# gavinsyw/2ACE-mmWave-Channel-Estimation

Measured on AMD Instinct MI355X. Metric: channel recoveries/sec (32-ant, 256 RSS meas, 200 ADMM iters) @1/2/4/8 GPU, higher is better.
Workload: dtype f64

## Files before the change

2ace-mmwave-channel-estimation_amd/ace_amd/_lib.py:

```python
from __future__ import annotations

import ctypes as C
import os
import pathlib

_HERE = pathlib.Path(__file__).resolve().parent
LIB_PATH = pathlib.Path(os.environ.get("ACE_LIB", _HERE / "libace.so"))

ACE_OK = 0
ACE_ERR_ARG = -1
ACE_ERR_UNSUPPORTED = -2
ACE_ERR_HIP = -3
ACE_ERR_WORKSPACE = -4

ACE_VARIANT_A2ONLY = 0
ACE_VARIANT_NUCLEAR = 1

ACE_ST_CONVERGED = 1
ACE_ST_NO_OPT = 2
ACE_ST_EIG_NOCONV = 4
ACE_ST_ROLLBACK = 8
ACE_ST_RANK_ONE = 128
ACE_ST_EVAL_DEGENERATE = 256
ACE_ST_RSS_SKIPPED = 512
ACE_ST_OMP_DEPENDENT = 1024
ACE_ST_GAMP_NANBREAK = 2048
ACE_ST_GAMP_MAXEM = 4096
ACE_ST_GAMP_FAILED = 8192

ACE_TRAIN_SHARED = 0
ACE_TRAIN_PER_REALISATION = 1

KERNEL_CLASSES = ["setup", "init", "pre", "apply_A", "apply_G", "ystep", "apply_K", "apply_AH", "zstep", "final", "msr"]


class AceError(RuntimeError):
    def __init__(self, code, msg):
        super().__init__(f"ace error {code}: {msg}")
        self.code = code


class AdmmCfg(C.Structure):
    _fields_ = [
        ("variant", C.c_int),
        ("scale_by_row", C.c_int),
        ("use_rank_one", C.c_int),
        ("maxiter", C.c_int),
        ("fixed_iters", C.c_int),
        ("a_shared", C.c_int),
        ("eig_warm", C.c_int),
        ("f64_applies", C.c_int),
        ("mu0", C.c_double),
        ("rho", C.c_double),
        ("tol_rel", C.c_double),
        ("tol_abs", C.c_double),
        ("r", C.c_int),
        ("reserved", C.c_int),
        ("rank_one", C.c_void_p),
    ]


class PipelineCfg(C.Structure):
    _fields_ = [
        ("variant", C.c_int),
        ("restarts", C.c_int),
        ("r", C.c_int),
        ("maxiter", C.c_int),
        ("eig_warm", C.c_int),
        ("stop_before_refine", C.c_int),
        ("train_layout", C.c_int),
        ("train_seed", C.c_int),
        ("mu0", C.c_double),
        ("rho", C.c_double),
        ("cc_frac", C.c_double),
        ("tol_rel", C.c_double),
        ("tol_abs", C.c_double),
    ]


class GampCfg(C.Structure):
    _fields_ = [
        ("snr_db", C.c_double),
        ("lambda0", C.c_double),
        ("learn_lambda", C.c_int),
        ("max_em_iter", C.c_int),
        ("gamp_nit", C.c_int),
        ("reserved", C.c_int),
        ("step0", C.c_double),
        ("gamp_tol", C.c_double),
    ]


class MinL2Cfg(C.Structure):
    _fields_ = [
        ("r", C.c_int),
        ("maxiter", C.c_int),
        ("train_seed", C.c_int),
        ("reserved", C.c_int),
        ("mu0", C.c_double),
        ("rho", C.c_double),
        ("cc_frac", C.c_double),
        ("tol_rel", C.c_double),
        ("tol_abs", C.c_double),
    ]


_dp, _ip, _bp = C.POINTER(C.c_double), C.POINTER(C.c_int32), C.POINTER(C.c_ubyte)


class StageArgs(C.Structure):
    _fields_ = ([(k, C.c_int32) for k in ("op", "row_mode", "batch", "n", "m", "r", "nc", "mt", "count", "ld", "col",
                                          "first", "scatter", "isentinel")]
                + [("or_mask", C.c_uint32), ("bit", C.c_uint32), ("len", C.c_int64)]
                + [(k, C.c_double) for k in ("mu0", "tol_abs", "value", "sentinel")]
                + [(k, _dp) for k in ("X", "Y", "P0", "B", "S", "g", "M", "A", "G", "geinv", "q", "qmax", "Xmax",
                                      "Ymax", "anorm", "bnorm", "optX", "optY", "Zb1", "Zb2", "Yb1", "Yb2", "src",
                                      "state")]
                + [(k, _ip) for k in ("flags", "rows", "idx", "isrc", "idst")]
                + [("mask", _bp), ("bsrc", _bp)]
                + [(k, _dp) for k in ("Xo", "Yo", "Mo", "No", "qo", "state_out")]
                + [("iout", _ip), ("flags_out", _ip), ("bout", _bp)])


def _load():
    if not LIB_PATH.exists():
        raise ImportError(
            f"ace_amd: HIP library {LIB_PATH} not found -- build it with "
            f"`make -C 2ace-mmwave-channel-estimation_amd/csrc` (or __graft_entry__.build()). "
            f"There is no CPU fallback on the product path.")
    lib = C.CDLL(str(LIB_PATH))
    vp, dp, ip, up = C.c_void_p, C.POINTER(C.c_double), C.POINTER(C.c_int32), C.POINTER(C.c_uint32)
    cfgp = C.POINTER(AdmmCfg)
    lib.ace_admm_cfg_default.argtypes = [cfgp]
    lib.ace_admm_cfg_default.restype = None
    lib.ace_admm_workspace_size.argtypes = [cfgp, C.c_int, C.c_int, C.c_int]
    lib.ace_admm_workspace_size.restype = C.c_size_t
    lib.ace_admm_solve_batch.argtypes = [cfgp, C.c_int, C.c_int, C.c_int, C.c_int, C.c_int,
                                         vp, vp, vp, vp, vp, vp, vp, vp, vp, C.c_size_t, vp]
    lib.ace_admm_solve_batch.restype = C.c_int
    lib.ace_admm_solve_host.argtypes = [cfgp, C.c_int, C.c_int, C.c_int, C.c_int, C.c_int,
                                        dp, dp, dp, dp, dp, ip, up, dp]
    lib.ace_admm_solve_host.restype = C.c_int
    pcfgp = C.POINTER(PipelineCfg)
    lib.ace_pipeline_cfg_default.argtypes = [pcfgp, C.c_int]
    lib.ace_pipeline_cfg_default.restype = None
    lib.ace_pipeline_workspace_size.argtypes = [pcfgp, C.c_int, C.c_int, C.c_int]
    lib.ace_pipeline_workspace_size.restype = C.c_size_t
    lib.ace_pipeline_solve_batch.argtypes = [pcfgp, C.c_int, C.c_int, C.c_int, C.c_int, C.c_int,
                                             vp, vp, ip, vp, vp, vp, vp, vp, vp, C.c_size_t, vp]
    lib.ace_pipeline_solve_batch.restype = C.c_int
    lib.ace_pipeline_solve_host.argtypes = [pcfgp, C.c_int, C.c_int, C.c_int, C.c_int, C.c_int,
                                            dp, dp, ip, dp, dp, dp, ip, up]
    lib.ace_pipeline_solve_host.restype = C.c_int
    lib.ace_synth_codebook.argtypes = [C.c_uint64, C.c_int64, C.c_int, C.c_int, C.c_int, vp, vp]
    lib.ace_synth_codebook.restype = C.c_int
    lib.ace_synth_channels.argtypes = [C.c_uint64, C.c_int64, C.c_int, C.c_int, C.c_int, C.c_int, C.c_int,
                                       C.c_double, C.c_double, vp, C.c_int, vp, vp, vp, vp]
    lib.ace_synth_channels.restype = C.c_int
    lib.ace_prof_start.argtypes = [C.c_int]
    lib.ace_prof_start.restype = C.c_int
    lib.ace_prof_sample.argtypes = [C.c_int, C.c_uint32]
    lib.ace_prof_sample.restype = C.c_int
    lib.ace_prof_stop.argtypes = [dp, ip]
    lib.ace_prof_stop.restype = C.c_int
    lib.ace_prof_msp_steps.argtypes = [C.POINTER(C.c_longlong)]
    lib.ace_prof_msp_steps.restype = C.c_int
    lib.ace_prof_work.argtypes = [dp]
    lib.ace_prof_work.restype = C.c_int
    lib.ace_prof_work_ex.argtypes = [dp, dp, dp]
    lib.ace_prof_work_ex.restype = C.c_int
    lib.ace_nuclear_prox_batch.argtypes = [C.c_int, C.c_int, C.c_int, vp, C.c_double, vp, vp]
    lib.ace_nuclear_prox_batch.restype = C.c_int
    lib.ace_evaluate_batch.argtypes = [C.c_int, C.c_int, C.c_int, vp, vp, vp, vp, vp]
    lib.ace_evaluate_batch.restype = C.c_int
    lib.ace_evaluate_host.argtypes = [C.c_int, C.c_int, C.c_int, dp, dp, dp, up]
    lib.ace_evaluate_host.restype = C.c_int
    lib.ace_rss_evaluate_batch.argtypes = [C.c_int, C.c_int, C.c_int, vp, vp, vp, C.c_int, vp, vp, vp, vp]
    lib.ace_rss_evaluate_batch.restype = C.c_int
    lib.ace_rss_evaluate_host.argtypes = [C.c_int, C.c_int, C.c_int, dp, dp, dp, C.c_int, dp, dp, up]
    lib.ace_rss_evaluate_host.restype = C.c_int
    lib.ace_beam_scan_batch.argtypes = [C.c_int] * 5 + [vp, vp, vp, vp, C.c_int, vp, vp, vp, vp, vp, vp]
    lib.ace_beam_scan_batch.restype = C.c_int
    lib.ace_beam_scan_host.argtypes = [C.c_int] * 5 + [dp, dp, dp, dp, C.c_int, dp, ip, dp, dp, up]
    lib.ace_beam_scan_host.restype = C.c_int
    lib.ace_omp_workspace_size.argtypes = [C.c_int] * 4
    lib.ace_omp_workspace_size.restype = C.c_size_t
    lib.ace_omp_solve_batch.argtypes = [C.c_int] * 4 + [C.c_double] + [vp] * 10 + [C.c_size_t, vp]
    lib.ace_omp_solve_batch.restype = C.c_int
    lib.ace_omp_solve_host.argtypes = [C.c_int] * 4 + [C.c_double, dp, dp, dp, ip, dp, ip, dp, up, dp]
    lib.ace_omp_solve_host.restype = C.c_int
    gcfgp = C.POINTER(GampCfg)
    lib.ace_gamp_cfg_default.argtypes = [gcfgp]
    lib.ace_gamp_cfg_default.restype = None
    lib.ace_gamp_workspace_size.argtypes = [C.c_int] * 3
    lib.ace_gamp_workspace_size.restype = C.c_size_t
    lib.ace_gamp_solve_batch.argtypes = [gcfgp] + [C.c_int] * 3 + [vp] * 9 + [C.c_size_t, vp]
    lib.ace_gamp_solve_batch.restype = C.c_int
    lib.ace_gamp_solve_host.argtypes = [gcfgp] + [C.c_int] * 3 + [dp, dp, dp, dp, dp, ip, ip, up]
    lib.ace_gamp_solve_host.restype = C.c_int
    mcfgp = C.POINTER(MinL2Cfg)
    lib.ace_minl2_cfg_default.argtypes = [mcfgp]
    lib.ace_minl2_cfg_default.restype = None
    lib.ace_minl2_workspace_size.argtypes = [C.c_int] * 4
    lib.ace_minl2_workspace_size.restype = C.c_size_t
    lib.ace_minl2_admm_batch.argtypes = [mcfgp] + [C.c_int] * 5 + [vp] * 12 + [vp, C.c_size_t, vp]
    lib.ace_minl2_admm_batch.restype = C.c_int
    lib.ace_minl2_admm_host.argtypes = [mcfgp] + [C.c_int] * 5 + [dp, dp, dp, ip, dp, dp, dp, ip, ip, dp, dp, up]
    lib.ace_minl2_admm_host.restype = C.c_int
    lib.ace_minl2_solve_workspace_size.argtypes = [mcfgp] + [C.c_int] * 3
    lib.ace_minl2_solve_workspace_size.restype = C.c_size_t
    lib.ace_minl2_solve_batch.argtypes = [mcfgp] + [C.c_int] * 3 + [vp, vp, ip] + [vp] * 6 + [vp, C.c_size_t, vp]
    lib.ace_minl2_solve_batch.restype = C.c_int
    lib.ace_minl2_solve_host.argtypes = [mcfgp] + [C.c_int] * 3 + [dp, dp, ip, dp, dp, dp, ip, ip, up]
    lib.ace_minl2_solve_host.restype = C.c_int
    lib.ace_spectral_init_host.argtypes = [C.c_int, C.c_int, C.c_int, C.c_int, vp, vp, vp, vp]
    lib.ace_spectral_init_host.restype = C.c_int
    lib.ace_path_counts.argtypes = [C.POINTER(C.c_int64), C.c_int]
    lib.ace_path_counts.restype = C.c_int
    lib.ace_lds_request.argtypes = [C.c_char_p, C.c_int, C.POINTER(C.c_size_t)]
    lib.ace_lds_request.restype = C.c_int
    lib.ace_stage_host.argtypes = [C.POINTER(StageArgs)]
    lib.ace_stage_host.restype = C.c_int
    lib.ace_last_error.argtypes = []
    lib.ace_last_error.restype = C.c_char_p
    lib.ace_version.argtypes = []
    lib.ace_version.restype = C.c_char_p
    return lib


LIB = _load()


def check(rc):
    if rc != ACE_OK:
        raise AceError(rc, LIB.ace_last_error().decode())
    return rc


PATHS = ("int8_shared", "codes_private", "f64_shared", "f64_private")


def path_counts(reset=False):
    v = (C.c_int64 * 4)()
    check(LIB.ace_path_counts(v, int(bool(reset))))
    return dict(zip(PATHS, v))


def lds_request(kernel: str, m: int) -> int:
    v = C.c_size_t()
    check(LIB.ace_lds_request(kernel.encode(), int(m), C.byref(v)))
    return v.value


def default_cfg(**kw) -> AdmmCfg:
    cfg = AdmmCfg()
    LIB.ace_admm_cfg_default(C.byref(cfg))
    for k, v in kw.items():
        if not hasattr(cfg, k):
            raise TypeError(f"unknown ace_admm_cfg field {k!r}")
        setattr(cfg, k, v)
    return cfg


def gamp_cfg(**kw) -> GampCfg:
    cfg = GampCfg()
    LIB.ace_gamp_cfg_default(C.byref(cfg))
    for k, v in kw.items():
        if not hasattr(cfg, k):
            raise TypeError(f"unknown ace_gamp_cfg field {k!r}")
        setattr(cfg, k, v)
    return cfg


def minl2_cfg(**kw) -> MinL2Cfg:
    cfg = MinL2Cfg()
    LIB.ace_minl2_cfg_default(C.byref(cfg))
    for k, v in kw.items():
        if not hasattr(cfg, k):
            raise TypeError(f"unknown ace_minl2_cfg field {k!r}")
        setattr(cfg, k, v)
    return cfg


def pipeline_cfg(variant, **kw) -> PipelineCfg:
    cfg = PipelineCfg()
    LIB.ace_pipeline_cfg_default(C.byref(cfg), int(variant))
    for k, v in kw.items():
        if not hasattr(cfg, k):
            raise TypeError(f"unknown ace_pipeline_cfg field {k!r}")
        setattr(cfg, k, v)
    return cfg
```

2ace-mmwave-channel-estimation_amd/csrc/ace_admm.cpp:

```cpp
#include "ace_host.hpp"

#include <cmath>
#include <cstdio>
#include <cstdlib>
#include <utility>
#include <vector>
#include <algorithm>
#include <map>
#include <mutex>

namespace ace {

size_t linops_bytes(bool shared, int batch, int m, int n) {
    Carver cv{nullptr};
    LinOps L;
    linops_carve(cv, shared, batch, m, n, &L);
    return cv.off;
}

void linops_carve(Carver& cv, bool shared, int batch, int m, int n, LinOps* L) {
    const size_t cz = 16, mats = shared ? 1 : (size_t)batch;
    L->shared = shared;
    L->m = m;
    L->n = n;
    L->AH = shared ? cv.take(cz * n * m) : nullptr;
    const bool pc = !shared && pc_supported(m, n);
    L->K = cv.take(mats * std::max(cz * m * m, pc ? pc_gw_bytes(m) : 0));
    L->G = cv.take(mats * std::max(cz * m * m, pc ? pc_gt_bytes(m) : 0));
    L->pcodes = pc ? cv.take<uint32_t>(pc_codes_bytes(m, n) * (size_t)batch) : nullptr;
    L->pcb = pc ? cv.take(sizeof(double) * (size_t)batch) : nullptr;
    L->pcflag = pc ? cv.take<int>(sizeof(int)) : nullptr;
    L->pc_ok = false;
    L->batch = batch;
    L->ns = shared ? cv.take(cz * 4 * m * m + 2 * sizeof(double)) : nullptr;
    L->LA8 = shared ? cv.take<int8_t>(i8_frag_bytes(m, n)) : nullptr;
    L->LAH8 = shared ? cv.take<int8_t>(i8_frag_bytes(n, m)) : nullptr;
    L->LK8 = shared ? cv.take<int8_t>(i8k_frag_bytes(m)) : nullptr;
    L->c8 = shared ? cv.take(2 * sizeof(double)) : nullptr;
    L->i8flag = shared ? cv.take<int>(sizeof(int)) : nullptr;
    L->Gf = shared && m <= GYK_MAXM ? cv.take(gyk_gfrag_bytes(m)) : nullptr;
    L->Kfr = shared && m <= GYK_MAXM ? cv.take(gyk_gfrag_bytes(m)) : nullptr;
    L->frag_ok = false;
    L->i8ok = false;
    L->gyk_ok = false;
    L->allow_i8 = true;
}

struct Knobs {
    int zcompact = 0, cold_sync = 0, msp_fail_it = -1, gyf_ctl = 1, msr_start = 56, msr_retry = 8, msr_waves = 8;
    int tkeig = 6;
    bool tk_trace = false;
    bool msr = true;
    bool fuse = true, gyf = true, mspace = true, lazy_dual = true, lean = true, nuc_msp = true, i8r = true, zcert = true;
    bool r1lz = true;
    double msp_room = 32.0;
};
static Knobs read_knobs() {
    Knobs k;
    const auto on = [](const char* name) {
        const char* e = getenv(name);
        return !(e && e[0] == '0');
    };
    const auto num = [](const char* name, double dflt) {
        const char* e = getenv(name);
        return e ? atof(e) : dflt;
    };
    k.zcompact = (int)num("ACE_ZCOMPACT", 0);
    k.cold_sync = exp_env("ACE_COLD_SYNC") ? atoi(exp_env("ACE_COLD_SYNC")) : 0;
    k.msp_fail_it = (int)num("ACE_MSP_FAIL_IT", -1);
    k.gyf_ctl = (int)num("ACE_GYF_CTL", 1);
    k.msp_room = num("ACE_MSP_ROOM", 32.0);
    k.fuse = on("ACE_FUSE");
    k.gyf = on("ACE_GYF");
    k.mspace = on("ACE_MSPACE");
    k.lazy_dual = on("ACE_LAZY_DUAL");
    k.lean = on("ACE_LEAN");
    k.nuc_msp = on("ACE_NUC_MSP");
    k.i8r = on("ACE_I8_STAGES");
    k.msr = on("ACE_MSR");
    k.zcert = on("ACE_ZCERT");
    k.r1lz = on("ACE_R1_LANCZOS");
    k.tkeig = (int)num("ACE_TK_EIG", 6);
    k.tk_trace = num("ACE_TK_TRACE", 0) != 0;
    k.msr_start = (int)num("ACE_MSR_START", 56);
    k.msr_retry = (int)num("ACE_MSR_RETRY", 8);
    if (k.msr_retry < 1) k.msr_retry = 1;
    k.msr_waves = (int)num("ACE_MSR_WAVES", 8) == 4 ? 4 : 8;
    return k;
}
static bool msr_trace() {
    static const bool v = [] {
        const char* e = exp_env("ACE_MSR_TRACE");
        return e && e[0] == '1';
    }();
    return v;
}
static bool fuse_ok(const Knobs& k, int m) {
    return k.fuse && lds_ok_budget(i8ah_budget(1), i8ah_lds_bytes(m) + i8ah_fuse_lds_bytes());
}
static bool gyf_ok(const Knobs& k, int m) { return k.gyf && lds_ok_budget(gyf_budget(), gyf_lds_bytes(m)); }

static bool i8_disabled() {
    static const bool v = [] {
        const char* e = getenv("ACE_NO_I8");
        return e && e[0] == '1';
    }();
    return v;
}

static int i8_setup(LinOps& L, hipStream_t st) {
    const int m = L.m, n = L.n;
    L.i8ok = false;
    if (!L.allow_i8 || i8_disabled()) return ACE_OK;
    ACE_HIP(hipMemsetAsync(L.LA8, 0, i8_frag_bytes(m, n), st));
    ACE_HIP(hipMemsetAsync(L.LAH8, 0, i8_frag_bytes(n, m), st));
    ACE_HIP(hipMemsetAsync(L.i8flag, 0, sizeof(int), st));
    launch_max_abs(2LL * m * n, L.A, L.c8, st);
    launch_i8_expand(m, n, L.A, L.c8, L.LA8, L.LAH8, L.i8flag, st);
    int flag = 1;
    double c[2] = {0.0, 0.0};
    ACE_HIP(read_back(&flag, L.i8flag, sizeof(int), st));
    ACE_HIP(read_back(c, L.c8, sizeof(double), st));
    L.i8ok = flag == 0 && c[0] > 0.0 && std::isfinite(c[0]) && lds_ok_budget(i8ah_budget(0), i8ah_lds_bytes(m)) &&
             lds_ok_budget(i8ah_budget(2), i8ah_lds_bytes(m));
    if (!L.i8ok) return ACE_OK;
    c[1] = c[0] * c[0];
    ACE_HIP(upload(L.c8 + 1, c + 1, sizeof(double), st));
    ACE_HIP(hipMemsetAsync(L.LK8, 0, i8k_frag_bytes(m), st));
    launch_i8k_expand(m, L.K, L.c8, L.LK8, L.i8flag, st);
    ACE_HIP(read_back(&flag, L.i8flag, sizeof(int), st));
    L.i8ok = flag == 0;
    L.gyk_ok = L.i8ok && L.Gf && lds_ok_budget(gyk_budget(), gyk_lds_bytes(m));
    return ACE_OK;
}

int ns_inverse(LinOps& L, hipStream_t st) {
    const int m = L.m;
    const long long mm = (long long)m * m;
    double* Ap = L.ns;
    double* Id = L.ns + 2 * mm;
    double* R = L.ns + 4 * mm;
    double* Xn = L.ns + 6 * mm;
    double* X = L.G;
    double* flag = L.ns + 8 * mm;
    launch_ns_prep(m, L.K, Ap, Id, X, st, flag + 1);
    double b = 0.0;
    ACE_HIP(read_back(&b, flag + 1, sizeof(double), st));
    int kpred = 60;
    if (std::isfinite(b) && b >= 1.0) {
        const double rho = (b - 1.0) / (b + 1.0);
        kpred = 0;
        for (double e = rho; e >= 1e-10 && kpred < 60; e *= e) ++kpred;
    }
    int it = 0;
    bool done = false;
    auto step = [&]() -> int {
        launch_zgemm(1, true, m, m, m, Ap, m, 0, X, m, 0, R, Id, m, 0, 1, st);
        launch_zgemm(2, true, m, m, m, R, m, 0, X, m, 0, Xn, X, m, 0, 1, st);
        launch_hermitize(m, Xn, st);
        std::swap(X, Xn);
        ++it;
        return ACE_OK;
    };
    for (int k = 0; k <= kpred && k < 60; ++k) ACE_TRY(step());
    {
        double h = 0.0;
        launch_max_abs(2 * mm, R, flag, st);
        ACE_HIP(read_back(&h, flag, sizeof(double), st));
        done = h < 1e-10;
    }
    for (; it < 60 && !done;) {
        launch_zgemm(1, true, m, m, m, Ap, m, 0, X, m, 0, R, Id, m, 0, 1, st);
        double h = 0.0;
        launch_max_abs(2 * mm, R, flag, st);
        ACE_HIP(read_back(&h, flag, sizeof(double), st));
        done = h < 1e-10;
        launch_zgemm(2, true, m, m, m, R, m, 0, X, m, 0, Xn, X, m, 0, 1, st);
        launch_hermitize(m, Xn, st);
        std::swap(X, Xn);
        ++it;
    }
#ifdef ACE_DEBUG_SPEC
    fprintf(stderr, "ns_inverse m %d b %g kpred %d it %d done %d\n", m, b, kpred, it, (int)done);
#endif
    if (!done) return fail(ACE_ERR_UNSUPPORTED, "setup: Newton-Schulz inverse of I + K did not converge");
    if (X != L.G) ACE_HIP(hipMemcpyAsync(L.G, X, sizeof(double) * 2 * mm, hipMemcpyDeviceToDevice, st));
    return ACE_OK;
}

static int pc_setup(LinOps& L, int batch, hipStream_t st) {
    const int m = L.m, n = L.n;
    L.pc_ok = false;
    if (L.shared || !L.pcodes || !L.allow_i8 || i8_disabled() || !pc_supported(m, n) || batch != L.batch ||
        !zstep_takes_w(ACE_VARIANT_A2ONLY, 1))
        return ACE_OK;
    ACE_HIP(hipMemsetAsync(L.pcflag, 0, sizeof(int), st));
    launch_pc_pack(batch, m, n, L.A, L.pcb, L.pcodes, L.pcflag, st);
    int flag = 1;
    ACE_HIP(read_back(&flag, L.pcflag, sizeof(int), st));
    if (flag != 0) return ACE_OK;
    launch_pc_ginv(batch, m, n, L.pcodes, L.pcb, L.K, L.G, st);
    ACE_LAUNCHED("private setup (code images, G_b)");
    L.pc_ok = true;
    return ACE_OK;
}

int linops_setup(LinOps& L, int batch, hipStream_t st) {
    const int m = L.m, n = L.n;
    const int mats = L.shared ? 1 : batch;
    const long long mm = (long long)m * m, mn = (long long)m * n;
    ProfScope ps(ACE_K_SETUP, st);
    if (!L.shared) {
        ACE_TRY(pc_setup(L, batch, st));
        if (L.pc_ok) return ACE_OK;
    }
    launch_zgemm(0, true, m, n, m, L.A, n, mn, L.A, n, mn, L.K, nullptr, m, mm, mats, st);
    if (L.shared) {
        ACE_TRY(ns_inverse(L, st));
    } else {
        ACE_HIP(hipMemcpyAsync(L.G, L.K, sizeof(double) * 2 * mm * mats, hipMemcpyDeviceToDevice, st));
        launch_inv_ipk(m, mats, L.G, mm, st);
    }
    if (L.shared) {
        launch_conj_transpose(m, n, L.A, L.AH, st);
        L.frag_ok = L.Gf && L.Kfr;
        if (L.frag_ok) {
            launch_gyk_gfrag(m, L.G, L.Gf, st);
            launch_gyk_gfrag(m, L.K, L.Kfr, st);
        }
        ACE_TRY(i8_setup(L, st));
    }
    ACE_LAUNCHED("operator setup (K, G, A^H, fragments, digit planes)");
    return ACE_OK;
}

void admm_state_carve(Carver& cv, int batch, int m, int n, int r, AdmmState* s) {
    const size_t cz = 16, bn = (size_t)batch * r * n, bm = (size_t)batch * r * m;
    s->X = cv.take(cz * bn);
    s->Z = cv.take(cz * bn);
    s->N = cv.take(cz * bn);
    s->V = cv.take(cz * bn);
    s->optX = cv.take(cz * bn);
    s->Q = cv.take(cz * (size_t)batch * 32 * 32);
    s->Z2 = cv.take(cz * (size_t)batch * n);
    s->N2 = cv.take(cz * (size_t)batch * n);
    s->AX = cv.take(cz * (size_t)batch * m);
    for (int i = 0; i < 2; ++i) s->Y[i] = cv.take(cz * bm);
    for (int i = 0; i < 2; ++i) s->KY[i] = cv.take(cz * bm);
    s->M = cv.take(cz * bm);
    s->S = cv.take(cz * bm);
    s->T = cv.take(cz * bm);
    s->g = cv.take(cz * bm);
    s->optY = cv.take(cz * bm);
    s->ypart = cv.take(sizeof(double) * 5 * (size_t)batch * r * ((m + 63) / 64));
// ... 96 lines not shown
        SplitRes& r = it->second;
        r.used = ++tick;
        for (int h = 0; h < nsplit; ++h) {
            ev[h] = r.e[h];
            cev[h] = r.c[h];
            if (h > 0) ss[h] = r.s[h];
        }
    }
    ACE_HIP(hipEventRecord(ev[0], st));
    for (int h = 1; h < nsplit; ++h) ACE_HIP(hipStreamWaitEvent(ss[h], ev[0], 0));
    std::vector<AdmmState> ws(nsplit);
    std::vector<int> nb(nsplit);
    for (int h = 0; h < nsplit; ++h) {
        const long long ob = (long long)h * chunk;
        nb[h] = (int)std::max(0LL, std::min((long long)chunk, batch - ob));
        ws[h] = state_slice(w, ob, m, n, za0.tx);
    }
    static const int stg = [] {
        const char* e = exp_env("ACE_STAGGER");
        return e ? atoi(e) : 0;
    }();
    hipEvent_t evs = nullptr;
    if (stg > 0 && nsplit > 1) ACE_HIP(hipEventCreateWithFlags(&evs, hipEventDisableTiming));
    auto split_fail = [&](int lc) -> int {
        for (int h = 1; h < nsplit; ++h)
            if (hipEventRecord(ev[h], ss[h]) == hipSuccess) (void)hipStreamWaitEvent(st, ev[h], 0);
        if (evs) (void)hipEventDestroy(evs);
        return lc;
    };
#define SPLIT_LAUNCHED(stage)                                           \
    do {                                                                \
        const int lc_ = ::ace::launch_check(stage, __FILE__, __LINE__); \
        if (lc_) return split_fail(lc_);                                \
    } while (0)
    auto stagger_mark = [&](int h, int it, int k) -> hipError_t {
        return (evs && h == 0 && it == 1 && k == stg) ? hipEventRecord(evs, ss[0]) : hipSuccess;
    };
    const bool lean = p.variant != ACE_VARIANT_NUCLEAR && za0.warm && za0.Q && kn.lean;
    const bool msp = lean && za0.lazy_dual && fuse_ok(kn, m) && gyf_ok(kn, m) && kn.mspace;
    const DualCtl dc{za0.tol_abs, za0.tol_rel, za0.rho, za0.fixed_iters, n, 1, w.done};
    const int cold_sync = kn.cold_sync;
    auto barrier = [&]() -> int {
        for (int h = 0; h < nsplit; ++h) ACE_HIP(hipEventRecord(cev[h], ss[h]));
        for (int h = 0; h < nsplit; ++h)
            for (int k = 0; k < nsplit; ++k)
                if (k != h) ACE_HIP(hipStreamWaitEvent(ss[h], cev[k], 0));
        return ACE_OK;
    };
    const bool msr = msp && kn.msr && kn.gyf_ctl && msr_supported(m) && gyf_ok(kn, m) && fuse_ok(kn, m);
    int msr_next = kn.msr_start;
    int q = 0, rc = ACE_OK;
    for (int it = 1; it <= p.maxiter && rc == ACE_OK; ++it) {
        bool run_msr = false;
        if (msr && it >= msr_next && it < p.maxiter) {
            for (int h = 1; h < nsplit; ++h) {
                ACE_HIP(hipEventRecord(cev[h], ss[h]));
                ACE_HIP(hipStreamWaitEvent(st, cev[h], 0));
            }
            ACE_HIP(hipMemsetD32Async(reinterpret_cast<hipDeviceptr_t>(w.done + 28), 0, 3, st));
            launch_msr_ready(batch, w.st, it, w.done + 28, st);
            int nr[3] = {0, 0, 0};
            ACE_HIP(read_back(nr, w.done + 28, sizeof(nr), st));
            run_msr = nr[0] == 0;
            if (msr_trace())
                fprintf(stderr, "msr check it %d: not ready %d (not m-space %d, test pending %d)\n", it, nr[0], nr[1],
                        nr[2]);
            if (!run_msr) msr_next = it + kn.msr_retry;
        }
        if (run_msr) {
            int pidx[4] = {-1, -1, -1, -1};
            for (int h = 0; h < nsplit; ++h) {
                if (nb[h] == 0) continue;
                const AdmmState& wh = ws[h];
                ZArgs za = za0;
                za.it = it;
                za.st = wh.st;
                za.msp = 1;
                za.msp_fail_it = kn.msp_fail_it;
                za.rank_one = za0.rank_one ? za0.rank_one + (long long)h * chunk : nullptr;
                const MsrArgs ma{L.Gf, B + (long long)h * chunk * m, {wh.Y[0], wh.Y[1]}, wh.M, wh.AX,
                                 {wh.Sg[0], wh.Sg[1]}, wh.optS, wh.optY, wh.st, w.done + 8 + h, w.done + 1,
                                 w.done + 12 + 4 * h, msr_trace() ? w.done + 40 + h : nullptr, nb[h], m, it, p.maxiter};
                ACE_HIP(hipMemsetD32Async(reinterpret_cast<hipDeviceptr_t>(w.done + 8 + h), p.maxiter, 1, ss[h]));
                ACE_HIP(hipMemsetD32Async(reinterpret_cast<hipDeviceptr_t>(w.done + 12 + 4 * h), 0, 4, ss[h]));
                ProfScope ps(ACE_K_MSR, ss[h]);
                pidx[h] = ps.idx;
                launch_msr(ma, za, kn.msr_waves, ss[h]);
                SPLIT_LAUNCHED("m-space run (msr_kernel)");
            }
            for (int h = 1; h < nsplit; ++h) {
                ACE_HIP(hipEventRecord(cev[h], ss[h]));
                ACE_HIP(hipStreamWaitEvent(st, cev[h], 0));
            }
            int rv[20] = {p.maxiter, p.maxiter, p.maxiter, p.maxiter};
            ACE_HIP(read_back(rv, w.done + 8, sizeof(int) * 20, st));
            for (int h = 0; h < nsplit; ++h) {
                if (pidx[h] >= 0) g_prof.work[pidx[h]] = 8.0 * m * m * rv[4 + 4 * h];
                if (msr_trace())
                    fprintf(stderr, "msr h %d it %d: resume %d steps %d notready %d fail %d pend %d\n", h, it, rv[h],
                            rv[4 + 4 * h], rv[5 + 4 * h], rv[6 + 4 * h], rv[7 + 4 * h]);
            }
            if (msr_trace()) {
                int vw[4] = {0, 0, 0, 0};
                ACE_HIP(read_back(vw, w.done + 40, sizeof(vw), st));
                fprintf(stderr, "msr it %d: vectors written %d %d %d %d (m = %d)\n", it, vw[0], vw[1], vw[2], vw[3], m);
            }
            int e = p.maxiter;
            for (int h = 0; h < nsplit; ++h)
                if (nb[h] > 0) e = std::min(e, std::max(it, rv[h]));
            it = e;
            q = (it - 1) & 1;
            msr_next = e + kn.msr_retry;
        }
        const bool csync = nsplit > 1 && it <= cold_sync;
      for (int phase = 0; phase < (csync ? 2 : 1); ++phase) {
        const int pmask = csync ? (1 << phase) : 3;
        for (int h = 0; h < nsplit; ++h) {
            if (nb[h] == 0) continue;
            const AdmmState& wh = ws[h];
            const hipStream_t sh = ss[h];
            if (evs && h > 0 && it == 1) ACE_HIP(hipStreamWaitEvent(sh, evs, 0));
            const double* Bh = B + (long long)h * chunk * m;
            double* Zc = (it & 1) ? wh.Z : wh.Z2;
            double* Nc = (it & 1) ? wh.N : wh.N2;
            ACE_HIP(stagger_mark(h, it, 1));
            ZArgs za = za0;
            za.it = it;
            za.wmode = 1;
            za.yfused = 1;
            za.ypart = nullptr;
            za.X = wh.X;
            za.Z = Zc;
            za.N = Nc;
            za.Zn = (it & 1) ? wh.Z2 : wh.Z;
            za.Nn = (it & 1) ? wh.N2 : wh.N;
            za.Q = wh.Q;
            za.st = wh.st;
            za.optX = wh.optX;
            za.optY = wh.optY;
            za.Xcur = wh.V;
            za.Ynew = wh.Y[1 - q];
            za.Yold = wh.Y[q];
            za.fixup_now = it == p.maxiter;
            za.rank_one = za0.rank_one ? za0.rank_one + (long long)h * chunk : nullptr;
            za.lean = lean;
            za.compact = lean && kn.zcompact > 0 && it > kn.zcompact && it != p.maxiter;
            za.xfuse = lean && (it != p.maxiter || msp) && fuse_ok(kn, m);
            za.msp = msp;
            za.Af = L.A;
            za.Sold = wh.Sg[(it + 1) & 1];
            za.Snew = wh.Sg[it & 1];
            za.optS = wh.optS;
            za.msp_fail_it = kn.msp_fail_it;
            const bool gyf = za.xfuse && za0.lazy_dual && gyf_ok(kn, m);
            GykArgs ga{L.Gf, wh.T, Bh, wh.Y[q], wh.M, wh.Y[1 - q], wh.g, wh.KY[q], wh.KY[1 - q], wh.optY,
                       L.LK8, L.c8, wh.st, wh.AX, 2 - q, L.LA8, Zc, Nc, w.zeros, n, za0.lazy_dual, dc, gyf ? 1 : 0,
                       gyf && msp ? 1 : 0, it, za.Sold, wh.Sg[it & 1], wh.optS, za0.np,
                       {za0.fl[0], za0.fl[1], za0.fl[2], za0.fl[3]}, za.rank_one, kn.msp_room};
            if (!(pmask & 1)) {
            } else if (gyf) {
                ProfScope ps(ACE_K_APPLY_G, sh);
                launch_gyf(nb[h], m, n, ga, L.LAH8, wh.X, za, kn.gyf_ctl, sh);
                SPLIT_LAUNCHED("g / Y-step / apply_AH (gyf_kernel)");
            } else {
                {
                    ProfScope ps(ACE_K_APPLY_G, sh);
                    launch_gyk(nb[h], m, ga, sh);
                }
                SPLIT_LAUNCHED("g / Y-step (gyk_kernel)");
                ACE_HIP(stagger_mark(h, it, 2));
                ProfScope ps(ACE_K_APPLY_AH, sh);
                launch_i8_apply_AH(nb[h], m, n, L.LAH8, wh.g, wh.X, L.c8, wh.st, sh, za.xfuse ? &za : nullptr);
                SPLIT_LAUNCHED("apply_AH (i8ah_kernel)");
            }
            ACE_HIP(stagger_mark(h, it, 3));
            if (pmask & 2) {
                ProfScope ps(ACE_K_ZSTEP, sh);
                if (lean && !za.xfuse) launch_zlean(za, nb[h], sh);
                launch_zstep(p.variant, false, za, nb[h], sh);
                SPLIT_LAUNCHED("Z-step");
            }
        }
        if (csync) ACE_TRY(barrier());
      }
        q = 1 - q;
        if (!p.fixed_iters && (it % 8 == 0) && it < p.maxiter) {
            for (int h = 1; h < nsplit; ++h) {
                ACE_HIP(hipEventRecord(cev[h], ss[h]));
                ACE_HIP(hipStreamWaitEvent(st, cev[h], 0));
            }
            int h_done = 0;
            ACE_HIP(read_back(&h_done, w.done, sizeof(int), st));
            if (h_done >= batch) break;
        }
    }
    for (int h = 1; h < nsplit; ++h) {
        ACE_HIP(hipEventRecord(ev[h], ss[h]));
        ACE_HIP(hipStreamWaitEvent(st, ev[h], 0));
    }
    ACE_LAUNCHED("split iterations");
#undef SPLIT_LAUNCHED
    {
        ProfScope ps(ACE_K_FINAL, st);
        if (msp) launch_i8_msp_optx(batch, m, n, L.LAH8, w.optS, w.optX, L.c8, w.st, w.Z, w.Z2, w.Sg[0], w.Sg[1], st);
        if (msp && g_prof.on && g_prof.msp_used < g_prof.msp_cap)
            ACE_HIP(hipMemcpyAsync(g_prof.msp_slots + g_prof.msp_used++, w.done + 1, sizeof(int),
                                   hipMemcpyDeviceToHost, st));
        launch_finalize_r(n, m, 1, 1, batch, w.optX, w.optY, w.V, w.Y[q], Xo, Yo, iters, status, mu_out, w.st, st, w.Z,
                          w.Z2, w.Y[0], w.Y[1]);
    }
    ACE_LAUNCHED("finalize (split)");
    if (evs) ACE_HIP(hipEventDestroy(evs));
    return rc;
}

static int admm_nuclear_msp(const LinOps& L, const AdmmParams& p, const AdmmState& w, const ZArgs& za0, int batch,
                            const double* B, double* Xo, double* Yo, int32_t* iters, uint32_t* status,
                            double* mu_out, hipStream_t st) {
    const int m = L.m, n = L.n;
    NmsArgs a{};
    a.Gf = L.Gf;
    a.Kf = L.Kfr;
    a.B = B;
    a.M = w.M;
    double *Eb[2] = {w.Sg[0], w.Sg[1]}, *AEb[2] = {w.KY[0], w.KY[1]};
    a.Eo = Eb[0];
    a.En = Eb[1];
    a.AEo = AEb[0];
    a.AEn = AEb[1];
    a.P0 = w.T;
    a.optW = w.optS;
    a.optY = w.optY;
    a.curW = w.g;
    a.rs = w.st;
    a.dc = DualCtl{za0.tol_abs, za0.tol_rel, za0.rho, za0.fixed_iters, n, 1, w.done};
    ZArgs za = za0;
    za.lazy_dual = 1;
    {
        ProfScope ps(ACE_K_INIT, st);
        launch_zgemm(0, false, m, n, batch, L.A, n, 0, w.X, n, 0, w.T, nullptr, m, 0, 1, st);
        launch_nms_init(batch, n, m, w.X, a, st);
    }
    int q = 0, it = 1;
    for (; it <= p.maxiter; ++it) {
        a.Yo = w.Y[q];
        a.Yn = w.Y[1 - q];
        a.Eo = Eb[q];
        a.En = Eb[1 - q];
        a.AEo = AEb[q];
        a.AEn = AEb[1 - q];
        za.it = it;
        {
            ProfScope ps(ACE_K_APPLY_G, st);
            launch_nms(batch, m, a, za, false, st);
        }
        ACE_LAUNCHED("A2nuclear m-space iteration (nms_kernel)");
        q = 1 - q;
        if (!p.fixed_iters && (it % 8 == 0) && it < p.maxiter) {
            int h_done = 0;
            ACE_HIP(read_back(&h_done, w.done, sizeof(int), st));
            if (h_done >= batch) break;
        }
    }
    {
        ProfScope ps(ACE_K_FINAL, st);
        a.Yo = w.Y[q];
        a.Yn = w.Y[1 - q];
        za.it = std::min(it, p.maxiter);
        launch_nms(batch, m, a, za, true, st);
        launch_nms_out(batch, n, m, w.X, a, w.V, w.g, st);
        launch_zgemm(2, false, n, m, batch, L.AH, m, 0, w.g, m, 0, w.optX, w.V, n, 0, 1, st);
        launch_finalize_r(n, m, 1, 1, batch, w.optX, w.optY, w.optX, w.Y[q], Xo, Yo, iters, status, mu_out, w.st, st,
                          nullptr, nullptr, nullptr, nullptr);
    }
    ACE_LAUNCHED("finalize (A2nuclear m-space)");
    return ACE_OK;
}

static int tk_report(const Knobs& kn, const AdmmState& w, int rc, hipStream_t st) {
    if (!kn.tk_trace || rc != ACE_OK) return rc;
    int tkc[2] = {0, 0};
    ACE_HIP(read_back(tkc, w.done + 32, sizeof(tkc), st));
    fprintf(stderr, "[ace] tridiagonal Z-steps %d, Jacobi fallbacks %d\n", tkc[0], tkc[1]);
    return rc;
}

int admm_run(const LinOps& L, const AdmmParams& p, const AdmmState& w, int batch, const double* B,
             const double* X0, double* Xo, double* Yo, int32_t* iters, uint32_t* status, double* mu_out,
             hipStream_t st) {
    const int m = L.m, n = L.n, r = p.r;
    const Knobs kn = read_knobs();
    if (!L.shared && r != 1) return fail(ACE_ERR_UNSUPPORTED, "private sensing matrices support r = 1 only");
    if (p.part && (r == 1 || !L.shared || p.part->m != m))
        return fail(ACE_ERR_UNSUPPORTED, "per-realisation partitions run the r-column stages on a shared A");
    const int row_mode = (r == 1) ? 1 : p.row_mode;
    const int nv = batch * r;
    const long long mm = (long long)m * m, mn = (long long)m * n;
    const bool fast = (r == 1);
    const bool fused = fast && L.shared;
    const bool i8 = fused && L.i8ok && zstep_takes_w(p.variant, r);
    const bool gyk = i8 && L.gyk_ok;
    const bool pc = !L.shared && L.pc_ok && r == 1 && zstep_takes_w(p.variant, r);
    const bool wmode = i8 || pc;
    const bool i8r = !fast && L.shared && L.i8ok && kn.i8r && nv >= 256;
    g_path[(i8 || i8r) ? 0 : pc ? 1 : L.shared ? 2 : 3].fetch_add(1, std::memory_order_relaxed);
    if (L.pc_ok && !pc) return fail(ACE_ERR_UNSUPPORTED, "private phase-code setup without its iteration path");

    auto applyA = [&](int mode, const double* Vin, double* C, const double* E) {
        if (L.shared) launch_zgemm(mode, false, m, n, nv, L.A, n, 0, Vin, n, 0, C, E, m, 0, 1, st);
        else launch_zgemv_rows(mode, m, n, batch, L.A, mn, Vin, n, C, E, m, st);
    };
    auto applyMM = [&](const double* Lm, const double* Vin, double* C) {
        if (L.shared) launch_zgemm(0, false, m, m, nv, Lm, m, 0, Vin, m, 0, C, nullptr, m, 0, 1, st);
        else launch_zgemv_rows(0, m, m, batch, Lm, mm, Vin, m, C, nullptr, m, st);
    };
    auto applyAH = [&](const double* gin, double* C, const double* E) {
        if (L.shared) launch_zgemm(2, false, n, m, nv, L.AH, m, 0, gin, m, 0, C, E, n, 0, 1, st);
        else launch_zgemv_cols(2, m, n, batch, L.A, mn, gin, m, C, E, n, st);
    };

    ZArgs za{};
    za.n = n;
    za.m = m;
    za.tx = p.tx;
    za.rx = p.rx;
    za.r = r;
    za.row_mode = row_mode;
    za.X = w.X;
    za.N = w.N;
    za.Z = w.Z;
    za.Q = w.Q;
    za.st = w.st;
    za.optX = w.optX;
    za.optY = w.optY;
    za.done_count = w.done;
    za.np = rank_profile(p.prof_tx ? p.prof_tx : p.tx, p.rx, m, p.prof_n ? p.prof_n : n,
                         p.rank_one ? 0 : p.use_rank_one, za.rl, za.fl);
    za.rank_one = p.rank_one;
    za.tol_rel = p.tol_rel;
    za.tol_abs = p.tol_abs;
    za.rho = p.rho;
    za.fixed_iters = p.fixed_iters;
    za.warm = p.eig_warm;
    za.zcert = kn.zcert ? 1 : 0;
    za.mthr = p.part ? p.part->mt : 0;
    za.r1lz = kn.r1lz ? 1 : 0;
    za.tkeig = kn.tkeig > 0 ? kn.tkeig : 0;
    za.tkcnt = w.done + 32;
    za.wmode = 0;
    za.Xcur = w.V;
    za.Zn = nullptr;
    za.Nn = nullptr;
    za.zeros = w.zeros;
    za.nuclear = p.variant == ACE_VARIANT_NUCLEAR;
    za.lazy_dual = (gyk && kn.lazy_dual) ? 1 : 0;
    za.Kf = L.K;

    const bool nms = L.shared && L.frag_ok && r == 1 && p.variant == ACE_VARIANT_NUCLEAR && kn.nuc_msp && nms_supported(m);
    ACE_HIP(hipMemsetAsync(w.done, 0, 256, st));
    ACE_HIP(hipMemsetAsync(w.zeros, 0, 16 * (size_t)n, st));
    {
        ProfScope ps(ACE_K_INIT, st);
        if (pc) launch_pc_apply_a(batch, m, n, L.pcodes + pc_codesA_off(batch, m, n), L.pcb, X0, w.T, st);
        else applyA(0, X0, w.T, nullptr);
        launch_init_r(row_mode, n, m, r, batch, X0, w.T, B, w.X, w.Y[0], w.M, w.N, w.st, p.mu0, st, p.part);
        if (!nms) {
            za.it = 0;
            launch_zstep(p.variant, true, za, batch, st);
            if (!pc && !za.lazy_dual) applyMM(L.K, w.Y[0], w.KY[0]);
        }
    }
    ACE_LAUNCHED("init (A X0, init, Z-step)");
    if (nms) return admm_nuclear_msp(L, p, w, za, batch, B, Xo, Yo, iters, status, mu_out, st);

    int q = 0;
    const int poll = 8;
    const int nsplit = gyk ? split_count(batch) : 1;
    if (nsplit > 1 || (gyk && kn.mspace && p.variant != ACE_VARIANT_NUCLEAR))
        return tk_report(kn, w, admm_iterate_split(L, p, w, za, batch, B, nsplit, kn, Xo, Yo, iters, status, mu_out, st), st);
    const double fl_mn = 8.0 * m * n * nv, fl_mm = 8.0 * m * m * nv;
    const double vb = 16.0 * nv;
    const double op_mn = 2.0 * 8 * (2.0 * m) * (2.0 * n) * nv, op_mm = 2.0 * 8 * 2 * (2.0 * m) * (2.0 * m) * nv;
    const double shA = L.shared ? 16.0 * m * n : 16.0 * m * n * batch, shM = L.shared ? 16.0 * m * m : 16.0 * m * m * batch;
    const double zs_fl = !fast ? (p.variant == ACE_VARIANT_NUCLEAR
                                      ? 8.0 * 3 * n * r * r * batch
                                      : (8.0 * p.tx * p.tx * p.rx * r + 0.8e6 * std::pow(p.tx / 32.0, 3)) * batch)
                               : 0.0;
    const double zs_b = !fast ? (80.0 * n * r + 64.0 * m * r + 32.0 * p.tx * p.tx) * batch : 0.0;
    double *Zc = w.Z, *Nc = w.N, *Zo = w.Z2, *No = w.N2;
    double lv = 1.0;
    for (int it = 1; it <= p.maxiter; ++it) {
        if (pc) {
            ProfScope ps(ACE_K_APPLY_G, st);
            const PgkArgs pa{m, n, L.pcodes, L.pcodes + pc_codesA_off(batch, m, n), L.G, L.pcb, B, w.Y[q], w.M,
                             w.Y[1 - q], w.X, w.optY, w.st, w.AX, 2 - q, Zc, Nc, w.zeros};
            launch_pgk(batch, pa, st);
            ACE_LAUNCHED("private g / Y-step / apply_AH (pgk_kernel)");
        } else if (gyk) {
        } else if (i8) {
            ProfScope ps(ACE_K_APPLY_A, st);
            launch_i8_apply_A(batch, n, m, L.LA8, Zc, Nc, w.Y[q], w.M, w.T, L.c8, w.st, w.zeros, gyk ? w.AX : nullptr, st);
            ACE_LAUNCHED("apply_A (i8a_kernel)");
        } else if (fused) {
            ProfScope ps(ACE_K_APPLY_A, st, lv * (fl_mn));
            launch_zgemm_fused(true, m, n, batch, L.A, n, w.Z, w.N, n, w.T, w.Y[q], w.M, m, w.st, st);
        } else {
            {
                ProfScope ps(ACE_K_PRE, st, 0.0, lv * (vb * (3.0 * m + (i8r ? 0.0 : 3.0 * n))));
                launch_pre(n * r, m * r, batch, w.Z, w.N, w.Y[q], w.M, i8r ? nullptr : w.V, w.S, w.st, st);
            }
            if (i8r) {
                ProfScope ps(ACE_K_APPLY_A, st, 0.0, lv * (vb * (2.0 * n + 3.0 * m)), lv * (op_mn));
                launch_i8_apply_A(nv, n, m, L.LA8, w.Z, w.N, w.Y[q], w.M, w.T, L.c8, w.st, w.zeros, nullptr, st, r);
                ACE_LAUNCHED("r-column apply_A (i8a_kernel)");
            } else {
                ProfScope ps(ACE_K_APPLY_A, st, lv * (fl_mn), lv * (vb * (n + 2.0 * m) + shA));
                applyA(1, w.V, w.T, w.S);
            }
        }
        if (pc) {
        } else if (gyk) {
            ProfScope ps(ACE_K_APPLY_G, st);
            const GykArgs ga{L.Gf, w.T, B, w.Y[q], w.M, w.Y[1 - q], w.g, w.KY[q], w.KY[1 - q], w.optY, L.LK8, L.c8, w.st,
                             w.AX, 2 - q, L.LA8, Zc, Nc, w.zeros, n, za.lazy_dual,
                             DualCtl{za.tol_abs, za.tol_rel, za.rho, za.fixed_iters, n, 1, w.done}};
            launch_gyk(batch, m, ga, st);
            ACE_LAUNCHED("g / Y-step (gyk_kernel)");
        } else if (fused) {
            ProfScope ps(ACE_K_APPLY_G, st, lv * (fl_mm));
            const YsArgs ys{B, w.Y[q], w.M, w.Y[1 - q], w.ypart};
            launch_zgemm_ystep(m, batch, L.G, w.T, w.g, ys, w.st, st);
        } else {
            {
                ProfScope ps(ACE_K_APPLY_G, st, lv * (fl_mm), lv * (vb * 2.0 * m + shM) * (p.part ? 2.0 : 1.0));
                applyMM(L.G, w.T, w.g);
                if (p.part) launch_part_gfix(batch, r, *p.part, L.G, w.g, w.st, st);
            }
            {
                ProfScope ps(ACE_K_YSTEP, st, 0.0, lv * (vb * 6.0 * m + 8.0 * m * batch));
                if (fast) launch_ystep(m, batch, w.S, w.g, w.M, B, w.Y[q], w.Y[1 - q], w.st, st);
                else launch_ystep_r(row_mode, m, r, batch, w.S, w.g, w.M, B, w.Y[q], w.Y[1 - q], w.st, st, p.part);
            }
        }
        ACE_LAUNCHED("apply_A / g = G T / Y-step");
        if (!gyk && !pc) {
            ProfScope ps(ACE_K_APPLY_K, st, lv * ((i8 || i8r) ? 0.0 : fl_mm), lv * ((i8 && !i8r) ? 0.0 : vb * 2.0 * m + (i8r ? 0.0 : shM)), lv * (i8r ? op_mm : 0.0));
            if (i8) launch_i8_apply_K(batch, m, L.LK8, w.Y[1 - q], w.KY[1 - q], L.c8, w.st, st);
            else if (i8r) launch_i8_apply_K(nv, m, L.LK8, w.Y[1 - q], w.KY[1 - q], L.c8, w.st, st, r);
            else applyMM(L.K, w.Y[1 - q], w.KY[1 - q]);
            ACE_LAUNCHED((i8 || i8r) ? "K Y (i8ah_kernel<KY>)" : "K Y (zgemm)");
        }
        if (!pc) {
            ProfScope ps(ACE_K_APPLY_AH, st, lv * ((wmode || i8r) ? 0.0 : fl_mn),
                         lv * (wmode ? 0.0 : i8r ? vb * (m + 3.0 * n) : vb * (m + 2.0 * n) + shA), lv * (i8r ? op_mn : 0.0));
            if (wmode) {
                za.xfuse = gyk && wmode && p.variant != ACE_VARIANT_NUCLEAR && za.warm && za.Q && kn.lean &&
                           it != p.maxiter && fuse_ok(kn, m);
                if (za.xfuse) {
                    za.it = it;
                    za.wmode = 1;
                    za.Z = Zc;
                    za.N = Nc;
                    za.Zn = Zo;
                    za.Nn = No;
                }
                launch_i8_apply_AH(batch, m, n, L.LAH8, w.g, w.X, L.c8, w.st, st, za.xfuse ? &za : nullptr);
            }
            else if (fused) launch_zgemm_fused(false, n, m, batch, L.AH, m, w.g, nullptr, m, w.X, w.Z, w.N, n, w.st, st);
            else if (i8r) {
                ZArgs zv{};
                zv.r = r;
                zv.xzn = 1;
                zv.Z = w.Z;
                zv.N = w.N;
                zv.zeros = w.zeros;
                launch_i8_apply_AH(nv, m, n, L.LAH8, w.g, w.X, L.c8, w.st, st, nullptr, &zv);
            } else applyAH(w.g, w.X, w.V);
            ACE_LAUNCHED((wmode || i8r) ? "apply_AH (i8ah_kernel)" : "apply_AH (zgemm)");
        }
        za.it = it;
        za.wmode = wmode;
        if (wmode) {
            za.Z = Zc;
            za.N = Nc;
            za.Zn = Zo;
            za.Nn = No;
        }
        za.ypart = fused && !gyk ? w.ypart : nullptr;
        za.yfused = gyk || pc;
        za.ytiles = (m + 63) / 64;
        za.Ynew = w.Y[1 - q];
        za.Yold = w.Y[q];
        za.KYnew = w.KY[1 - q];
        za.KYold = w.KY[q];
        za.lean = wmode && p.variant != ACE_VARIANT_NUCLEAR && za.warm && za.Q && kn.lean;
        za.fixup_now = it == p.maxiter;
        za.compact = za.lean && kn.zcompact > 0 && it > kn.zcompact;
        {
            ProfScope ps(ACE_K_ZSTEP, st, lv * (zs_fl), lv * (zs_b));
            if (za.lean && !za.xfuse) launch_zlean(za, batch, st);
            launch_zstep(p.variant, false, za, batch, st);
            ACE_LAUNCHED("Z-step");
        }
        q = 1 - q;
        if (wmode) {
            std::swap(Zc, Zo);
            std::swap(Nc, No);
        }
        if (!p.fixed_iters && (it % poll == 0) && it < p.maxiter) {
            int h_done = 0;
            ACE_HIP(read_back(&h_done, w.done, sizeof(int), st));
            if (h_done >= batch) break;
            lv = (double)(batch - h_done) / batch;
        }
    }
    {
        ProfScope ps(ACE_K_FINAL, st);
        launch_finalize_r(n, m, r, row_mode ? r : 1, batch, w.optX, w.optY, wmode ? w.V : w.X, w.Y[q], Xo, Yo, iters, status,
                          mu_out, w.st, st, wmode ? w.Z : nullptr, wmode ? w.Z2 : nullptr, (gyk || pc) ? w.Y[0] : nullptr,
                          (gyk || pc) ? w.Y[1] : nullptr);
    }
    ACE_LAUNCHED("finalize");
    return tk_report(kn, w, ACE_OK, st);
}

}
```

2ace-mmwave-channel-estimation_amd/csrc/ace_api.cpp:

```cpp
#include <algorithm>
#include <cstring>
#include <mutex>
#include <unordered_map>

#include "ace_host.hpp"

using namespace ace;

namespace {
int cols(const ace_admm_cfg* c) { return c->r == 0 ? 1 : c->r; }

int validate(const ace_admm_cfg* c, int batch, int m, int n, int tx, int rx) {
    if (!c) return fail(ACE_ERR_ARG, "cfg is NULL");
    if (batch < 1 || m < 1 || n < 1) return fail(ACE_ERR_ARG, "batch/m/n must be >= 1 (got %d/%d/%d)", batch, m, n);
    if (tx * rx != n) return fail(ACE_ERR_ARG, "n (%d) != tx*rx (%d*%d)", n, tx, rx);
    if (c->variant != ACE_VARIANT_A2ONLY && c->variant != ACE_VARIANT_NUCLEAR)
        return fail(ACE_ERR_ARG, "unknown variant %d", c->variant);
    if (c->variant == ACE_VARIANT_A2ONLY && (tx < 1 || tx > 32 || ((tx & 1) && tx > 31) || rx > 32))
        return fail(ACE_ERR_UNSUPPORTED, "A2only Z-prox needs tx in [1,32] and rx <= 32 (got %d, %d)", tx, rx);
    if (n > 4096 || m > 4096) return fail(ACE_ERR_UNSUPPORTED, "m, n must be <= 4096 (got %d, %d)", m, n);
    if (c->maxiter < 1) return fail(ACE_ERR_ARG, "maxiter must be >= 1");
    if (!(c->mu0 > 0) || !(c->rho > 0)) return fail(ACE_ERR_ARG, "mu0 and rho must be > 0");
    const int r = cols(c);
    if (r < 1 || r > 32) return fail(ACE_ERR_UNSUPPORTED, "r must be in [1, 32] (got %d)", r);
    if (r > 1 && !c->a_shared) return fail(ACE_ERR_UNSUPPORTED, "r > 1 needs a shared A (a_shared = 1)");
    return ACE_OK;
}
}

namespace ace {
namespace {
std::mutex g_lds_mu;
std::unordered_map<const void*, size_t> g_lds_budget;
thread_local std::string t_refused;
}

size_t lds_dyn_budget(const void* kernel) {
    std::lock_guard<std::mutex> lk(g_lds_mu);
    const auto it = g_lds_budget.find(kernel);
    if (it != g_lds_budget.end()) return it->second;
    hipFuncAttributes fa{};
    size_t budget = 0;
    if (hipFuncGetAttributes(&fa, kernel) == hipSuccess && fa.sharedSizeBytes < LDS_PER_CU) {
        const size_t want = LDS_PER_CU - fa.sharedSizeBytes;
        if (hipFuncSetAttribute(kernel, hipFuncAttributeMaxDynamicSharedMemorySize, (int)want) == hipSuccess)
            budget = want;
    }
    (void)hipGetLastError();
    g_lds_budget.emplace(kernel, budget);
    return budget;
}

void launch_refused(const char* kernel, size_t need, size_t budget) {
    if (!t_refused.empty()) return;
    char buf[256];
    snprintf(buf, sizeof buf, "%s not launched: %zu B of dynamic LDS requested, budget %zu B", kernel, need, budget);
    t_refused = buf;
}

bool lds_ok_budget(size_t budget, size_t need) { return need <= 64 * 1024 || need <= budget; }
bool lds_ok(const void* kernel, size_t need) {
    return need <= 64 * 1024 || need <= lds_dyn_budget(kernel);
}
bool lds_fits(const void* kernel, const char* name, size_t need) {
    if (lds_ok(kernel, need)) return true;
    launch_refused(name, need, lds_dyn_budget(kernel));
    return false;
}

int launch_check(const char* stage, const char* file, int line) {
    if (!t_refused.empty()) {
        const std::string why = t_refused;
        t_refused.clear();
        (void)hipGetLastError();
        return fail(ACE_ERR_UNSUPPORTED, "%s: %s (%s:%d)", stage, why.c_str(), file, line);
    }
    const hipError_t e = hipGetLastError();
    if (e != hipSuccess) return fail(ACE_ERR_HIP, "%s: launch failed: %s (%s:%d)", stage, hipGetErrorString(e), file, line);
    return ACE_OK;
}
}

extern "C" {

const char* ace_last_error(void) { return g_err.c_str(); }
const char* ace_version(void) { return "ace-mi355x 0.1.0 (gfx950)"; }

int ace_lds_request(const char* kernel, int m, size_t* bytes) {
    g_err.clear();
    if (!kernel || !bytes || m < 1) return fail(ACE_ERR_ARG, "bad ace_lds_request arguments");
    const std::string k = kernel;
    if (k == "i8ah" || k == "i8ah_ky") *bytes = i8ah_lds_bytes(m);
    else if (k == "i8ah_fuse") *bytes = i8ah_lds_bytes(m) + i8ah_fuse_lds_bytes();
    else if (k == "gyk") *bytes = gyk_lds_bytes(m);
    else if (k == "gyf") *bytes = gyf_lds_bytes(m);
    else if (k == "msr") *bytes = msr_request_bytes();
    else if (k == "nms") *bytes = nms_lds_bytes(m);
    else if (k == "hetrd") *bytes = hetrd_request_bytes(m, 0);
    else if (k == "hetrd_blk") *bytes = hetrd_request_bytes(m, 1);
    else if (k == "he2hb") *bytes = heev2_request_bytes(m, 0);
    else if (k == "hb2st") *bytes = heev2_request_bytes(m, 1);
    else if (k == "bt2") *bytes = heev2_request_bytes(m, 2);
    else if (k == "scan") *bytes = scan_request_bytes();
    else if (k == "omp") *bytes = omp_request_bytes(m);
    else if (k == "gamp") *bytes = gamp_request_bytes(m);
    else if (k == "minl2") *bytes = minl2_request_bytes(m);
    else if (k == "part_geinv") *bytes = part_geinv_request_bytes(m);
    else return fail(ACE_ERR_ARG, "unknown kernel '%s'", kernel);
    return ACE_OK;
}

int ace_prof_sample(int stride, uint32_t full_mask) {
    g_err.clear();
    if (stride < 1) return fail(ACE_ERR_ARG, "stride must be >= 1");
    g_prof.stride = stride;
    g_prof.full = full_mask;
    return ACE_OK;
}

int ace_prof_start(int max_launches) {
    g_err.clear();
    if (max_launches < 1) return fail(ACE_ERR_ARG, "max_launches must be >= 1");
    for (hipEvent_t e : g_prof.ev) (void)hipEventDestroy(e);
    g_prof.ev.assign(2 * (size_t)max_launches, nullptr);
    for (auto& e : g_prof.ev) ACE_HIP(hipEventCreate(&e));
    g_prof.cls.assign(max_launches, 0);
    g_prof.work.assign(max_launches, 0.0);
    g_prof.wbytes.assign(max_launches, 0.0);
    g_prof.wops.assign(max_launches, 0.0);
    g_prof.used = 0;
    for (int& c : g_prof.seen) c = 0;
    if (!g_prof.msp_slots) {
        g_prof.msp_cap = 4096;
        ACE_HIP(hipHostMalloc(reinterpret_cast<void**>(&g_prof.msp_slots), sizeof(int) * g_prof.msp_cap));
    }
    g_prof.msp_used = 0;
    g_prof.on = true;
    return ACE_OK;
}

int ace_prof_msp_steps(long long* steps) {
    g_err.clear();
    if (!steps) return fail(ACE_ERR_ARG, "steps is NULL");
    *steps = g_prof.msp_total;
    return ACE_OK;
}

int ace_prof_work(double* flops) {
    g_err.clear();
    if (!flops) return fail(ACE_ERR_ARG, "flops is NULL");
    for (int c = 0; c < ACE_NKCLASS; ++c) flops[c] = g_prof.work_tot[c];
    return ACE_OK;
}

int ace_prof_work_ex(double* flops, double* bytes, double* int8_ops) {
    g_err.clear();
    for (int c = 0; c < ACE_NKCLASS; ++c) {
        if (flops) flops[c] = g_prof.work_tot[c];
        if (bytes) bytes[c] = g_prof.bytes_tot[c];
        if (int8_ops) int8_ops[c] = g_prof.ops_tot[c];
    }
    return ACE_OK;
}

int ace_path_counts(int64_t* counts, int reset) {
    g_err.clear();
    for (int k = 0; k < 4; ++k) {
        const long long v = reset ? g_path[k].exchange(0) : g_path[k].load();
        if (counts) counts[k] = v;
    }
    return ACE_OK;
}

int ace_prof_stop(double* total_ms, int32_t* launches) {
    g_err.clear();
    g_prof.on = false;
    for (int c = 0; c < ACE_NKCLASS; ++c) {
        if (total_ms) total_ms[c] = 0.0;
        if (launches) launches[c] = 0;
        g_prof.work_tot[c] = g_prof.bytes_tot[c] = g_prof.ops_tot[c] = 0.0;
    }
    for (size_t i = 0; i < g_prof.used; ++i) {
        ACE_HIP(hipEventSynchronize(g_prof.ev[2 * i + 1]));
        float ms = 0.f;
        ACE_HIP(hipEventElapsedTime(&ms, g_prof.ev[2 * i], g_prof.ev[2 * i + 1]));
        const int c = g_prof.cls[i];
        g_prof.work_tot[c] += g_prof.work[i];
        g_prof.bytes_tot[c] += g_prof.wbytes[i];
        g_prof.ops_tot[c] += g_prof.wops[i];
        if (total_ms) total_ms[c] += ms;
        if (launches) launches[c] += 1;
    }
    for (hipEvent_t e : g_prof.ev) (void)hipEventDestroy(e);
    g_prof.ev.clear();
    g_prof.cls.clear();
    g_prof.work.clear();
    g_prof.wbytes.clear();
    g_prof.wops.clear();
    g_prof.used = 0;
    ACE_HIP(hipDeviceSynchronize());
    g_prof.msp_total = 0;
    for (int i = 0; i < g_prof.msp_used; ++i) g_prof.msp_total += g_prof.msp_slots[i];
    g_prof.msp_used = 0;
    return ACE_OK;
}

void ace_admm_cfg_default(ace_admm_cfg* c) {
    std::memset(c, 0, sizeof *c);
    c->variant = ACE_VARIANT_A2ONLY;
    c->scale_by_row = 1;
    c->use_rank_one = 0;
    c->maxiter = 500;
    c->fixed_iters = 0;
    c->a_shared = 1;
    c->eig_warm = 1;
    c->mu0 = 1e-3;
    c->rho = 1.03;
    c->tol_rel = 1e-4;
    c->tol_abs = 1e-8;
    c->r = 1;
    c->rank_one = nullptr;
}

size_t ace_admm_workspace_size(const ace_admm_cfg* cfg, int batch, int m, int n) {
    if (!cfg || batch < 1 || m < 1 || n < 1) return 0;
    Carver cv{nullptr};
    LinOps L;
    AdmmState w;
    linops_carve(cv, cfg->a_shared != 0, batch, m, n, &L);
    admm_state_carve(cv, batch, m, n, std::max(1, cols(cfg)), &w);
    return cv.off + 256;
}

}

namespace {
int solve_core(const ace_admm_cfg* cfg, int batch, int m, int n, int tx, int rx, int prof_tx, int prof_n,
               const double* A, const double* B, const double* X0, double* Xo, double* Yo, int32_t* iters,
               uint32_t* status, double* mu_out, void* workspace, size_t workspace_bytes, hipStream_t st);

int solve_odd_tx(const ace_admm_cfg* cfg, int batch, int m, int n, int tx, int rx, const double* A,
                 const double* B, const double* X0, double* Xo, double* Yo, int32_t* iters, uint32_t* status,
                 double* mu_out, hipStream_t st) {
    const int txp = tx + 1, np = txp * rx, r = cols(cfg), R = cfg->scale_by_row ? r : 1;
    const size_t arows = (size_t)(cfg->a_shared ? 1 : batch) * m * rx, xrows = (size_t)batch * r * rx,
                 orows = (size_t)batch * R * rx, ws = ace_admm_workspace_size(cfg, batch, m, np) + 4096;
    DevScope d;
    d.borrow(st);
    double *dA, *dX0, *dX;
    char* dW;
    ACE_TRY(d.alloc(&dA, 2 * arows * txp));
    ACE_TRY(d.alloc(&dX0, 2 * xrows * txp));
    ACE_TRY(d.alloc(&dX, 2 * orows * txp));
    ACE_TRY(d.alloc(&dW, ws));
    ACE_HIP(hipMemsetAsync(dA, 0, arows * txp * 16, st));
    ACE_HIP(hipMemsetAsync(dX0, 0, xrows * txp * 16, st));
    ACE_HIP(hipMemcpy2DAsync(dA, (size_t)txp * 16, A, (size_t)tx * 16, (size_t)tx * 16, arows, hipMemcpyDeviceToDevice, st));
    ACE_HIP(hipMemcpy2DAsync(dX0, (size_t)txp * 16, X0, (size_t)tx * 16, (size_t)tx * 16, xrows, hipMemcpyDeviceToDevice,
                             st));
    ACE_TRY(solve_core(cfg, batch, m, np, txp, rx, tx, n, dA, B, dX0, dX, Yo, iters, status, mu_out, dW, ws, st));
    ACE_HIP(hipMemcpy2DAsync(Xo, (size_t)tx * 16, dX, (size_t)txp * 16, (size_t)tx * 16, orows, hipMemcpyDeviceToDevice,
                             st));
    return ACE_OK;
}
}

extern "C" {

int ace_admm_solve_batch(const ace_admm_cfg* cfg, int batch, int m, int n, int tx, int rx, const double* A,
                         const double* B, const double* X0, double* Xo, double* Yo, int32_t* iters, uint32_t* status,
                         double* mu_out, void* workspace, size_t workspace_bytes, void* stream) {
    g_err.clear();
    int rc = validate(cfg, batch, m, n, tx, rx);
    if (rc) return rc;
    if (!A || !B || !X0 || !Xo || !Yo || !workspace) return fail(ACE_ERR_ARG, "NULL buffer");
    hipStream_t st = (hipStream_t)stream;
    if (cfg->variant == ACE_VARIANT_A2ONLY && (tx & 1))
        return solve_odd_tx(cfg, batch, m, n, tx, rx, A, B, X0, Xo, Yo, iters, status, mu_out, st);
    return solve_core(cfg, batch, m, n, tx, rx, 0, 0, A, B, X0, Xo, Yo, iters, status, mu_out, workspace,
                      workspace_bytes, st);
}

}

namespace {
int solve_core(const ace_admm_cfg* cfg, int batch, int m, int n, int tx, int rx, int prof_tx, int prof_n,
               const double* A, const double* B, const double* X0, double* Xo, double* Yo, int32_t* iters,
               uint32_t* status, double* mu_out, void* workspace, size_t workspace_bytes, hipStream_t st) {
    const size_t need = ace_admm_workspace_size(cfg, batch, m, n);
    if (need > workspace_bytes)
        return fail(ACE_ERR_WORKSPACE, "workspace too small: need %zu bytes, got %zu", need, workspace_bytes);
    poison_workspace(workspace, workspace_bytes, st);
    Carver cv{(char*)(((uintptr_t)workspace + 255) & ~(uintptr_t)255)};
    LinOps L;
    AdmmState w;
    linops_carve(cv, cfg->a_shared != 0, batch, m, n, &L);
    admm_state_carve(cv, batch, m, n, cols(cfg), &w);
    L.A = A;
    L.allow_i8 = cfg->f64_applies == 0;
    ACE_TRY(linops_setup(L, batch, st));
    AdmmParams p{};
    p.variant = cfg->variant;
    p.r = cols(cfg);
    p.row_mode = cfg->scale_by_row != 0;
    p.maxiter = cfg->maxiter;
    p.fixed_iters = cfg->fixed_iters;
    p.eig_warm = cfg->eig_warm;
    p.mu0 = cfg->mu0;
    p.rho = cfg->rho;
    p.tol_rel = cfg->tol_rel;
    p.tol_abs = cfg->tol_abs;
    p.tx = tx;
    p.rx = rx;
    p.prof_tx = prof_tx;
    p.prof_n = prof_n;
    p.use_rank_one = cfg->use_rank_one;
    p.rank_one = cfg->rank_one;
    return admm_run(L, p, w, batch, B, X0, Xo, Yo, iters, status, mu_out, st);
}
}

extern "C" {

int ace_admm_solve_host(const ace_admm_cfg* cfg, int batch, int m, int n, int tx, int rx, const double* A,
                        const double* B, const double* X0, double* X, double* Y, int32_t* iters, uint32_t* status,
                        double* mu) {
    g_err.clear();
    int rc = validate(cfg, batch, m, n, tx, rx);
    if (rc) return rc;
    const int r = cols(cfg), R = cfg->scale_by_row ? r : 1;
    const size_t nA = (size_t)(cfg->a_shared ? 1 : batch) * m * n * 2;
    const size_t nB = (size_t)batch * m, nX0 = (size_t)batch * r * n * 2, nX = (size_t)batch * R * n * 2,
                 nY = (size_t)batch * R * m * 2;
    const size_t ws = ace_admm_workspace_size(cfg, batch, m, n) + 4096;
    DevScope d;
    double *dA, *dB, *dX0, *dX, *dY, *dM;
    char* dW;
    int32_t* dI;
    uint32_t* dS;
    ACE_TRY(d.put(&dA, A, nA));
    ACE_TRY(d.put(&dB, B, nB));
    ACE_TRY(d.put(&dX0, X0, nX0));
    ACE_TRY(d.alloc(&dX, nX));
    ACE_TRY(d.alloc(&dY, nY));
    ACE_TRY(d.alloc(&dW, ws));
    ACE_TRY(d.alloc(&dI, (size_t)batch));
    ACE_TRY(d.alloc(&dS, (size_t)batch));
    ACE_TRY(d.alloc(&dM, (size_t)batch));
    ace_admm_cfg dcfg = *cfg;
    if (cfg->rank_one) {
        uint8_t* dR;
        ACE_TRY(d.put(&dR, cfg->rank_one, (size_t)batch));
        dcfg.rank_one = dR;
    }
    ACE_TRY(ace_admm_solve_batch(&dcfg, batch, m, n, tx, rx, dA, dB, dX0, dX, dY, dI, dS, dM, dW, ws, nullptr));
    ACE_HIP(hipDeviceSynchronize());
// ... 40 lines not shown
```

2ace-mmwave-channel-estimation_amd/csrc/ace_common.hpp:

```cpp
#pragma once
#include <hip/hip_runtime.h>
#include <stdint.h>
#include <cstdlib>

#include "../../include/ace.h"

namespace ace {

using d2 = double2;
typedef double d4v __attribute__((ext_vector_type(4)));

__device__ __forceinline__ d2 cmul(d2 a, d2 b) { return make_double2(a.x * b.x - a.y * b.y, a.x * b.y + a.y * b.x); }
__device__ __forceinline__ d2 cmulc(d2 a, d2 b) {  return make_double2(a.x * b.x + a.y * b.y, a.x * b.y - a.y * b.x); }
__device__ __forceinline__ d2 cadd(d2 a, d2 b) { return make_double2(a.x + b.x, a.y + b.y); }
__device__ __forceinline__ d2 csub(d2 a, d2 b) { return make_double2(a.x - b.x, a.y - b.y); }
__device__ __forceinline__ d2 cscale(d2 a, double s) { return make_double2(a.x * s, a.y * s); }
__device__ __forceinline__ double cabs2(d2 a) { return a.x * a.x + a.y * a.y; }

struct RealState {
    double mu, last_res, opt_obj, nB;
    double obj2, nAX2, nY2, nJM2, dY2;
    double vbound;
    double dAtY, nAtY;
    int32_t iters, done, status, objcol;
// ... 51 lines not shown
}
__device__ __forceinline__ double bsum16(double v) {
    v += bfly16<1>(v);
    v += bfly16<2>(v);
    v += bfly16<4>(v);
    v += bfly16<8>(v);
    return v;
}
__device__ __forceinline__ double bmax16(double v) {
    v = fmax(v, bfly16<1>(v));
    v = fmax(v, bfly16<2>(v));
    v = fmax(v, bfly16<4>(v));
    v = fmax(v, bfly16<8>(v));
    return v;
}
__device__ __forceinline__ double wave_sum(double v) {
#pragma unroll
    for (int o = 32; o > 0; o >>= 1) v += __shfl_xor(v, o, 64);
    return v;
}

__device__ __forceinline__ double wave_max(double v) {
#pragma unroll
    for (int o = 32; o > 0; o >>= 1) v = fmax(v, __shfl_xor(v, o, 64));
    return v;
}

struct VMax {
    double m = 0.0, s = 0.0;
    __device__ __forceinline__ void add(double2 v) {
        const double ax = fabs(v.x), ay = fabs(v.y);
        m = fmax(m, fmax(ax, ay));
        s += 0.0 * (ax + ay);
    }
};

__device__ __forceinline__ double xor16_sum(double v) {
    const auto lo = __builtin_amdgcn_permlane16_swap(__double2loint(v), __double2loint(v), false, false);
    const auto hi = __builtin_amdgcn_permlane16_swap(__double2hiint(v), __double2hiint(v), false, false);
    return __hiloint2double(hi[0], lo[0]) + __hiloint2double(hi[1], lo[1]);
}
__device__ __forceinline__ double xor32_sum(double v) {
    const auto lo = __builtin_amdgcn_permlane32_swap(__double2loint(v), __double2loint(v), false, false);
    const auto hi = __builtin_amdgcn_permlane32_swap(__double2hiint(v), __double2hiint(v), false, false);
    return __hiloint2double(hi[0], lo[0]) + __hiloint2double(hi[1], lo[1]);
}
__device__ __forceinline__ double wave_sum_dpp(double v) {
    return xor32_sum(xor16_sum(bsum16(v)));
}
template <int NV>
__device__ __forceinline__ void block_sum_dpp(double (&v)[NV], double* sh) {
    const int lane = threadIdx.x & 63, w = threadIdx.x >> 6, nw = (blockDim.x + 63) >> 6;
#pragma unroll
    for (int i = 0; i < NV; ++i) v[i] = wave_sum_dpp(v[i]);
    __syncthreads();
    if (lane == 0)
#pragma unroll
        for (int i = 0; i < NV; ++i) sh[w * NV + i] = v[i];
    __syncthreads();
#pragma unroll
    for (int i = 0; i < NV; ++i) {
        double s = 0.0;
        for (int k = 0; k < nw; ++k) s += sh[k * NV + i];
        v[i] = s;
    }
    __syncthreads();
}

template <int NV>
__device__ __forceinline__ void block_sum_dpp1(double (&v)[NV], double* sh) {
    const int lane = threadIdx.x & 63, w = threadIdx.x >> 6, nw = (blockDim.x + 63) >> 6;
#pragma unroll
    for (int i = 0; i < NV; ++i) v[i] = wave_sum_dpp(v[i]);
    if (lane == 0)
#pragma unroll
        for (int i = 0; i < NV; ++i) sh[w * NV + i] = v[i];
    __syncthreads();
#pragma unroll
    for (int i = 0; i < NV; ++i) {
        double s = 0.0;
        for (int k = 0; k < nw; ++k) s += sh[k * NV + i];
        v[i] = s;
    }
}

template <int NV>
__device__ __forceinline__ void block_sum(double (&v)[NV], double* sh) {
    const int lane = threadIdx.x & 63, w = threadIdx.x >> 6, nw = (blockDim.x + 63) >> 6;
#pragma unroll
    for (int i = 0; i < NV; ++i) v[i] = wave_sum(v[i]);
    __syncthreads();
    if (lane == 0)
#pragma unroll
        for (int i = 0; i < NV; ++i) sh[w * NV + i] = v[i];
    __syncthreads();
#pragma unroll
    for (int i = 0; i < NV; ++i) {
        double s = 0.0;
        for (int k = 0; k < nw; ++k) s += sh[k * NV + i];
        v[i] = s;
    }
    __syncthreads();
}

inline const char* exp_env(const char* name) {
#ifdef ACE_EXPERIMENTS
    return getenv(name);
#else
    (void)name;
    return nullptr;
#endif
}

constexpr size_t LDS_PER_CU = 160 * 1024;
size_t lds_dyn_budget(const void* kernel);
void launch_refused(const char* kernel, size_t need, size_t budget);
int launch_check(const char* stage, const char* file, int line);
#define ACE_LAUNCHED(stage)                                                 \
    do {                                                                    \
        const int lc_ = ::ace::launch_check(stage, __FILE__, __LINE__);     \
        if (lc_) return lc_;                                                \
    } while (0)
bool lds_fits(const void* kernel, const char* name, size_t need);
bool lds_ok(const void* kernel, size_t need);
bool lds_ok_budget(size_t budget, size_t need);
size_t msr_request_bytes();
size_t hetrd_request_bytes(int d, int blk);
size_t heev2_request_bytes(int d, int which);
size_t scan_request_bytes();
size_t omp_request_bytes(int d);
size_t gamp_request_bytes(int d);
size_t minl2_request_bytes(int m);
size_t part_geinv_request_bytes(int te);

void launch_zgemm(int mode, bool conj_l, int M, int K, int nb, const double* L, int ldl, long long strideL,
                  const double* V, int ldv, long long strideV, double* C, const double* E, int ldc,
                  long long strideC, int nz, hipStream_t st, const double* klim = nullptr, long long klim_stride = 0);

void launch_zgemv_rows(int mode, int M, int K, int nb, const double* L, long long strideL, const double* V,
                       int ldv, double* C, const double* E, int ldc, hipStream_t st);
void launch_zgemv_cols(int mode, int M, int K, int nb, const double* L, long long strideL, const double* V,
                       int ldv, double* C, const double* E, int ldc, hipStream_t st);

void launch_inv_ipk(int m, int count, double* G, long long strideG, hipStream_t st);
struct RealState;
void launch_zgemm_fused(bool fv, int M, int K, int nb, const double* L, int ldl, const double* V, const double* V2,
                        int ldv, double* C, const double* E, const double* E2, int ldc, const RealState* rs,
                        hipStream_t st);
int i8_nks(int kc);
int i8_ncols(int mc);
size_t i8_frag_bytes(int mc, int kc);
void launch_i8_expand(int m, int n, const double* A, const double* cmax, int8_t* LA, int8_t* LH, int* flag,
                      hipStream_t st);
void launch_i8_apply_A(int nb, int n, int m, const int8_t* LA, const double* Z, const double* N, const double* Y,
                       const double* M, double* T, const double* cmax, const RealState* rs, const double* zeros,
                       const double* AX, hipStream_t st, int rcols = 1);
struct ZArgs;
void launch_i8_apply_AH(int nb, int m, int n, const int8_t* LAH, const double* g, double* W, const double* cmax,
                        const RealState* rs, hipStream_t st, const ZArgs* fuse = nullptr,
                        const ZArgs* plain = nullptr);
size_t i8ah_lds_bytes(int kc);
size_t i8ah_fuse_lds_bytes();
size_t i8ah_budget(int kind);
void launch_i8_msp_optx(int nb, int m, int n, const int8_t* LAH, const double* optS, double* optX, const double* cmax,
                        RealState* rs, const double* Zb1, const double* Zb2, const double* S0, const double* S1,
                        hipStream_t st);
constexpr int GYK_MAXM = 256;
size_t gyk_gfrag_bytes(int m);
size_t gyk_lds_bytes(int m);
size_t gyk_budget();
size_t gyf_budget();
void launch_gyk_gfrag(int m, const double* G, double* Gf, hipStream_t st);
struct GykArgs {
    const double* Gf;
    const double* T;
    const double* B;
    const double* Yo;
    double* M;
    double* Yn;
    double* g;
    const double* KYo;
    double* KYn;
    double* optY;
    const int8_t* LK;
    const double* c8;
    RealState* rs;
    double* AX;
    int yn_id;
    const int8_t* LA;
    const double* Z;
    const double* N;
    const double* zeros;
    int n;
    int lazy;
    DualCtl dc;
    int glds;
    int msp;
    int it;
    const double* Sold;
    double* Snew;
    double* optS;
    int np;
    double fl[4];
    const unsigned char* rank_one;
    double room;
};
void launch_gyk(int nb, int m, const GykArgs& a, hipStream_t st);
size_t gyf_lds_bytes(int m);
void launch_gyf(int nb, int m, int n, const GykArgs& a, const int8_t* LAH, double* W, const ZArgs& za, int ctl,
                hipStream_t st);
struct MsrArgs {
    const double* Gf;
    const double* B;
    double* Y[2];
    double* M;
    double* AX;
    double* S[2];
    double* optS;
    double* optY;
    RealState* rs;
    int* resume;
    int* mspcount;
    int* steps;
    int* vecw;
    int nb, m, it0, it_end;
};
bool msr_supported(int m);
void launch_msr_ready(int nb, const RealState* rs, int it, int* notready, hipStream_t st);
void launch_msr(const MsrArgs& a, const ZArgs& za, int waves, hipStream_t st);
size_t i8k_frag_bytes(int m);
void launch_i8k_expand(int m, const double* K, const double* cmax, int8_t* LK, int* flag, hipStream_t st);
void launch_i8_apply_K(int nb, int m, const int8_t* LK, const double* Y, double* KY, const double* cmax,
                       const RealState* rs, hipStream_t st, int rcols = 1);
void launch_ns_prep(int m, const double* K, double* Ap, double* Id, double* X0, hipStream_t st, double* bnd);
void launch_max_abs(long long n, const double* x, double* out, hipStream_t st);
void launch_hermitize(int m, double* X, hipStream_t st);

constexpr int PC_MAXM = 256, PC_MAXN = 2048;
bool pc_supported(int m, int n);
size_t pc_codes_bytes(int m, int n);
size_t pc_codesA_off(int batch, int m, int n);
size_t pc_gw_bytes(int m);
size_t pc_gt_bytes(int m);
void launch_pc_pack(int batch, int m, int n, const double* A, double* cb, uint32_t* codes, int* flag, hipStream_t st);
void launch_pc_ginv(int batch, int m, int n, const uint32_t* codes, const double* cb, double* Gw, double* Gt,
                    hipStream_t st);
struct PgkArgs {
    int m, n;
    const uint32_t* codesH;
    const uint32_t* codesA;
    const double* Gt;
    const double* cb;
    const double* B;
    const double* Yo;
    double* M;
    double* Yn;
    double* W;
    double* optY;
    RealState* rs;
    double* AX;
    int yn_id;
    const double* Z;
    const double* N;
    const double* zeros;
};
void launch_pgk(int batch, const PgkArgs& a, hipStream_t st);
void launch_pc_apply_a(int batch, int m, int n, const uint32_t* codesA, const double* cb, const double* X0, double* P0,
                       hipStream_t st);

struct NmsArgs {
    const double* Gf;
    const double* Kf;
    const double* B;
    const double* Yo;
    double* Yn;
    double* M;
    double* Eo;
    double* En;
    double* AEo;
    double* AEn;
    const double* P0;
    double* optW;
    double* optY;
    double* curW;
    RealState* rs;
    DualCtl dc;
};
size_t nms_lds_bytes(int m);
bool nms_supported(int m);
void launch_nms(int nb, int m, const NmsArgs& a, const ZArgs& za, bool fin, hipStream_t st);
void launch_nms_init(int nb, int n, int m, const double* Xi, const NmsArgs& a, hipStream_t st);
void launch_nms_out(int nb, int n, int m, const double* Xi, const NmsArgs& a, double* V, double* Wsel, hipStream_t st);

struct ZArgs {
    int n, m, tx, rx;
    int r;
    int row_mode;
    const double* X;
    double* N;
    double* Z;
    double* Q;
    RealState* st;
    double* optX;
    double* optY;
    const double* Ynew;
    const double* Yold;
    const double* KYnew;
    const double* KYold;
    int* done_count;
    int np;
    int rl[4];
    double fl[4];
    const unsigned char* rank_one;
    double tol_rel, tol_abs, rho;
    int it, fixed_iters, warm, ld_state;
    const double* ypart;
    int ytiles;
    int wmode;
    double* Xcur;
    double* Zn;
    double* Nn;
    int yfused;
    const double* zeros;
    int nuclear;
    int lean;
    int lazy_dual;
    const double* Kf;
    int fixup_now;
    int xfuse;
    int compact;
    int msp;
    const double* Af;
    const double* Sold;
    const double* Snew;
    const double* optS;
    int matz;
    int msp_fail_it;
    int xzn;
    int zcert;
    int r1lz;
    int mthr;
    int tkeig;
    int* tkcnt;
};
__device__ __forceinline__ double2 xw(double2 z, double2 n, double2 w, double imu) {
    return make_double2(fma(-n.x, imu, z.x) + w.x, fma(-n.y, imu, z.y) + w.y);
}
struct YsArgs {
    const double* B;
    const double* Yo;
    double* M;
    double* Yn;
    double* part;
};
void launch_zgemm_ystep(int m, int nb, const double* G, const double* T, double* g, const YsArgs& ys,
                        const RealState* rs, hipStream_t st);

void launch_zstep(int variant, bool init, const ZArgs& a, int batch, hipStream_t st);
int launch_nuclear_prox(int batch, int n, int r, const double* E, double tau, double* Z, hipStream_t st);
bool zstep_takes_w(int variant, int r);

struct ZProfile {
    int np;
    int rl[4];
    double fl[4];
};
__device__ __forceinline__ ZProfile z_profile_flag(const ZArgs& a, int rank_one_b) {
    ZProfile p;
    if (rank_one_b) {
        p.np = 1;
        p.rl[0] = 1;
        p.fl[0] = 0.95;
        for (int i = 1; i < 4; ++i) { p.rl[i] = 0; p.fl[i] = 0.0; }
    } else {
        p.np = a.np;
        for (int i = 0; i < 4; ++i) { p.rl[i] = a.rl[i]; p.fl[i] = a.fl[i]; }
    }
    return p;
}
__device__ __forceinline__ ZProfile z_profile(const ZArgs& a, int b) {
    return z_profile_flag(a, a.rank_one ? (int)a.rank_one[b] : 0);
}
void launch_zstep1w(bool init, const ZArgs& a, int batch, hipStream_t st);
void launch_zlean(const ZArgs& a, int batch, hipStream_t st);
void launch_pre(int n, int m, int batch, const double* Z, const double* N, const double* Y, const double* M, double* V,
                double* S, const RealState* rs, hipStream_t st);
void launch_ystep(int m, int batch, const double* S, const double* g, double* M, const double* B, const double* Yold,
                  double* Ynew, RealState* rs, hipStream_t st);
struct PartRows {
    const int* rows;
    const unsigned char* mask;
    const double* geinv;
    int m, mt, ldmask;
};
constexpr int PART_MAXTE = 96;
void launch_init_r(int row_mode, int n, int m, int r, int batch, const double* X0, const double* P0,
                   const double* B, double* X, double* Y, double* M, double* N, RealState* rs, double mu0,
                   hipStream_t st, const PartRows* pr = nullptr);
void launch_ystep_r(int row_mode, int m, int r, int batch, const double* S, const double* g, double* M,
                    const double* B, const double* Yold, double* Ynew, RealState* rs, hipStream_t st,
                    const PartRows* pr = nullptr);
void launch_part_geinv(int nb, const PartRows& pr, const double* G, double* geinv, int* status, hipStream_t st);
void launch_part_gfix(int nb, int r, const PartRows& pr, const double* G, double* g, const RealState* rs,
                      hipStream_t st);
void launch_part_expand(int nb, int r, const PartRows& pr, const double* src, double* dst, hipStream_t st);
void launch_part_compact(int nb, int r, const PartRows& pr, const double* src, double* dst, hipStream_t st);
void launch_part_quality(int n, int nb, const PartRows& pr, const double* A, const double* X, const double* B,
                         double* q, hipStream_t st);
void launch_finalize_r(int n, int m, int r, int nc, int batch, const double* optX, const double* optY,
                       const double* Xc, const double* Yc, double* Xo, double* Yo, int32_t* iters,
                       uint32_t* status, double* mu, RealState* rs, hipStream_t st,
                       const double* Zb1 = nullptr, const double* Zb2 = nullptr, const double* Yb1 = nullptr,
                       const double* Yb2 = nullptr);
void launch_conj_transpose(int rows, int cols, const double* A, double* AH, hipStream_t st);
void launch_synth_codebook(uint64_t seed, long long first, int count, int m, int n, double* A, hipStream_t st);
void launch_synth_channels(uint64_t seed, long long first, int count, int m, int tx, int rx, int L, double snr_db,
                           double x0_noise, const double* A, int a_shared, double* vecH, double* B, double* X0,
                           hipStream_t st);

}
```

2ace-mmwave-channel-estimation_amd/csrc/ace_host.hpp:

```cpp
#pragma once
#include <hip/hip_runtime.h>

#include <cmath>
#include <cstdarg>
#include <cstdio>
#include <cstdlib>
#include <cstring>
#include <atomic>
#include <string>
#include <vector>

#include "ace_common.hpp"

namespace ace {

inline thread_local std::string g_err;

__attribute__((format(printf, 2, 3))) inline int fail(int code, const char* fmt, ...) {
    char buf[512];
    va_list ap;
    va_start(ap, fmt);
    vsnprintf(buf, sizeof buf, fmt, ap);
    va_end(ap);
    g_err = buf;
    return code;
}

#define ACE_HIP(call)                                                                                  \
    do {                                                                                               \
        hipError_t e_ = (call);                                                                        \
        if (e_ != hipSuccess) return fail(ACE_ERR_HIP, "%s: %s (%s:%d)", #call, hipGetErrorString(e_), \
                                          __FILE__, __LINE__);                                         \
    } while (0)

#define ACE_TRY(call)          \
    do {                       \
        int rc_ = (call);      \
        if (rc_) return rc_;   \
    } while (0)

struct Prof {
    bool on = false;
    std::vector<hipEvent_t> ev;
    std::vector<int> cls;
    std::vector<double> work;
    std::vector<double> wbytes;
    std::vector<double> wops;
    double work_tot[ACE_NKCLASS] = {};
    double bytes_tot[ACE_NKCLASS] = {};
    double ops_tot[ACE_NKCLASS] = {};
    size_t used = 0;
    int stride = 1;
    unsigned full = 0;
    int seen[ACE_NKCLASS] = {};
    int* msp_slots = nullptr;
    int msp_cap = 0, msp_used = 0;
    long long msp_total = 0;
};
inline Prof g_prof;
inline std::atomic<long long> g_path[4];

struct Pinned {
    void* p = nullptr;
    size_t cap = 0;
    ~Pinned() {
        if (p) (void)hipHostFree(p);
    }
    hipError_t reserve(size_t bytes) {
        if (bytes <= cap) return hipSuccess;
        if (p) (void)hipHostFree(p);
        p = nullptr;
        cap = 0;
        const size_t want = bytes < 4096 ? 4096 : bytes;
        const hipError_t e = hipHostMalloc(&p, want, hipHostMallocDefault);
        if (e == hipSuccess) cap = want;
        return e;
    }
};
inline thread_local Pinned g_stage;
inline hipError_t read_back(void* dst, const void* src, size_t bytes, hipStream_t st) {
    hipError_t e = g_stage.reserve(bytes);
    if (e == hipSuccess) e = hipMemcpyAsync(g_stage.p, src, bytes, hipMemcpyDeviceToHost, st);
    if (e == hipSuccess) e = hipStreamSynchronize(st);
    if (e == hipSuccess) memcpy(dst, g_stage.p, bytes);
    return e;
}
inline hipError_t upload(void* dst, const void* src, size_t bytes, hipStream_t st) {
    hipError_t e = g_stage.reserve(bytes);
    if (e == hipSuccess) e = hipStreamSynchronize(st);
    if (e == hipSuccess) memcpy(g_stage.p, src, bytes);
    if (e == hipSuccess) e = hipMemcpyAsync(dst, g_stage.p, bytes, hipMemcpyHostToDevice, st);
    if (e == hipSuccess) e = hipStreamSynchronize(st);
    return e;
}

inline void poison_workspace(void* ws, size_t bytes, hipStream_t st) {
    static const bool on = [] {
        const char* e = exp_env("ACE_POISON");
        return e && e[0] == '1';
    }();
    if (on) (void)hipMemsetAsync(ws, 0xFF, bytes, st);
}

struct ProfScope {
    hipStream_t st;
    int idx = -1;
    ProfScope(int c, hipStream_t s, double work = 0.0, double bytes = 0.0, double ops = 0.0) : st(s) {
        const bool pick = ((g_prof.full >> c) & 1u) || (g_prof.seen[c] % g_prof.stride) == 0;
        if (g_prof.on) ++g_prof.seen[c];
        if (g_prof.on && pick && g_prof.used < g_prof.cls.size()) {
            idx = (int)g_prof.used++;
            g_prof.cls[idx] = c;
            g_prof.work[idx] = work;
            g_prof.wbytes[idx] = bytes;
            g_prof.wops[idx] = ops;
            (void)hipEventRecord(g_prof.ev[2 * idx], st);
        }
    }
    ~ProfScope() {
        if (idx >= 0) (void)hipEventRecord(g_prof.ev[2 * idx + 1], st);
    }
};

inline int rank_profile(int tx, int rx, int m, int n, int use_rank_one, int* rl, double* fl) {
    const int sz = tx < rx ? tx : rx;
    const int r0 = (int)std::ceil(std::sqrt((double)sz) * 0.5), r1 = (int)std::ceil(std::sqrt((double)sz) * 0.7);
    const int r2 = (int)std::ceil(std::sqrt((double)sz));
    int r3 = (int)std::ceil(std::sqrt((double)sz) * 2.0);
    if (r3 > sz) r3 = sz;
    if (use_rank_one) { rl[0] = 1; fl[0] = 0.95; return 1; }
    if (m >= n * 3) { rl[0] = r3; fl[0] = 0.995; return 1; }
    if (r1 <= 2) { rl[0] = r2; fl[0] = 0.95; return 1; }
    if (r0 <= 2) {
        rl[0] = r1; rl[1] = r2; rl[2] = r3;
        fl[0] = 0.9; fl[1] = 0.95; fl[2] = 0.995;
        return 3;
    }
    rl[0] = r0; rl[1] = r1; rl[2] = r2; rl[3] = r3;
    fl[0] = 0.8; fl[1] = 0.9; fl[2] = 0.95; fl[3] = 0.995;
    return 4;
}

struct Carver {
    char* base;
    size_t off = 0;
    template <class T = double>
    T* take(size_t bytes) {
        char* p = base ? base + off : nullptr;
        off += (bytes + 255) & ~(size_t)255;
        return reinterpret_cast<T*>(p);
    }
};

template <class T>
struct NoDeduce {
    using type = T;
};
struct DevScope {
    std::vector<void*> bufs;
    hipStream_t st = nullptr;
    bool drain = false, owned = false;
    DevScope() = default;
    DevScope(const DevScope&) = delete;
    DevScope& operator=(const DevScope&) = delete;
    ~DevScope() {
        if (drain) (void)hipStreamSynchronize(st);
        if (owned) (void)hipStreamDestroy(st);
        for (void* p : bufs) (void)hipFree(p);
    }
    int own_stream() {
        ACE_HIP(hipStreamCreateWithFlags(&st, hipStreamNonBlocking));
        drain = owned = true;
        return ACE_OK;
    }
    void borrow(hipStream_t s) {
        st = s;
        drain = true;
    }
    template <class T>
    int alloc(T** p, size_t count) {
        void* q = nullptr;
        ACE_HIP(hipMalloc(&q, sizeof(T) * (count ? count : 1)));
        bufs.push_back(q);
        *p = static_cast<T*>(q);
        return ACE_OK;
    }
    template <class T>
    int set(T* dst, const typename NoDeduce<T>::type* src, size_t count, typename NoDeduce<T>::type fill = T{}) {
        if (!count) return ACE_OK;
        std::vector<T> tmp;
        if (!src) {
            tmp.assign(count, fill);
            src = tmp.data();
        }
        if (owned) ACE_HIP(upload(dst, src, sizeof(T) * count, st));
        else ACE_HIP(hipMemcpy(dst, src, sizeof(T) * count, hipMemcpyHostToDevice));
        return ACE_OK;
    }
    template <class T>
    int put(T** p, const typename NoDeduce<T>::type* src, size_t count, typename NoDeduce<T>::type fill = T{}) {
        ACE_TRY(alloc(p, count));
        return set(*p, src, count, fill);
    }
    template <class T>
    int get(T* dst, const typename NoDeduce<T>::type* src, size_t count) {
        if (!dst || !count) return ACE_OK;
        if (owned) ACE_HIP(read_back(dst, src, sizeof(T) * count, st));
        else ACE_HIP(hipMemcpy(dst, src, sizeof(T) * count, hipMemcpyDeviceToHost));
        return ACE_OK;
    }
// ... 70 lines not shown
```

2ace-mmwave-channel-estimation_amd/csrc/ace_i8gemm.hip:

```cpp
#include "ace_i8.hpp"
#include "ace_mfma.hpp"
#include "ace_zcommon.hpp"

namespace ace {

namespace {

#ifdef ACE_PHASE_STAMPS
#define STAMP_DECL unsigned long long ts_[12] = {}
#define STAMP(i) do { if (blockIdx.x == 5 && threadIdx.x == 0) ts_[i] = __builtin_amdgcn_s_memrealtime(); } while (0)
#define STAMP_D(i) (i < k_ ? ts_[i] - ts_[i - 1] : 0ull)
#define STAMP_PRINT(name, k) do { if (blockIdx.x == 5 && threadIdx.x == 0) { const int k_ = (k); \
    printf("%s %llu %llu %llu %llu %llu %llu %llu\n", name, STAMP_D(1), STAMP_D(2), STAMP_D(3), STAMP_D(4), \
           STAMP_D(5), STAMP_D(6), STAMP_D(7)); } } while (0)
#else
#define STAMP_DECL
#define STAMP(i)
#define STAMP_PRINT(name, k)
#endif

constexpr int RB = 16;
constexpr int ROWS = RB * 8;
constexpr int KC = 128;
constexpr int NCB = 512;
constexpr int NT = 512;
constexpr int KSC = KC / 32;

__device__ __forceinline__ int i8_nks_dev(int kc) { return (2 * kc + KC - 1) / KC * KSC; }

__device__ __forceinline__ void digits4(const double (&v)[4], double p2, uint32_t (&out)[8]) {
    uint32_t lo[4];
    int32_t hi[4];
#pragma unroll
    for (int i = 0; i < 4; ++i) {
        const double x = rint(v[i] * p2);
        const double h = floor(x * 0x1p-32);
        const double l = fma(-h, 0x1p32, x);
        hi[i] = (int32_t)h;
        lo[i] = (uint32_t)l;
    }
#pragma unroll
    for (int t = 0; t < 8; ++t) {
        uint32_t d[4];
#pragma unroll
        for (int i = 0; i < 4; ++i) {
            if (t < 4) d[i] = (lo[i] >> (7 * t)) & 127u;
            else if (t == 4) d[i] = __builtin_amdgcn_alignbit((uint32_t)hi[i], lo[i], 28) & 127u;
            else if (t == 5) d[i] = ((uint32_t)hi[i] >> 3) & 127u;
            else if (t == 6) d[i] = ((uint32_t)hi[i] >> 10) & 127u;
            else d[i] = (uint32_t)(hi[i] >> 17) & 255u;
        }
        out[t] = d[0] | (d[1] << 8) | (d[2] << 16) | (d[3] << 24);
    }
}

__device__ __forceinline__ void aload(const int8_t* arow, int rstride, i4v (&af)[4]) {
#ifdef ACE_I8_PROBE_NO_LDS
    for (int R = 0; R < 4; ++R) af[R] = i4v{R, 1, 2, 3};
#else
#pragma unroll
    for (int R = 0; R < 4; ++R) af[R] = *reinterpret_cast<const i4v*>(arow + 32 * R * rstride);
#endif
}
__device__ __forceinline__ void kstep(const i4v (&af)[4], i4v b0, i4v b1, i16v (&acc)[4][2]) {
#pragma unroll
    for (int R = 0; R < 4; ++R) {
        acc[R][0] = __builtin_amdgcn_mfma_i32_32x32x32_i8(af[R], b0, acc[R][0], 0, 0, 0);
        acc[R][1] = __builtin_amdgcn_mfma_i32_32x32x32_i8(af[R], b1, acc[R][1], 0, 0, 0);
    }
}

constexpr int SK = 2;
struct BSet {
    i4v f[SK][2];
};
__device__ __forceinline__ void bload(BSet& b, const i4v* bp0, const i4v* bp1, int ks0, int kmax) {
#pragma unroll
    for (int kk = 0; kk < SK; ++kk) {
        const long long ks = min(ks0 + kk, kmax);
        b.f[kk][0] = bp0[ks * 64];
        b.f[kk][1] = bp1[ks * 64];
    }
}
__device__ __forceinline__ void stage_mma(const int8_t* arow, int rstride, const BSet& b, i16v (&acc)[4][2]) {
    i4v a0[4], a1[4];
    aload(arow, rstride, a0);
    aload(arow + 32, rstride, a1);
    kstep(a0, b.f[0][0], b.f[0][1], acc);
    kstep(a1, b.f[1][0], b.f[1][1], acc);
}
constexpr int SKR = SK * 32;
constexpr int RSA = SKR + 16;
template <bool TOL>
__device__ __forceinline__ void i8a_block(int nb, int Kc, int Mc, int nks, const i4v* __restrict__ Bf,
                                          const double* __restrict__ Zp, const double* __restrict__ Np,
                                          const double* __restrict__ Yp, const double* __restrict__ Mp,
                                          double* __restrict__ Tp, int ldt, const double* __restrict__ cptr,
                                          const RealState* __restrict__ rs, const double* __restrict__ zeros,
                                          const double* __restrict__ AXp, int8_t (*As)[ROWS * RSA], double* sc_s,
                                          double* imu_s, int* live_s, const int* avok_s, int j0, int cb, int rc = 1) {
    const int t = threadIdx.x, lane = t & 63, w = t >> 6;
    const int bl = t >> 5, cq = t & 31, jb = j0 + bl;
    const RealState* rj = rs + (jb < nb ? jb / rc : 0);
    const bool live = jb < nb && !rj->done;
    const double imu = live ? 1.0 / rj->mu : 0.0;
    const d2* z = reinterpret_cast<const d2*>(Zp) + (long long)(live ? jb : 0) * Kc;
    const d2* nn = (live && rj->nzero) ? reinterpret_cast<const d2*>(zeros)
                                       : reinterpret_cast<const d2*>(Np) + (long long)(live ? jb : 0) * Kc;
    double p2, sc;
    plane_scale(live ? rj->vbound : 0.0, *cptr, p2, sc);
    if (cq == 0) {
        sc_s[bl] = sc;
        imu_s[bl] = imu;
        live_s[bl] = live;
    }
    const int nstage = nks / SK, kmax = nks - 1;
    struct Raw {
        d2 z, n;
    };
    auto gload = [&](int s, Raw& r) {
        const int k = min(32 * s + cq, Kc - 1);
        r.z = z[k];
        r.n = nn[k];
    };
    auto lstore = [&](const Raw& r, int s, int buf) {
        const bool in = live && 32 * s + cq < Kc;
        const double v[2] = {in ? fma(-r.n.x, imu, r.z.x) : 0.0, in ? fma(-r.n.y, imu, r.z.y) : 0.0};
        uint32_t lo[2];
        int32_t hi[2];
#pragma unroll
        for (int i = 0; i < 2; ++i) {
            const double x = rint(v[i] * p2);
            const double h = floor(x * 0x1p-32);
            hi[i] = (int32_t)h;
            lo[i] = (uint32_t)fma(-h, 0x1p32, x);
        }
#pragma unroll
        for (int tt = 0; tt < 8; ++tt) {
            uint32_t d[2];
#pragma unroll
            for (int i = 0; i < 2; ++i) {
                if (tt < 4) d[i] = (lo[i] >> (7 * tt)) & 127u;
                else if (tt == 4) d[i] = __builtin_amdgcn_alignbit((uint32_t)hi[i], lo[i], 28) & 127u;
                else if (tt == 5) d[i] = ((uint32_t)hi[i] >> 3) & 127u;
                else if (tt == 6) d[i] = ((uint32_t)hi[i] >> 10) & 127u;
                else d[i] = (uint32_t)(hi[i] >> 17) & 255u;
            }
            *reinterpret_cast<uint16_t*>(&As[buf][lds_row(bl, tt) * RSA + 2 * cq]) = (uint16_t)(d[0] | (d[1] << 8));
        }
    };

    const int ct0 = cb * (NCB / 32) + 2 * w;
    const i4v* bp0 = Bf + (long long)ct0 * nks * 64 + lane;
    const i4v* bp1 = bp0 + (long long)nks * 64;

    i16v acc[4][2];
#pragma unroll
    for (int R = 0; R < 4; ++R) acc[R][0] = acc[R][1] = i16v{};

    Raw r0, r1;
    BSet bA, bB;
    bload(bA, bp0, bp1, 0, kmax);
    gload(0, r0);
    gload(1, r1);
    lstore(r0, 0, 0);
    __syncthreads();
    const int8_t* arow0 = &As[0][(lane & 31) * RSA + 16 * (lane >> 5)];
    const int8_t* arow1 = arow0 + ROWS * RSA;
    for (int s = 0; s < nstage; s += 2) {
        bload(bB, bp0, bp1, (s + 1) * SK, kmax);
        gload(min(s + 2, nstage - 1), r0);
        __builtin_amdgcn_sched_barrier(0);
        stage_mma(arow0, RSA, bA, acc);
        __builtin_amdgcn_sched_barrier(0);
        lstore(r1, s + 1, 1);
        __syncthreads();
        bload(bA, bp0, bp1, (s + 2) * SK, kmax);
        gload(min(s + 3, nstage - 1), r1);
        __builtin_amdgcn_sched_barrier(0);
        stage_mma(arow1, RSA, bB, acc);
        __builtin_amdgcn_sched_barrier(0);
        lstore(r0, s + 2, 0);
        __syncthreads();
    }

    const int h = lane >> 5, ldo = 2 * Mc;
#pragma unroll
    for (int R = 0; R < 4; ++R)
#pragma unroll
        for (int q = 0; q < 2; ++q) {
            const int blo = 4 * R + 2 * q + h, j = j0 + blo;
            if (j >= nb || !live_s[blo]) continue;
            const double scb = sc_s[blo], im = imu_s[blo];
#pragma unroll
            for (int c = 0; c < 2; ++c) {
                const int col = (ct0 + c) * 32 + (lane & 31);
                if (col >= ldo) continue;
                const long long off = (long long)j * ldo + col;
                const double av = avok_s[blo] ? AXp[off] : scb * recombine(acc[R][c], q);
                const double tv = fma(-Mp[off], im, Yp[off]) - av;
                if (TOL) Tp[blo * ldt + col] = tv;
                else Tp[off] = tv;
            }
        }
}

__global__ __launch_bounds__(NT, 1) void i8a_kernel(int nb, int Kc, int Mc, int nks, const i4v* __restrict__ Bf,
                                                    const double* __restrict__ Zp, const double* __restrict__ Np,
                                                    const double* __restrict__ Yp, const double* __restrict__ Mp,
                                                    double* __restrict__ Tp, const double* __restrict__ cptr,
                                                    const RealState* __restrict__ rs, const double* __restrict__ zeros,
                                                    const double* __restrict__ AXp, int rc) {
    __shared__ __attribute__((aligned(16))) int8_t As[2][ROWS * RSA];
    __shared__ double sc_s[RB], imu_s[RB];
    __shared__ int live_s[RB], avok_s[RB];
    const int t = threadIdx.x, j0 = blockIdx.x * RB;
    if (t < RB) {
        const int j = j0 + t;
        avok_s[t] = AXp && j < nb && !rs[j].done && rs[j].avok;
    }
    __syncthreads();
    i8a_block<false>(nb, Kc, Mc, nks, Bf, Zp, Np, Yp, Mp, Tp, 0, cptr, rs, zeros, AXp, As, sc_s, imu_s, live_s, avok_s,
                     j0, blockIdx.y, rc);
}

struct FuseState {
    int el, keep_cur, optsrc;
};
template <bool KY, bool FUSE, bool GLDS>
__device__ __forceinline__ void i8ah_body(int nb, int Kc, int Mc, int nks, const i4v* __restrict__ Bf,
                                          const double* __restrict__ Gp, double* __restrict__ Wp,
                                          const double* __restrict__ cptr, const RealState* __restrict__ rs,
                                          const ZArgs& za, int8_t* Ad, double* zsum, const d2* gl, int gst) {
    __shared__ double sc_s[RB], imu_s[RB];
    __shared__ int live_s[RB];
    __shared__ FuseState fs_s[FUSE ? RB : 1];
    __shared__ int z0_s[(!FUSE && !KY) ? RB : 1];
    __shared__ int nz_s[(!FUSE && !KY) ? RB : 1];
    const int rst = 32 * nks + 16;

    const int t = threadIdx.x, lane = t & 63, w = t >> 6;
    const int j0 = blockIdx.x * RB;
    const int bl = t >> 5, cp = t & 31, jb = j0 + bl;
    STAMP_DECL;
    STAMP(0);
    const bool matz = !FUSE && !KY && za.matz;
    const int rc = (!FUSE && za.r > 1) ? za.r : 1;
    const bool live = jb < nb && (matz ? rs[jb].optsrc == 3
                                       : (!rs[jb / rc].done && !(za.msp && rs[jb / rc].mzit == za.it)));
    if (!__syncthreads_or(live)) return;
    const int zn_id = 1 + (za.it & 1);
    if constexpr (!FUSE && !KY) {
        if (matz && t < RB) z0_s[t] = j0 + t < nb ? rs[j0 + t].z0id : 0;
    }
    if constexpr (FUSE) {
        if (t < RB) {
            const int j = j0 + t;
            FuseState f{};
            if (j < nb && !rs[j].done && !(za.msp && rs[j].mzit == za.it)) {
                const RealState& r = rs[j];
                f.el = r.kfok && r.nzero;
                const bool improved_pre = sqrt(r.obj2) < r.opt_obj;
                f.keep_cur = !improved_pre && !(r.opt_obj < INFINITY);
                f.optsrc = r.optsrc;
            }
            fs_s[t] = f;
        }
    }
    const d2* g = reinterpret_cast<const d2*>(Gp) + (long long)jb * Kc;

    constexpr int GR = 4;
    const int nst = nks / 4;
    d2 gv[GR][2];
    double mx = 0.0, sn = 0.0;
    auto gat = [&](int s, int u) -> d2 {
        const int k = 64 * s + 2 * cp + u;
        if constexpr (GLDS) return (live && k < Kc) ? gl[bl * gst + k] : make_double2(0.0, 0.0);
        return (live && k < Kc) ? g[k] : make_double2(0.0, 0.0);
    };
#pragma unroll
    for (int s = 0; s < GR; ++s)
#pragma unroll
        for (int u = 0; u < 2; ++u) gv[s][u] = s < nst ? gat(s, u) : make_double2(0.0, 0.0);
    auto acc_max = [&](d2 v) {
        const double ax = fabs(v.x), ay = fabs(v.y);
        mx = fmax(mx, fmax(ax, ay));
        sn += 0.0 * (ax + ay);
    };
#pragma unroll
    for (int s = 0; s < GR; ++s) {
        acc_max(gv[s][0]);
        acc_max(gv[s][1]);
    }
    for (int s = GR; s < nst; ++s) {
        acc_max(gat(s, 0));
        acc_max(gat(s, 1));
    }
#pragma unroll
    for (int o = 1; o < 32; o <<= 1) {
        mx = fmax(mx, __shfl_xor(mx, o, 64));
        sn += __shfl_xor(sn, o, 64);
    }
    double p2, sc;
    plane_scale(mx + sn, *cptr, p2, sc);
    if (cp == 0) {
        sc_s[bl] = sc;
        live_s[bl] = live;
        imu_s[bl] = (!KY && !FUSE && za.xzn && live) ? 1.0 / rs[jb / rc].mu : 0.0;
        if constexpr (!FUSE && !KY) nz_s[bl] = za.xzn && live && rc > 1 && rs[jb / rc].nzero;
    }
    for (int s = 0; s < nst; ++s) {
        d2 x0, x1;
        if (s < GR) {
#pragma unroll
            for (int q = 0; q < GR; ++q)
                if (q == s) {
                    x0 = gv[q][0];
                    x1 = gv[q][1];
                }
        } else {
            x0 = gat(s, 0);
            x1 = gat(s, 1);
        }
        const double v[4] = {x0.x, x0.y, x1.x, x1.y};
        uint32_t d[8];
        digits4(v, p2, d);
#pragma unroll
        for (int tt = 0; tt < 8; ++tt) *reinterpret_cast<uint32_t*>(&Ad[lds_row(bl, tt) * rst + KC * s + 4 * cp]) = d[tt];
    }
    __syncthreads();
    STAMP(1);
    if constexpr (FUSE) {
        for (int r = 0; r < RB; ++r)
            if (fs_s[r].el && fs_s[r].optsrc == zn_id) {
                const long long o = (long long)(j0 + r) * 2 * Mc;
                for (int i = t; i < 2 * Mc; i += NT) za.optX[o + i] = za.Zn[o + i];
                __syncthreads();
                if (t == 0) za.st[j0 + r].optsrc = 0;
            }
    }

    const int h = lane >> 5, ldo = 2 * Mc, ocb = KY ? NCB / 2 : NCB, ncb = (ldo + ocb - 1) / ocb;
    const int8_t* arow = &Ad[(lane & 31) * rst + 16 * (lane >> 5)];
    const int total = ncb * nks;
    auto bfl = [&](BSet& b, int f0) {
#pragma unroll
        for (int kk = 0; kk < SK; ++kk) {
            const int f = min(f0 + kk, total - 1), cb = f / nks, ks = f - cb * nks;
            const i4v* p = Bf + ((long long)(cb * (NCB / 32) + 2 * w) * nks + ks) * 64 + lane;
            b.f[kk][0] = p[0];
            b.f[kk][1] = p[(long long)nks * 64];
        }
    };
    auto zload = [&](int cbk, double (&zv)[4][2][2]) {
        const int ct0 = cbk * (NCB / 32) + 2 * w;
#pragma unroll
        for (int R = 0; R < 4; ++R)
#pragma unroll
            for (int q = 0; q < 2; ++q) {
                const int blo = 4 * R + 2 * q + (lane >> 5), j = min(j0 + blo, nb - 1);
#pragma unroll
                for (int c = 0; c < 2; ++c) {
                    const int col = min((ct0 + c) * 32 + (lane & 31), 2 * Mc - 1);
                    zv[R][q][c] = fs_s[blo].el ? za.Z[(long long)j * 2 * Mc + col] : 0.0;
                }
            }
    };
    auto epilogue = [&](int cbk, i16v (&acc)[4][2], const double (&zv)[4][2][2]) {
        if constexpr (KY) {
            const int col = (cbk * (NCB / 64) + w) * 32 + (lane & 31);
#pragma unroll
            for (int R = 0; R < 4; ++R)
#pragma unroll
                for (int q = 0; q < 2; ++q) {
                    const int blo = 4 * R + 2 * q + h, j = j0 + blo;
                    if (j >= nb || !live_s[blo] || col >= ldo) continue;
                    i16v cmb;
#pragma unroll
                    for (int e = 0; e < 16; ++e) cmb[e] = acc[R][0][e] + 128 * acc[R][1][e];
                    Wp[(long long)j * ldo + col] = sc_s[blo] * recombine(cmb, q);
                }
#pragma unroll
            for (int R = 0; R < 4; ++R) acc[R][0] = acc[R][1] = i16v{};
            return;
        }
        const int ct0 = cbk * (NCB / 32) + 2 * w;
        if constexpr (FUSE) {
#pragma unroll
            for (int R = 0; R < 4; ++R)
#pragma unroll
                for (int q = 0; q < 2; ++q) {
                    const int blo = 4 * R + 2 * q + h, j = j0 + blo;
                    const bool el = fs_s[blo].el, kc = fs_s[blo].keep_cur;
                    double p0 = 0.0, p3 = 0.0;
                    if (j < nb && live_s[blo]) {
                        const double scb = sc_s[blo];
#pragma unroll
                        for (int c = 0; c < 2; ++c) {
                            const int col = (ct0 + c) * 32 + (lane & 31);
                            if (col >= ldo) continue;
                            const long long off = (long long)j * ldo + col;
                            const double wv = scb * recombine(acc[R][c], q);
                            if (el) {
                                const double x = zv[R][q][c] + wv, d = x - zv[R][q][c];
                                za.Zn[off] = x;
                                if (kc) za.Xcur[off] = x;
                                p0 += x * x;
                                p3 += d * d;
                            } else {
                                Wp[off] = wv;
                            }
                        }
                    }
                    if (el) {
                        double* zs = zsum + ((w * 8 + 2 * R + q) * 2) * 64 + lane;
                        zs[0] = cbk == 0 ? p0 : zs[0] + p0;
                        zs[64] = cbk == 0 ? p3 : zs[64] + p3;
                    }
                }
        } else {
#pragma unroll
        for (int R = 0; R < 4; ++R)
#pragma unroll
            for (int q = 0; q < 2; ++q) {
                const int blo = 4 * R + 2 * q + h, j = j0 + blo;
                if (j >= nb || !live_s[blo]) continue;
                const double scb = sc_s[blo];
#pragma unroll
                for (int c = 0; c < 2; ++c) {
                    const int col = (ct0 + c) * 32 + (lane & 31);
                    if (col >= ldo) continue;
                    const long long off = (long long)j * ldo + col;
                    const double wv = scb * recombine(acc[R][c], q);
                    if (matz) Wp[off] = (z0_s[blo] == 1 ? za.Z : za.Zn)[off] + wv;
                    else if (za.xzn) {
                        const double* nrow = nz_s[blo] ? za.zeros : za.N + (long long)j * ldo;
                        Wp[off] = fma(-nrow[col], imu_s[blo], za.Z[off]) + wv;
                    }
                    else Wp[off] = wv;
                }
            }
        }
#pragma unroll
        for (int R = 0; R < 4; ++R) acc[R][0] = acc[R][1] = i16v{};
    };
    i16v acc[4][2];
#pragma unroll
    for (int R = 0; R < 4; ++R) acc[R][0] = acc[R][1] = i16v{};
    BSet bA, bB;
    bfl(bA, 0);
    if constexpr (FUSE) {
        double zv[4][2][2];
        const int per = nks / (2 * SK);
        for (int cbk = 0; cbk < ncb; ++cbk) {
            const int f0 = cbk * nks;
            for (int i = 0; i < per - 1; ++i) {
                const int f = f0 + 2 * SK * i;
                bfl(bB, f + SK);
                __builtin_amdgcn_sched_barrier(0);
                stage_mma(arow + 32 * (f % nks), rst, bA, acc);
                __builtin_amdgcn_sched_barrier(0);
                bfl(bA, f + 2 * SK);
                __builtin_amdgcn_sched_barrier(0);
                stage_mma(arow + 32 * ((f + SK) % nks), rst, bB, acc);
                __builtin_amdgcn_sched_barrier(0);
            }
            const int f = f0 + 2 * SK * (per - 1);
            bfl(bB, f + SK);
            zload(cbk, zv);
            __builtin_amdgcn_sched_barrier(0);
            stage_mma(arow + 32 * (f % nks), rst, bA, acc);
            __builtin_amdgcn_sched_barrier(0);
            bfl(bA, f + 2 * SK);
            __builtin_amdgcn_sched_barrier(0);
            stage_mma(arow + 32 * ((f + SK) % nks), rst, bB, acc);
            __builtin_amdgcn_sched_barrier(0);
            epilogue(cbk, acc, zv);
        }
    } else {
        const double zv0[4][2][2] = {};
        for (int f = 0; f < total; f += 2 * SK) {
            bfl(bB, f + SK);
            __builtin_amdgcn_sched_barrier(0);
            stage_mma(arow + 32 * (f % nks), rst, bA, acc);
            __builtin_amdgcn_sched_barrier(0);
            bfl(bA, f + 2 * SK);
            __builtin_amdgcn_sched_barrier(0);
            stage_mma(arow + 32 * ((f + SK) % nks), rst, bB, acc);
            __builtin_amdgcn_sched_barrier(0);
            if ((f + 2 * SK) % nks == 0) epilogue(f / nks, acc, zv0);
        }
    }
    STAMP(2);
    if (!KY && !FUSE) STAMP_PRINT("i8ah prologue|sweep:", 3);
    if constexpr (!FUSE && !KY) {
        if (matz && (t & 31) == 0 && live) za.st[jb].optsrc = 0;
    }
    if constexpr (FUSE) {
        __syncthreads();
        {
            const int blo = t >> 5, sub = t & 31, R = blo >> 2, q = (blo >> 1) & 1, hh = blo & 1;
            double s0 = 0.0, s3 = 0.0;
            if (fs_s[blo].el && live_s[blo])
                for (int ww = 0; ww < 8; ++ww) {
                    const double* zs = zsum + ((ww * 8 + 2 * R + q) * 2) * 64 + 32 * hh + sub;
                    s0 += zs[0];
                    s3 += zs[64];
                }
#pragma unroll
            for (int o = 1; o < 32; o <<= 1) {
                s0 += __shfl_xor(s0, o, 64);
                s3 += __shfl_xor(s3, o, 64);
            }
            if (sub == 0 && fs_s[blo].el && live_s[blo]) {
                RealState* st = za.st + j0 + blo;
                st->fs0 = s0;
                st->fs3 = s3;
                st->fzit = za.it;
            }
        }
        STAMP(3);
        STAMP_PRINT("i8ah-fused prologue|sweep|post:", 4);
    }
}
template <bool KY, bool FUSE>
__global__ __launch_bounds__(NT, 1) void i8ah_kernel(int nb, int Kc, int Mc, int nks, const i4v* __restrict__ Bf,
                                                     const double* __restrict__ Gp, double* __restrict__ Wp,
                                                     const double* __restrict__ cptr,
                                                     const RealState* __restrict__ rs, ZArgs za) {
    extern __shared__ __attribute__((aligned(16))) int8_t Ad[];
    double* zsum = reinterpret_cast<double*>(Ad + ((ROWS * (32 * nks + 16) + 255) & ~255));
    i8ah_body<KY, FUSE, false>(nb, Kc, Mc, nks, Bf, Gp, Wp, cptr, rs, za, Ad, zsum, nullptr, 0);
}

__device__ __forceinline__ long long frag_off(int col, int k, int nks) {
    return ((long long)((col >> 5) * nks + (k >> 5)) * 64 + (col & 31) + 32 * ((k & 31) >> 4)) * 16 + (k & 15);
}
__global__ __launch_bounds__(256) void i8_expand_kernel(int m, int n, const double* __restrict__ Ap,
                                                         const double* __restrict__ cmax, int8_t* __restrict__ LA,
                                                         int nksA, int8_t* __restrict__ LH, int nksH, int* flag) {
    const long long e = blockIdx.x * 256LL + threadIdx.x;
    if (e >= (long long)m * n) return;
    const int i = (int)(e / n), k = (int)(e % n);
    const d2 a = reinterpret_cast<const d2*>(Ap)[e];
    const double c = *cmax;
    auto code = [&](double x, int& ok) -> int {
        if (x == c) return 1;
        if (x == -c) return -1;
        if (x == 0.0) return 0;
        ok = 0;
        return 0;
    };
    int ok = 1;
    const int p = code(a.x, ok), q = code(a.y, ok);
    if (!ok) atomicOr(flag, 1);
    LA[frag_off(2 * i, 2 * k, nksA)] = (int8_t)p;
    LA[frag_off(2 * i, 2 * k + 1, nksA)] = (int8_t)(-q);
    LA[frag_off(2 * i + 1, 2 * k, nksA)] = (int8_t)q;
    LA[frag_off(2 * i + 1, 2 * k + 1, nksA)] = (int8_t)p;
    LH[frag_off(2 * k, 2 * i, nksH)] = (int8_t)p;
    LH[frag_off(2 * k, 2 * i + 1, nksH)] = (int8_t)q;
    LH[frag_off(2 * k + 1, 2 * i, nksH)] = (int8_t)(-q);
    LH[frag_off(2 * k + 1, 2 * i + 1, nksH)] = (int8_t)p;
}
#ifndef ACE_GSK
#define ACE_GSK 4
#endif
constexpr int GSK = ACE_GSK;
constexpr int GRB = 16;
__host__ __device__ __forceinline__ int gyk_mp(int m) { return (m + 31) & ~31; }

__device__ __forceinline__ void ystep_elem(double e1, double e2, double e3, double mu, d2 mii, d2 yo, double Bi,
                                           d2& gv, d2& ax, d2& mn, d2& y, double (&v)[9]) {
#pragma clang fp contract(off)
    gv = comb3m(e1, e2, e3);
    const double imu = 1.0 / mu;
    const double pr = mii.x * imu, pi = mii.y * imu;
    ax = make_double2((yo.x - pr) - gv.x, (yo.y - pi) - gv.y);
    double cr = ax.x + pr, ci = ax.y + pi;
    double d = sqrt(cr * cr + ci * ci);
    if (d == 0.0) {
        cr = 1.0;
        ci = 0.0;
        d = 1.0;
    }
    const double f = (Bi / d + mu) / (1.0 + mu);
    y = make_double2(cr * f, ci * f);
    const double jr = ax.x - y.x, ji = ax.y - y.y;
    mn = make_double2(mii.x + jr * mu, mii.y + ji * mu);
    const double aax = sqrt(ax.x * ax.x + ax.y * ax.y) - Bi;
    v[0] += aax * aax;
    v[1] += ax.x * ax.x + ax.y * ax.y;
    v[2] += y.x * y.x + y.y * y.y;
    v[3] += jr * jr + ji * ji;
    const double dr = y.x - yo.x, di = y.y - yo.y;
    v[4] += dr * dr + di * di;
    const double ay = fmax(fabs(y.x), fabs(y.y));
    v[5] = fmax(v[5], ay);
    v[6] += 0.0 * (fabs(y.x) + fabs(y.y));
}
__device__ __forceinline__ void msp_sums_elem(d2 yo, d2 mii, double imu, d2 tv, d2 gv, double (&v)[9]) {
#pragma clang fp contract(off)
    const double ar = (yo.x - mii.x * imu) - tv.x, ai = (yo.y - mii.y * imu) - tv.y;
    v[7] += ar * gv.x + ai * gv.y;
    v[8] += gv.x * (tv.x - gv.x) + gv.y * (tv.y - gv.y);
}

template <bool GLDS>
__device__ __forceinline__ void gyk_body(int nb, int m, const GykArgs& a, unsigned char* smem, const ZArgs& za,
                                         int za_ctl) {
    __shared__ double red[8][GRB][9];
    __shared__ double sc_s[GRB], p2_s[GRB];
    __shared__ int live_s[GRB], imp_s[GRB], avok_s[GRB], oys_s[GRB], pend_s[GRB], msp_s[GRB], ent_s[GRB], oss_s[GRB];
    __shared__ double imu0_s[GRB], mu_s[GRB];
    const int mp = gyk_mp(m), tst = mp + 1;
    d2* Ts = reinterpret_cast<d2*>(smem);
    int8_t* Ad = reinterpret_cast<int8_t*>(smem) + ((GRB * tst * 16 + 255) & ~255);
    const int t = threadIdx.x, lane = t & 63, w = t >> 6, j0 = blockIdx.x * GRB;
    STAMP_DECL;
    STAMP(0);
    constexpr int TU = 8;
    d2 tyv[TU], tmv[TU], txv[TU];
    const bool early = a.LA && a.AX;
    if (early) {
#pragma unroll
        for (int u = 0; u < TU; ++u) {
            const int idx = min(t + NT * u, GRB * mp - 1), jl = idx / mp, k = min(idx - jl * mp, m - 1);
            const long long o = (long long)min(j0 + jl, nb - 1) * m + k;
            tyv[u] = reinterpret_cast<const d2*>(a.Yo)[o];
            tmv[u] = reinterpret_cast<const d2*>(a.M)[o];
            txv[u] = reinterpret_cast<const d2*>(a.AX)[o];
        }
    }
    if (t < GRB) {
        const int j = j0 + t;
        const bool lv = j < nb && !a.rs[j].done;
        live_s[t] = lv;
        avok_s[t] = lv && a.AX && a.rs[j].avok;
        mu_s[t] = lv ? a.rs[j].mu : 1.0;
        imu0_s[t] = lv ? 1.0 / mu_s[t] : 0.0;
        oys_s[t] = lv ? a.rs[j].optysrc : 0;
        pend_s[t] = lv && a.lazy && a.rs[j].dpend;
        int ms = 0, en = 0;
        if (GLDS && a.msp && lv && a.it >= 2) {
            const RealState& r = a.rs[j];
            ms = r.msp || (avok_s[t] && r.kfok && r.nzero && r.opt_obj < INFINITY && r.fzit == a.it - 1);
            en = ms && !r.msp;
        }
        msp_s[t] = ms;
        ent_s[t] = en;
        oss_s[t] = lv ? a.rs[j].optsrc : 0;
    }
    __syncthreads();
    auto t_from = [&](const d2 (&yv)[TU], const d2 (&mv)[TU], const d2 (&xv)[TU]) {
#pragma unroll
        for (int u = 0; u < TU; ++u) {
            const int idx = t + NT * u;
            if (idx >= GRB * mp) continue;
            const int jl = idx / mp, k = idx - jl * mp;
            d2 v = make_double2(0.0, 0.0);
            if (live_s[jl] && avok_s[jl] && k < m) {
                const double im = imu0_s[jl];
                v = make_double2(fma(-mv[u].x, im, yv[u].x) - xv[u].x, fma(-mv[u].y, im, yv[u].y) - xv[u].y);
            }
            Ts[jl * tst + k] = v;
        }
    };
    if (early) t_from(tyv, tmv, txv);
    const int nksK = i8_nks_dev(m), rst = 32 * nksK + 16;
    if (a.lazy && __syncthreads_or(t < GRB && pend_s[t])) {
        const int bl = t >> 5, cp = t & 31, h = lane >> 5, ldo = 2 * m, ocb = NCB / 2, ncb = (ldo + ocb - 1) / ocb;
        const int8_t* arow = &Ad[(lane & 31) * rst + 16 * (lane >> 5)];
        const i4v* Bf = reinterpret_cast<const i4v*>(a.LK);
        const int total = ncb * nksK;
        const double* Ysd = reinterpret_cast<const double*>(Ts);
        for (int pass = 0; pass < 2; ++pass) {
            double mx = 0.0, sn = 0.0;
            for (int i = cp; i < mp; i += 32) {
                d2 v = make_double2(0.0, 0.0);
                if (pend_s[bl] && i < m) {
                    const long long o = (long long)(j0 + bl) * m + i;
                    const d2 yk = reinterpret_cast<const d2*>(a.Yo)[o];
                    v = pass ? csub(yk, reinterpret_cast<const d2*>(a.Yn)[o]) : yk;
                }
                Ts[bl * tst + i] = v;
                mx = fmax(mx, fmax(fabs(v.x), fabs(v.y)));
                sn += 0.0 * (fabs(v.x) + fabs(v.y));
            }
#pragma unroll
            for (int o = 1; o < 32; o <<= 1) {
                mx = fmax(mx, __shfl_xor(mx, o, 64));
                sn += __shfl_xor(sn, o, 64);
            }
            double p2, sc;
            plane_scale(mx + sn, a.c8[1], p2, sc);
            if (cp == 0) sc_s[bl] = sc;
            __syncthreads();
            for (int s = 0; s < nksK / KSC; ++s) {
                d2 x[2];
#pragma unroll
                for (int u = 0; u < 2; ++u) {
                    const int k = 64 * s + 2 * cp + u;
                    x[u] = k < m ? Ts[bl * tst + k] : make_double2(0.0, 0.0);
                }
                const double v[4] = {x[0].x, x[0].y, x[1].x, x[1].y};
                uint32_t d[8];
                digits4(v, p2, d);
#pragma unroll
                for (int tt = 0; tt < 8; ++tt)
                    *reinterpret_cast<uint32_t*>(&Ad[lds_row(bl, tt) * rst + KC * s + 4 * cp]) = d[tt];
            }
            __syncthreads();
            auto bfl = [&](BSet& bs, int f0) {
#pragma unroll
                for (int kk = 0; kk < SK; ++kk) {
                    const int f = min(f0 + kk, total - 1), cb = f / nksK, ks = f - cb * nksK;
                    const i4v* pp = Bf + ((long long)(cb * (NCB / 32) + 2 * w) * nksK + ks) * 64 + lane;
                    bs.f[kk][0] = pp[0];
                    bs.f[kk][1] = pp[(long long)nksK * 64];
                }
            };
            double pacc[4][2];
#pragma unroll
            for (int R = 0; R < 4; ++R) pacc[R][0] = pacc[R][1] = 0.0;
            i16v acc[4][2];
#pragma unroll
            for (int R = 0; R < 4; ++R) acc[R][0] = acc[R][1] = i16v{};
            BSet bA, bB;
            bfl(bA, 0);
            for (int f = 0; f < total; f += 2 * SK) {
                bfl(bB, f + SK);
                __builtin_amdgcn_sched_barrier(0);
                stage_mma(arow + 32 * (f % nksK), rst, bA, acc);
                __builtin_amdgcn_sched_barrier(0);
                bfl(bA, f + 2 * SK);
                __builtin_amdgcn_sched_barrier(0);
                stage_mma(arow + 32 * ((f + SK) % nksK), rst, bB, acc);
                __builtin_amdgcn_sched_barrier(0);
                if ((f + 2 * SK) % nksK == 0) {
                    const int col = ((f / nksK) * (NCB / 64) + w) * 32 + (lane & 31);
#pragma unroll
                    for (int R = 0; R < 4; ++R)
#pragma unroll
                        for (int q = 0; q < 2; ++q) {
                            const int blo = 4 * R + 2 * q + h;
                            if (pend_s[blo] && col < ldo) {
                                i16v cmb;
#pragma unroll
                                for (int e = 0; e < 16; ++e) cmb[e] = acc[R][0][e] + 128 * acc[R][1][e];
                                pacc[R][q] += Ysd[2 * blo * tst + col] * (sc_s[blo] * recombine(cmb, q));
                            }
                        }
#pragma unroll
                    for (int R = 0; R < 4; ++R) acc[R][0] = acc[R][1] = i16v{};
                }
            }
#pragma unroll
            for (int R = 0; R < 4; ++R)
#pragma unroll
                for (int q = 0; q < 2; ++q) {
#pragma unroll
                    for (int o = 1; o < 32; o <<= 1) pacc[R][q] += __shfl_xor(pacc[R][q], o, 64);
                    if ((lane & 31) == 0) red[w][4 * R + 2 * q + h][pass] = pacc[R][q];
                }
            __syncthreads();
        }
        if (t < GRB && pend_s[t]) {
            double nv = 0.0, dv = 0.0;
            for (int q = 0; q < 8; ++q) {
                nv += red[q][t][0];
                dv += red[q][t][1];
            }
            RealState* rs = a.rs + j0 + t;
            if (dual_finish(a.dc, rs, dv, nv)) live_s[t] = 0;
            mu_s[t] = rs->mu;
            imu0_s[t] = 1.0 / mu_s[t];
        }
        __syncthreads();
        if (early) {
#pragma unroll
            for (int u = 0; u < TU; ++u) {
                const int idx = min(t + NT * u, GRB * mp - 1), jl = idx / mp, k = min(idx - jl * mp, m - 1);
                const long long o = (long long)min(j0 + jl, nb - 1) * m + k;
                tyv[u] = reinterpret_cast<const d2*>(a.Yo)[o];
                tmv[u] = reinterpret_cast<const d2*>(a.M)[o];
                txv[u] = reinterpret_cast<const d2*>(a.AX)[o];
            }
            t_from(tyv, tmv, txv);
        }
    }
    if (a.yn_id)
        for (int r = 0; r < GRB; ++r)
            if (oys_s[r] == a.yn_id)
                for (int i = t; i < m; i += NT)
                    reinterpret_cast<d2*>(a.optY)[(long long)(j0 + r) * m + i] =
                        reinterpret_cast<const d2*>(a.Yn)[(long long)(j0 + r) * m + i];
    int need = 0;
    if (a.LA && t < GRB) need = live_s[t] && !avok_s[t];
    if (__syncthreads_or(need)) {
        for (int idx = t; idx < GRB * tst; idx += NT) Ts[idx] = make_double2(0.0, 0.0);
        __syncthreads();
        i8a_block<true>(nb, a.n, m, i8_nks_dev(a.n), reinterpret_cast<const i4v*>(a.LA), a.Z, a.N, a.Yo, a.M,
                        reinterpret_cast<double*>(Ts), 2 * tst, a.c8, a.rs, a.zeros, a.AX,
                        reinterpret_cast<int8_t(*)[ROWS * RSA]>(Ad), sc_s, p2_s, live_s, avok_s, j0, 0);
    } else if (early) {
    } else
    for (int idx = t; idx < GRB * mp; idx += NT) {
        const int jl = idx / mp, k = idx - jl * mp, j = j0 + jl;
        d2 v = make_double2(0.0, 0.0);
        if (live_s[jl] && k < m) {
            const long long o = (long long)j * m + k;
            if (avok_s[jl]) {
                const d2 y = reinterpret_cast<const d2*>(a.Yo)[o], mm = reinterpret_cast<const d2*>(a.M)[o],
                         ax = reinterpret_cast<const d2*>(a.AX)[o];
                const double im = imu0_s[jl];
                v = make_double2(fma(-mm.x, im, y.x) - ax.x, fma(-mm.y, im, y.y) - ax.y);
            } else {
                v = reinterpret_cast<const d2*>(a.T)[o];
            }
        }
        Ts[jl * tst + k] = v;
    }
    __syncthreads();
    STAMP(1);

    const int nct = mp / 16, nks = mp / 4;
    const d2* const gp[2] = {reinterpret_cast<const d2*>(a.Gf) + (long long)min(2 * w, nct - 1) * 64 + lane,
                             reinterpret_cast<const d2*>(a.Gf) + (long long)min(2 * w + 1, nct - 1) * 64 + lane};
    d4v p1[2], p2[2], p3[2];
    frag_mv<2, GSK>(gp, Ts, tst, nct, nks, lane, p1, p2, p3);
    d2 mi[2][4], yov[2][4], sov[2][4];
    double biv[2][4], muv[4];
    const bool mspl = GLDS && a.msp;
#pragma unroll
    for (int r = 0; r < 4; ++r) {
        const int jl = (lane >> 4) + 4 * r;
        muv[r] = mu_s[jl];
#pragma unroll
        for (int c = 0; c < 2; ++c) {
            const int i = min(16 * (2 * w + c) + (lane & 15), m - 1);
            const long long off = (long long)(live_s[jl] ? j0 + jl : j0) * m + i;
            mi[c][r] = reinterpret_cast<const d2*>(a.M)[off];
            yov[c][r] = reinterpret_cast<const d2*>(a.Yo)[off];
            biv[c][r] = a.B[off];
            sov[c][r] = mspl ? reinterpret_cast<const d2*>(a.Sold)[off] : make_double2(0.0, 0.0);
        }
    }
    __syncthreads();
    STAMP(2);
#ifdef ACE_GYK_PROBE_ONLY_A
    {
        double sacc = 0.0;
        for (int c = 0; c < 2; ++c)
            for (int r = 0; r < 4; ++r) sacc += p1[c][r] + p2[c][r] + p3[c][r];
        if (sacc == 12345.678) a.g[0] = sacc;
    }
    return;
#endif

    double v7[4][9];
#pragma unroll
    for (int r = 0; r < 4; ++r)
#pragma unroll
        for (int k = 0; k < 9; ++k) v7[r][k] = 0.0;
#pragma unroll
    for (int c = 0; c < 2; ++c) {
        const int ct = 2 * w + c;
#pragma unroll
        for (int r = 0; r < 4; ++r) {
            const int jl = (lane >> 4) + 4 * r, j = j0 + jl, i = 16 * ct + (lane & 15);
            if (ct >= nct || i >= m || !live_s[jl]) continue;
            const long long off = (long long)j * m + i;
            const double mu = muv[r];
            const d2 mii = mi[c][r], yo = yov[c][r];
            d2 gv, ax, mn, y;
            ystep_elem(p1[c][r], p2[c][r], p3[c][r], mu, mii, yo, biv[c][r], gv, ax, mn, y, v7[r]);
            if constexpr (!GLDS) reinterpret_cast<d2*>(a.g)[off] = gv;
            if (a.AX) reinterpret_cast<d2*>(a.AX)[off] = ax;
            reinterpret_cast<d2*>(a.M)[off] = mn;
            reinterpret_cast<d2*>(a.Yn)[off] = y;
            if constexpr (GLDS) {
                if (msp_s[jl]) {
                    msp_sums_elem(yo, mii, 1.0 / mu, Ts[jl * tst + i], gv, v7[r]);
                    const d2 so = ent_s[jl] ? make_double2(0.0, 0.0) : sov[c][r];
                    d2* sn = reinterpret_cast<d2*>(a.Snew) + off;
                    if (oss_s[jl] == 4 + (a.it & 1)) reinterpret_cast<d2*>(a.optS)[off] = *sn;
                    *sn = cadd(so, gv);
                }
                Ts[jl * tst + i] = gv;
            } else {
                Ts[jl * tst + i] = y;
            }
        }
    }
#ifdef ACE_GYK_PROBE_P1
    return;
#endif
#pragma unroll
    for (int r = 0; r < 4; ++r) {
#pragma unroll
        for (int k = 0; k < 5; ++k) v7[r][k] = bsum16(v7[r][k]);
        v7[r][5] = bmax16(v7[r][5]);
        v7[r][6] = bsum16(v7[r][6]);
        if (GLDS && a.msp) {
            v7[r][7] = bsum16(v7[r][7]);
            v7[r][8] = bsum16(v7[r][8]);
        }
        if ((lane & 15) == 0)
#pragma unroll
            for (int k = 0; k < 9; ++k) red[w][(lane >> 4) + 4 * r][k] = v7[r][k];
    }
    __syncthreads();
    STAMP(3);
    if (t < GRB) {
        double v[9] = {0, 0, 0, 0, 0, 0, 0, 0, 0};
        for (int q = 0; q < 8; ++q) {
#pragma unroll
            for (int k = 0; k < 5; ++k) v[k] += red[q][t][k];
            v[5] = fmax(v[5], red[q][t][5]);
            v[6] += red[q][t][6];
            v[7] += red[q][t][7];
            v[8] += red[q][t][8];
        }
        int imp = 0;
        double p2 = 1.0, sc = 0.0;
        if (live_s[t]) {
            RealState& rs = a.rs[j0 + t];
            rs.obj2 = v[0];
            rs.nAX2 = v[1];
            rs.nY2 = v[2];
            rs.nJM2 = v[3];
            rs.dY2 = v[4];
            imp = sqrt(v[0]) < rs.opt_obj;
            plane_scale(v[5] + v[6], a.c8[1], p2, sc);
            if (a.yn_id)
                rs.optysrc = imp ? a.yn_id : (oys_s[t] == a.yn_id ? 0 : oys_s[t]);
            if (msp_s[t]) {
                const double s0 = rs.fs0 + 2.0 * v[7] + v[8];
                const double s3 = v[8];
                bool take = !ent_s[t];
                if (!take) {
                    const bool r1 = a.rank_one && a.rank_one[j0 + t];
                    const int np = r1 ? 1 : a.np;
                    const double cum = rs.kfcum + a.room * sqrt(s3);
                    take = s0 > 0.0;
                    for (int p = 0; p < 4 && p < np; ++p) {
                        const double fl = r1 ? 0.95 : a.fl[p], lb = rs.kf[p] * (1.0 - 1e-12) - cum;
                        take = take && lb > 0.0 && lb * lb > fl * s0 * (1.0 + 1e-9);
                    }
                }
                if (take) {
                    atomicAdd(a.dc.done_count + 1, 1);
                    rs.fs0 = s0;
                    rs.fs3 = s3;
                    rs.fzit = a.it;
                    rs.mzit = a.it;
                    if (ent_s[t]) {
// ... 335 lines not shown
                    v[6] += red[q][t][6];
                    v[7] += red[q][t][7];
                    v[8] += red[q][t][8];
                }
                RealState& rs = rsl[t];
                rs.obj2 = v[0];
                rs.nAX2 = v[1];
                rs.nY2 = v[2];
                rs.nJM2 = v[3];
                rs.dY2 = v[4];
                const bool imp = sqrt(v[0]) < rs.opt_obj;
                rs.fs0 = rs.fs0 + 2.0 * v[7] + v[8];
                rs.fs3 = v[8];
                rs.fzit = it;
                rs.mzit = it;
                ++cnt;
                const int ok = fused_control<false>(za, &rs, z_profile(za, j0 + t), it);
                if (pbY && !imp) fl |= 1;
                if (pbS && !imp) fl |= 2;
                pbY = imp;
                pbS = imp && (ok & 1);
                if (pbY) fl |= 64;
                if (pbS) {
                    fl |= 128;
                    rs.optsrc = 3;
                }
                if (!(ok & 1)) fl |= 8;
                if (ok & 2) fl |= 16;
                fl |= rs.done ? 4 : 32;
                mylive = !rs.done;
                mu_s[t] = rs.mu;
            }
            flg_s[t] = fl;
        }
        __syncthreads();
        MSR_STAMP(4);
        int any = 0;
#pragma unroll
        for (int q = 0; q < GRB; ++q) {
            const int f = flg_s[q];
            any |= f;
        }
        const bool alive = any & 32;
        const bool stop = (any & 24) || it + 1 >= a.it_end || !alive;
        if (t < GRB) {
            const int f = flg_s[t];
            vw += (f & 1) + ((f >> 1) & 1);
            if (f & (4 | 32) && (stop || (f & 4))) vw += 6 + ((f >> 6) & 1) + ((f >> 7) & 1);
        }
#pragma unroll
        for (int r = 0; r < 4; ++r) {
            if (!lv[r]) continue;
            const int f = flg_s[(lane >> 4) + 4 * r];
            const bool wb = stop || (f & 4);
            const int jl = (lane >> 4) + 4 * r;
#pragma unroll
            for (int c = 0; c < TPW; ++c) {
                const int i = 16 * (TPW * w + c) + (lane & 15);
                const long long o = (long long)(j0 + jl) * m + i;
                d2* ssl = &Ss[(4 * c + r) * NTW + t];
                if (f & 1) reinterpret_cast<d2*>(a.optY)[o] = yv[c][r];
                if (f & 2) reinterpret_cast<d2*>(a.optS)[o] = *ssl;
                if (wb && (f & 64)) reinterpret_cast<d2*>(a.optY)[o] = yn[c][r];
                if (wb && (f & 128)) reinterpret_cast<d2*>(a.optS)[o] = sn[c][r];
                if (wb) {
                    reinterpret_cast<d2*>(a.Y[it & 1])[o] = yn[c][r];
                    reinterpret_cast<d2*>(a.Y[(it + 1) & 1])[o] = yv[c][r];
                    reinterpret_cast<d2*>(a.M)[o] = mv[c][r];
                    reinterpret_cast<d2*>(a.AX)[o] = Ts[jl * tst + i];
                    reinterpret_cast<d2*>(a.S[it & 1])[o] = sn[c][r];
                    reinterpret_cast<d2*>(a.S[(it + 1) & 1])[o] = *ssl;
                }
                *ssl = sn[c][r];
                yv[c][r] = yn[c][r];
            }
            if (f & 4) lv[r] = false;
        }
        MSR_STAMP(5);
        if (stop) {
#ifdef ACE_MSR_STAMPS
            if (blockIdx.x == 5 && t == 0)
                printf("msr it %d..%d: T %llu GT %llu bar %llu Ystep %llu ctl %llu wb %llu (x10ns)\n", a.it0, it,
                       ph[0], ph[1], ph[2], ph[3], ph[4], ph[5]);
#endif
            const int rp = (any & 8) ? it : it + 1;
            if (t < GRB && cnt) {
                atomicAdd(a.mspcount, cnt);
                atomicAdd(a.steps, cnt);
            }
            if (t < GRB && vw && a.vecw) atomicAdd(a.vecw, vw);
            if (t < GRB && live_s[t]) {
                if (mylive) rsl[t].mres = rp;
                a.rs[j0 + t] = rsl[t];
            }
            if (t == 0 && alive) atomicMin(a.resume, rp);
            if (t == 0 && (any & 24)) atomicAdd(a.steps + ((any & 8) ? 2 : 3), 1);
            return;
        }
    }
}

__global__ __launch_bounds__(256) void gyk_gfrag_kernel(int m, const double* __restrict__ Gp, double* __restrict__ Gf) {
    const int mp = gyk_mp(m), nct = mp / 16;
    const long long e = blockIdx.x * 256LL + threadIdx.x;
    if (e >= (long long)mp * mp) return;
    const int lane = (int)(e & 63);
    const long long q = e >> 6;
    const int ct = (int)(q % nct), ks = (int)(q / nct);
    const int i = 16 * ct + (lane & 15), k = 4 * ks + (lane >> 4);
    const d2 v = (i < m && k < m) ? reinterpret_cast<const d2*>(Gp)[(long long)i * m + k] : make_double2(0.0, 0.0);
    reinterpret_cast<d2*>(Gf)[e] = v;
}

__global__ __launch_bounds__(256) void i8k_expand_kernel(int m, const double* __restrict__ Kp,
                                                          const double* __restrict__ cmax, int8_t* __restrict__ LK,
                                                          int nks, int* flag) {
    const long long e = blockIdx.x * 256LL + threadIdx.x;
    if (e >= (long long)m * m) return;
    const int i = (int)(e / m), k = (int)(e % m);
    const d2 kv = reinterpret_cast<const d2*>(Kp)[e];
    const double c2 = cmax[1];
    const double kr = rint(kv.x / c2), ki = rint(kv.y / c2);
    if (fabs(kr) > 8192.0 || fabs(ki) > 8192.0) atomicOr(flag, 2);
    auto put = [&](int oc, int kk, double v) {
        const int iv = (int)v, hi = iv >> 7, lo = iv & 127;
        const int t = oc >> 5, cc = oc & 31;
        LK[frag_off(32 * (2 * t) + cc, kk, nks)] = (int8_t)lo;
        LK[frag_off(32 * (2 * t + 1) + cc, kk, nks)] = (int8_t)hi;
    };
    put(2 * i, 2 * k, kr);
    put(2 * i, 2 * k + 1, -ki);
    put(2 * i + 1, 2 * k, ki);
    put(2 * i + 1, 2 * k + 1, kr);
}
}
size_t msr_request_bytes() { return msr_lds_bytes(); }

int i8_nks(int kc) { return (2 * kc + KC - 1) / KC * KSC; }
int i8_ncols(int mc) { return (2 * mc + NCB - 1) / NCB * NCB; }
size_t i8_frag_bytes(int mc, int kc) { return (size_t)i8_ncols(mc) * i8_nks(kc) * 32; }

void launch_i8_expand(int m, int n, const double* A, const double* cmax, int8_t* LA, int8_t* LH, int* flag,
                      hipStream_t st) {
    const long long tot = (long long)m * n;
    hipLaunchKernelGGL(i8_expand_kernel, dim3((unsigned)((tot + 255) / 256)), dim3(256), 0, st, m, n, A, cmax, LA,
                       i8_nks(n), LH, i8_nks(m), flag);
}

size_t i8ah_lds_bytes(int kc) { return ((size_t)ROWS * (32 * i8_nks(kc) + 16) + 255) & ~(size_t)255; }
size_t i8ah_fuse_lds_bytes() { return (size_t)8 * 8 * 2 * 64 * sizeof(double); }

void launch_i8_apply_A(int nb, int n, int m, const int8_t* LA, const double* Z, const double* N, const double* Y,
                       const double* M, double* T, const double* cmax, const RealState* rs, const double* zeros,
                       const double* AX, hipStream_t st, int rcols) {
    dim3 grid((nb + RB - 1) / RB, i8_ncols(m) / NCB, 1), block(NT);
    hipLaunchKernelGGL(i8a_kernel, grid, block, 0, st, nb, n, m, i8_nks(n), reinterpret_cast<const i4v*>(LA), Z, N,
                       Y, M, T, cmax, rs, zeros, AX, rcols < 1 ? 1 : rcols);
}
size_t i8k_frag_bytes(int m) { return (size_t)2 * ((2 * m + NCB / 2 - 1) / (NCB / 2)) * (NCB / 2) * i8_nks(m) * 32; }
void launch_i8k_expand(int m, const double* K, const double* cmax, int8_t* LK, int* flag, hipStream_t st) {
    const long long tot = (long long)m * m;
    hipLaunchKernelGGL(i8k_expand_kernel, dim3((unsigned)((tot + 255) / 256)), dim3(256), 0, st, m, K, cmax, LK,
                       i8_nks(m), flag);
}
void launch_i8_apply_K(int nb, int m, const int8_t* LK, const double* Y, double* KY, const double* cmax,
                       const RealState* rs, hipStream_t st, int rcols) {
    const size_t lds = i8ah_lds_bytes(m);
    if (!lds_fits(reinterpret_cast<const void*>(&i8ah_kernel<true, false>), "i8ah_kernel<KY>", lds)) return;
    dim3 grid((nb + RB - 1) / RB, 1, 1), block(NT);
    ZArgs za{};
    za.r = rcols;
    hipLaunchKernelGGL((i8ah_kernel<true, false>), grid, block, lds, st, nb, m, m, i8_nks(m),
                       reinterpret_cast<const i4v*>(LK), Y, KY, cmax + 1, rs, za);
}
size_t gyk_gfrag_bytes(int m) { return (size_t)gyk_mp(m) * gyk_mp(m) * 16; }
size_t gyk_lds_bytes(int m) {
    return (((size_t)GRB * (gyk_mp(m) + 1) * 16 + 255) & ~(size_t)255) +
           (i8ah_lds_bytes(m) > (size_t)2 * ROWS * RSA ? i8ah_lds_bytes(m) : (size_t)2 * ROWS * RSA);
}
void launch_gyk_gfrag(int m, const double* G, double* Gf, hipStream_t st) {
    const long long tot = (long long)gyk_mp(m) * gyk_mp(m);
    hipLaunchKernelGGL(gyk_gfrag_kernel, dim3((unsigned)((tot + 255) / 256)), dim3(256), 0, st, m, G, Gf);
}
void launch_gyk(int nb, int m, const GykArgs& a, hipStream_t st) {
    const size_t lds = gyk_lds_bytes(m);
    if (!lds_fits(reinterpret_cast<const void*>(&gyk_kernel), "gyk_kernel", lds)) return;
    hipLaunchKernelGGL(gyk_kernel, dim3((nb + GRB - 1) / GRB), dim3(NT), lds, st, nb, m, a);
}
size_t gyf_lds_bytes(int m) {
    const size_t ts = gyf_ts_bytes(m), ad = gyk_lds_bytes(m) - ts, zs = i8ah_fuse_lds_bytes();
    return ts + ad + (ts >= zs ? 0 : zs);
}
void launch_gyf(int nb, int m, int n, const GykArgs& a, const int8_t* LAH, double* W, const ZArgs& za, int ctl,
                hipStream_t st) {
    const size_t lds = gyf_lds_bytes(m);
    if (!lds_fits(reinterpret_cast<const void*>(&gyf_kernel), "gyf_kernel", lds)) return;
    const size_t ad = gyk_lds_bytes(m) - gyf_ts_bytes(m);
    hipLaunchKernelGGL(gyf_kernel, dim3((nb + GRB - 1) / GRB), dim3(NT), lds, st, nb, m, n, a,
                       reinterpret_cast<const i4v*>(LAH), W, za, ad, ctl);
}
__global__ __launch_bounds__(256) void msr_ready_kernel(int nb, const RealState* __restrict__ rs, int it, int* notready) {
    const int j = blockIdx.x * 256 + threadIdx.x;
    int bad = 0, nm = 0, np = 0;
    if (j < nb && !rs[j].done) {
        const RealState& r = rs[j];
        bad = !r.msp || r.dpend || r.mzit < it - 1 || r.zit < it - 1;
        nm = !r.msp;
        np = r.dpend;
    }
    bad = __syncthreads_count(bad);
    nm = __syncthreads_count(nm);
    np = __syncthreads_count(np);
    if (threadIdx.x == 0 && bad) {
        atomicAdd(notready, bad);
        atomicAdd(notready + 1, nm);
        atomicAdd(notready + 2, np);
    }
}
bool msr_supported(int m) { return m == 256; }
void launch_msr_ready(int nb, const RealState* rs, int it, int* notready, hipStream_t st) {
    hipLaunchKernelGGL(msr_ready_kernel, dim3((nb + 255) / 256), dim3(256), 0, st, nb, rs, it, notready);
}
void launch_msr(const MsrArgs& a, const ZArgs& za, int waves, hipStream_t st) {
    const size_t lds = msr_lds_bytes();
    if (waves == 8) {
        if (!lds_fits(reinterpret_cast<const void*>(&msr_kernel<2>), "msr_kernel<2>", lds)) return;
        hipLaunchKernelGGL(msr_kernel<2>, dim3((a.nb + GRB - 1) / GRB), dim3(512), lds, st, a, za);
    } else {
        if (!lds_fits(reinterpret_cast<const void*>(&msr_kernel<4>), "msr_kernel<4>", lds)) return;
        hipLaunchKernelGGL(msr_kernel<4>, dim3((a.nb + GRB - 1) / GRB), dim3(256), lds, st, a, za);
    }
}
__global__ __launch_bounds__(256) void msp_opt_gather_kernel(int m, RealState* rs, const double* S0, const double* S1,
                                                             double* optS) {
    const int b = blockIdx.x, os = rs[b].optsrc;
    if (os != 4 && os != 5) return;
    const d2* src = reinterpret_cast<const d2*>(os == 4 ? S0 : S1) + (long long)b * m;
    d2* dst = reinterpret_cast<d2*>(optS) + (long long)b * m;
    for (int i = threadIdx.x; i < m; i += 256) dst[i] = src[i];
    if (threadIdx.x == 0) rs[b].optsrc = 3;
}
void launch_i8_msp_optx(int nb, int m, int n, const int8_t* LAH, const double* optS, double* optX, const double* cmax,
                        RealState* rs, const double* Zb1, const double* Zb2, const double* S0, const double* S1,
                        hipStream_t st) {
    hipLaunchKernelGGL(msp_opt_gather_kernel, dim3(nb), dim3(256), 0, st, m, rs, S0, S1, const_cast<double*>(optS));
    ZArgs za{};
    za.matz = 1;
    za.st = rs;
    za.Z = const_cast<double*>(Zb1);
    za.Zn = const_cast<double*>(Zb2);
    launch_i8_apply_AH(nb, m, n, LAH, optS, optX, cmax, rs, st, nullptr, &za);
}
void launch_i8_apply_AH(int nb, int m, int n, const int8_t* LAH, const double* g, double* W, const double* cmax,
                        const RealState* rs, hipStream_t st, const ZArgs* fuse, const ZArgs* plain) {
    dim3 grid((nb + RB - 1) / RB, 1, 1), block(NT);
    if (fuse) {
        const size_t lds = i8ah_lds_bytes(m) + i8ah_fuse_lds_bytes();
        if (!lds_fits(reinterpret_cast<const void*>(&i8ah_kernel<false, true>), "i8ah_kernel<FUSE>", lds)) return;
        hipLaunchKernelGGL((i8ah_kernel<false, true>), grid, block, lds, st, nb, m, n, i8_nks(m),
                           reinterpret_cast<const i4v*>(LAH), g, W, cmax, rs, *fuse);
    } else {
        const size_t lds = i8ah_lds_bytes(m);
        if (!lds_fits(reinterpret_cast<const void*>(&i8ah_kernel<false, false>), "i8ah_kernel", lds)) return;
        hipLaunchKernelGGL((i8ah_kernel<false, false>), grid, block, lds, st, nb, m, n, i8_nks(m),
                           reinterpret_cast<const i4v*>(LAH), g, W, cmax, rs, plain ? *plain : ZArgs{});
    }
}
size_t i8ah_budget(int kind) {
    const void* k = kind == 1 ? reinterpret_cast<const void*>(&i8ah_kernel<false, true>)
                  : kind == 2 ? reinterpret_cast<const void*>(&i8ah_kernel<true, false>)
                              : reinterpret_cast<const void*>(&i8ah_kernel<false, false>);
    return lds_dyn_budget(k);
}
size_t gyk_budget() { return lds_dyn_budget(reinterpret_cast<const void*>(&gyk_kernel)); }
size_t gyf_budget() { return lds_dyn_budget(reinterpret_cast<const void*>(&gyf_kernel)); }

}
```

include/ace.h:

```cpp
#ifndef ACE_H_
#define ACE_H_

#include <stddef.h>
#include <stdint.h>

#ifdef __cplusplus
extern "C" {
#endif

#define ACE_OK 0
#define ACE_ERR_ARG -1
#define ACE_ERR_UNSUPPORTED -2
#define ACE_ERR_HIP -3
#define ACE_ERR_WORKSPACE -4

#define ACE_VARIANT_A2ONLY 0
#define ACE_VARIANT_NUCLEAR 1

#define ACE_ST_CONVERGED 1u
#define ACE_ST_NO_OPT 2u
#define ACE_ST_EIG_NOCONV 4u
#define ACE_ST_ROLLBACK 8u
#define ACE_ST_RANK_ONE 128u

// ... 124 lines not shown
enum {
    ACE_STAGE_INIT_R = 0, ACE_STAGE_YSTEP_R, ACE_STAGE_FINALIZE_R, ACE_STAGE_GRAM_ROTATE, ACE_STAGE_QUALITY,
    ACE_STAGE_PART_QUALITY, ACE_STAGE_KEEP_BEST, ACE_STAGE_FINISH, ACE_STAGE_PART_GEINV, ACE_STAGE_PART_GFIX,
    ACE_STAGE_PART_EXPAND, ACE_STAGE_PART_COMPACT, ACE_STAGE_ANORM, ACE_STAGE_BNORM, ACE_STAGE_GATHER_ROWS,
    ACE_STAGE_GATHER_B, ACE_STAGE_MOVE_ROWS, ACE_STAGE_MOVE_BYTES, ACE_STAGE_PUT_COL, ACE_STAGE_FLAG_BITS,
    ACE_STAGE_FILL, ACE_STAGE_NOPS
};
#define ACE_SG_NSTATE 9
#define ACE_SG_NFLAG 6
typedef struct ace_stage_args {
    int32_t op, row_mode, batch, n, m, r, nc, mt;
    int32_t count, ld, col, first, scatter, isentinel;
    uint32_t or_mask, bit;
    int64_t len;
    double mu0, tol_abs, value, sentinel;
    const double *X, *Y, *P0, *B, *S, *g, *M, *A, *G, *geinv;
    const double *q, *qmax, *Xmax, *Ymax, *anorm, *bnorm, *optX, *optY, *Zb1, *Zb2, *Yb1, *Yb2, *src;
    const double* state;
    const int32_t* flags;
    const int32_t *rows, *idx, *isrc, *idst;
    const unsigned char *mask, *bsrc;
    double *Xo, *Yo, *Mo, *No, *qo, *state_out;
    int32_t *iout, *flags_out;
    unsigned char* bout;
} ace_stage_args;
int ace_stage_host(const ace_stage_args* args);

#define ACE_DRIVER_A2ONLY 0
#define ACE_DRIVER_A2NUCLEAR 1
#define ACE_DRIVER_MULTIRES 2
#define ACE_DRIVER_PHASELIFT 3
int ace_recover_driver(int driver, int tx, int rx, int P, const double* cb_amp, const double* cb_angle,
                       const double* rss_dbm, int seed_id, int n_M, const int32_t* M_list,
                       double* H_amp, double* H_angle);
int ace_recover_driver_ex(int driver, int tx, int rx, int P, const double* cb_amp, const double* cb_angle,
                          const double* rss_dbm, int seed_id, int n_M, const int32_t* M_list, int maxiter,
                          double* H_amp, double* H_angle);
int ace_driver_m_sweep(int tx, int rx, int32_t* M_out);
int ace_driver_randperm(uint64_t seed, uint64_t stream, int P, int k, int32_t* out);

#define ACE_ST_BF_NONFINITE 16u
#define ACE_ST_BF_NOCONV 32u
#define ACE_ST_BF_DC 64u
int ace_svd_beamformer_batch(int batch, int tx, int rx, const double* H, const double* offset,
                             uint8_t* wr_code, uint8_t* wt_code, int32_t* beam_idx, double* rss,
                             uint32_t* status, double* vh_r, double* vh_t, void* stream);
int ace_svd_beamformer_host(int batch, int tx, int rx, const double* H, const double* offset,
                            uint8_t* wr_code, uint8_t* wt_code, int32_t* beam_idx, double* rss,
                            uint32_t* status, double* vh_r, double* vh_t);

#define ACE_ST_EVAL_DEGENERATE 256u
int ace_evaluate_batch(int batch, int tx, int rx, const double* X, const double* G,
                       double* metrics, uint32_t* status, void* stream);
int ace_evaluate_host(int batch, int tx, int rx, const double* X, const double* G,
                      double* metrics, uint32_t* status);

#define ACE_ST_RSS_SKIPPED 512u
int ace_rss_evaluate_batch(int batch, int n, int Pt, const double* X, const double* CB, const double* rss,
                           int rss_shared, double* metrics, double* pred, uint32_t* status, void* stream);
int ace_rss_evaluate_host(int batch, int n, int Pt, const double* X, const double* CB, const double* rss,
                          int rss_shared, double* metrics, double* pred,
                          uint32_t* status);

int ace_beam_scan_batch(int batch, int d0, int d1, int Q0, int Q1, const double* X, const double* W0,
                        const double* F1, const double* noise, int K, double* top_pow, int32_t* top_idx,
                        double* total, double* power, uint32_t* status, void* stream);
int ace_beam_scan_host(int batch, int d0, int d1, int Q0, int Q1, const double* X, const double* W0,
                       const double* F1, const double* noise, int K, double* top_pow, int32_t* top_idx,
                       double* total, double* power, uint32_t* status);

#define ACE_ST_OMP_DEPENDENT 1024u
size_t ace_omp_workspace_size(int batch, int d, int N, int kmax);
int ace_omp_solve_batch(int batch, int d, int N, int kmax, double tol, const double* D, const double* colscale,
                        const double* Y, int32_t* idx, double* coef, int32_t* count, double* resnorm,
                        uint32_t* status, double* x, void* workspace, size_t workspace_bytes, void* stream);
int ace_omp_solve_host(int batch, int d, int N, int kmax, double tol, const double* D, const double* colscale,
                       const double* Y, int32_t* idx, double* coef, int32_t* count, double* resnorm,
                       uint32_t* status, double* x);

#define ACE_ST_GAMP_NANBREAK 2048u
#define ACE_ST_GAMP_MAXEM 4096u
#define ACE_ST_GAMP_FAILED 8192u
typedef struct ace_gamp_cfg {
    double snr_db;
    double lambda0;
    int learn_lambda;
    int max_em_iter;
    int gamp_nit;
    int reserved;
    double step0;
    double gamp_tol;
} ace_gamp_cfg;
void ace_gamp_cfg_default(ace_gamp_cfg* cfg);
size_t ace_gamp_workspace_size(int batch, int d, int N);
int ace_gamp_solve_batch(const ace_gamp_cfg* cfg, int batch, int d, int N, const double* D, const double* Y,
                         double* xhat, double* xvar, double* params, int32_t* em_iters, int32_t* trace,
                         uint32_t* status, void* workspace, size_t workspace_bytes, void* stream);
int ace_gamp_solve_host(const ace_gamp_cfg* cfg, int batch, int d, int N, const double* D, const double* Y,
                        double* xhat, double* xvar, double* params, int32_t* em_iters, int32_t* trace,
                        uint32_t* status);

typedef struct ace_minl2_cfg {
    int r;
    int maxiter;
    int train_seed;
    int reserved;
    double mu0;
    double rho;
    double cc_frac;
    double tol_rel;
    double tol_abs;
} ace_minl2_cfg;
void ace_minl2_cfg_default(ace_minl2_cfg* cfg);
size_t ace_minl2_workspace_size(int batch, int m, int n, int r);
int ace_minl2_admm_batch(const ace_minl2_cfg* cfg, int batch, int m, int n, int r, int scale_by_row, const double* A,
                         const double* B, const double* X0, const int32_t* rcols, double* X, double* Y, double* Xall,
                         int32_t* iters, int32_t* objcol, double* opt_obj, double* mu, uint32_t* status,
                         void* workspace, size_t workspace_bytes, void* stream);
int ace_minl2_admm_host(const ace_minl2_cfg* cfg, int batch, int m, int n, int r, int scale_by_row, const double* A,
                        const double* B, const double* X0, const int32_t* rcols, double* X, double* Y, double* Xall,
                        int32_t* iters, int32_t* objcol, double* opt_obj, double* mu,
                        uint32_t* status);
size_t ace_minl2_solve_workspace_size(const ace_minl2_cfg* cfg, int batch, int m, int n);
int ace_minl2_solve_batch(const ace_minl2_cfg* cfg, int batch, int m, int n, const double* A, const double* B,
                          const int32_t* train_idx_host, double* X, double* Y, double* quality, int32_t* stage_iters,
                          int32_t* r_used, uint32_t* status, void* workspace, size_t workspace_bytes, void* stream);
int ace_minl2_solve_host(const ace_minl2_cfg* cfg, int batch, int m, int n, const double* A, const double* B,
                         const int32_t* train_idx, double* X, double* Y, double* quality, int32_t* stage_iters,
                         int32_t* r_used, uint32_t* status);

int ace_nuclear_prox_batch(int batch, int n, int r, const double* E, double tau, double* Z, void* stream);

int ace_synth_codebook(uint64_t seed, int64_t first, int count, int m, int n, double* A, void* stream);
int ace_synth_channels(uint64_t seed, int64_t first, int count, int m, int tx, int rx, int L,
                       double snr_db, double x0_noise, const double* A, int a_shared,
                       double* vecH, double* B, double* X0, void* stream);

#define ACE_K_SETUP 0
#define ACE_K_INIT 1
#define ACE_K_PRE 2
#define ACE_K_APPLY_A 3
#define ACE_K_APPLY_G 4
#define ACE_K_YSTEP 5
#define ACE_K_APPLY_K 6
#define ACE_K_APPLY_AH 7
#define ACE_K_ZSTEP 8
#define ACE_K_FINAL 9
#define ACE_K_MSR 10
#define ACE_NKCLASS 11
int ace_prof_start(int max_launches);
int ace_prof_sample(int stride, uint32_t full_mask);
int ace_prof_stop(double* total_ms, int32_t* launches);
int ace_prof_msp_steps(long long* steps);
int ace_prof_work(double* flops);
int ace_prof_work_ex(double* flops, double* bytes, double* int8_ops);

int ace_path_counts(int64_t* counts, int reset);

int ace_lds_request(const char* kernel, int m, size_t* bytes);

const char* ace_last_error(void);

const char* ace_version(void);

#ifdef __cplusplus
}
#endif
#endif
```

Before: 201,200.

## Skip int8 MFMA row-tiles for converged batch elements in apply_A/AH kernels

Each workgroup votes a mask of which 32-row tiles still hold live, unconverged problems, then dispatches a templated sweep that loads A fragments and issues MFMAs only for those tiles. Tiles whose AX slot can be reused are also marked, so Z/N loads read zeros instead of the real inputs. The goal is to drop int8 GEMM work and LDS traffic for batch entries that have already converged in late ADMM iterations. In exchange it adds a workgroup OR-reduction, four template instantiations (more code size and register pressure), and atomic skip counters for profiling.

Measured after the change: 203,100, median of 6. No clear change (+1.0%).

```diff
diff --git a/2ace-mmwave-channel-estimation_amd/ace_amd/_lib.py b/2ace-mmwave-channel-estimation_amd/ace_amd/_lib.py
--- a/2ace-mmwave-channel-estimation_amd/ace_amd/_lib.py
+++ b/2ace-mmwave-channel-estimation_amd/ace_amd/_lib.py
@@ -165,6 +165,9 @@
     lib.ace_prof_stop.restype = C.c_int
     lib.ace_prof_msp_steps.argtypes = [C.POINTER(C.c_longlong)]
     lib.ace_prof_msp_steps.restype = C.c_int
+    if hasattr(lib, "ace_prof_tile_skips"):
+        lib.ace_prof_tile_skips.argtypes = [C.POINTER(C.c_longlong)]
+        lib.ace_prof_tile_skips.restype = C.c_int
     lib.ace_prof_work.argtypes = [dp]
     lib.ace_prof_work.restype = C.c_int
     lib.ace_prof_work_ex.argtypes = [dp, dp, dp]
diff --git a/2ace-mmwave-channel-estimation_amd/csrc/ace_admm.cpp b/2ace-mmwave-channel-estimation_amd/csrc/ace_admm.cpp
--- a/2ace-mmwave-channel-estimation_amd/csrc/ace_admm.cpp
+++ b/2ace-mmwave-channel-estimation_amd/csrc/ace_admm.cpp
@@ -52,6 +52,7 @@
     bool tk_trace = false;
     bool msr = true;
     bool fuse = true, gyf = true, mspace = true, lazy_dual = true, lean = true, nuc_msp = true, i8r = true, zcert = true;
+    bool tiles = true, tile_trace = false;
     bool r1lz = true;
     double msp_room = 32.0;
 };
@@ -80,6 +81,8 @@
     k.msr = on("ACE_MSR");
     k.zcert = on("ACE_ZCERT");
     k.r1lz = on("ACE_R1_LANCZOS");
+    k.tiles = on("ACE_I8_TILES");
+    k.tile_trace = num("ACE_TILE_TRACE", 0) != 0;
     k.tkeig = (int)num("ACE_TK_EIG", 6);
     k.tk_trace = num("ACE_TK_TRACE", 0) != 0;
     k.msr_start = (int)num("ACE_MSR_START", 56);
@@ -100,6 +103,17 @@
 }
 static bool gyf_ok(const Knobs& k, int m) { return k.gyf && lds_ok_budget(gyf_budget(), gyf_lds_bytes(m)); }
 
+static int tile_report(const Knobs& kn, const AdmmState& w, hipStream_t st) {
+    if (g_prof.on && g_prof.tile_used < g_prof.msp_cap)
+        ACE_HIP(hipMemcpyAsync(g_prof.tile_slots + g_prof.tile_used++, w.done + I8_SKIP_SLOT, sizeof(int),
+                               hipMemcpyDeviceToHost, st));
+    if (kn.tile_trace) {
+        int c[2] = {0, 0};
+        ACE_HIP(read_back(c, w.done + I8_SKIP_SLOT, sizeof(c), st));
+        fprintf(stderr, "[ace] row-tile sweeps skipped %d, A V blocks with reused-AX slots %d\n", c[0], c[1]);
+    }
+    return ACE_OK;
+}
 static bool i8_disabled() {
     static const bool v = [] {
         const char* e = getenv("ACE_NO_I8");
@@ -502,11 +516,12 @@
             za.Snew = wh.Sg[it & 1];
             za.optS = wh.optS;
             za.msp_fail_it = kn.msp_fail_it;
+            za.tiles = kn.tiles ? 1 : 0;
             const bool gyf = za.xfuse && za0.lazy_dual && gyf_ok(kn, m);
             GykArgs ga{L.Gf, wh.T, Bh, wh.Y[q], wh.M, wh.Y[1 - q], wh.g, wh.KY[q], wh.KY[1 - q], wh.optY,
                        L.LK8, L.c8, wh.st, wh.AX, 2 - q, L.LA8, Zc, Nc, w.zeros, n, za0.lazy_dual, dc, gyf ? 1 : 0,
                        gyf && msp ? 1 : 0, it, za.Sold, wh.Sg[it & 1], wh.optS, za0.np,
-                       {za0.fl[0], za0.fl[1], za0.fl[2], za0.fl[3]}, za.rank_one, kn.msp_room};
+                       {za0.fl[0], za0.fl[1], za0.fl[2], za0.fl[3]}, za.rank_one, kn.msp_room, kn.tiles ? 1 : 0};
             if (!(pmask & 1)) {
             } else if (gyf) {
                 ProfScope ps(ACE_K_APPLY_G, sh);
@@ -556,6 +571,7 @@
         if (msp && g_prof.on && g_prof.msp_used < g_prof.msp_cap)
             ACE_HIP(hipMemcpyAsync(g_prof.msp_slots + g_prof.msp_used++, w.done + 1, sizeof(int),
                                    hipMemcpyDeviceToHost, st));
+        ACE_TRY(tile_report(kn, w, st));
         launch_finalize_r(n, m, 1, 1, batch, w.optX, w.optY, w.V, w.Y[q], Xo, Yo, iters, status, mu_out, w.st, st, w.Z,
                           w.Z2, w.Y[0], w.Y[1]);
     }
@@ -697,6 +713,7 @@
     za.r1lz = kn.r1lz ? 1 : 0;
     za.tkeig = kn.tkeig > 0 ? kn.tkeig : 0;
     za.tkcnt = w.done + 32;
+    za.tiles = kn.tiles ? 1 : 0;
     za.wmode = 0;
     za.Xcur = w.V;
     za.Zn = nullptr;
@@ -749,7 +766,8 @@
         } else if (gyk) {
         } else if (i8) {
             ProfScope ps(ACE_K_APPLY_A, st);
-            launch_i8_apply_A(batch, n, m, L.LA8, Zc, Nc, w.Y[q], w.M, w.T, L.c8, w.st, w.zeros, gyk ? w.AX : nullptr, st);
+            launch_i8_apply_A(batch, n, m, L.LA8, Zc, Nc, w.Y[q], w.M, w.T, L.c8, w.st, w.zeros, gyk ? w.AX : nullptr, st, 1,
+                              kn.tiles ? 1 : 0, w.done);
             ACE_LAUNCHED("apply_A (i8a_kernel)");
         } else if (fused) {
             ProfScope ps(ACE_K_APPLY_A, st, lv * (fl_mn));
@@ -761,7 +779,8 @@
             }
             if (i8r) {
                 ProfScope ps(ACE_K_APPLY_A, st, 0.0, lv * (vb * (2.0 * n + 3.0 * m)), lv * (op_mn));
-                launch_i8_apply_A(nv, n, m, L.LA8, w.Z, w.N, w.Y[q], w.M, w.T, L.c8, w.st, w.zeros, nullptr, st, r);
+                launch_i8_apply_A(nv, n, m, L.LA8, w.Z, w.N, w.Y[q], w.M, w.T, L.c8, w.st, w.zeros, nullptr, st, r,
+                                  kn.tiles ? 1 : 0, w.done);
                 ACE_LAUNCHED("r-column apply_A (i8a_kernel)");
             } else {
                 ProfScope ps(ACE_K_APPLY_A, st, lv * (fl_mn), lv * (vb * (n + 2.0 * m) + shA));
@@ -771,9 +790,10 @@
         if (pc) {
         } else if (gyk) {
             ProfScope ps(ACE_K_APPLY_G, st);
-            const GykArgs ga{L.Gf, w.T, B, w.Y[q], w.M, w.Y[1 - q], w.g, w.KY[q], w.KY[1 - q], w.optY, L.LK8, L.c8, w.st,
-                             w.AX, 2 - q, L.LA8, Zc, Nc, w.zeros, n, za.lazy_dual,
-                             DualCtl{za.tol_abs, za.tol_rel, za.rho, za.fixed_iters, n, 1, w.done}};
+            GykArgs ga{L.Gf, w.T, B, w.Y[q], w.M, w.Y[1 - q], w.g, w.KY[q], w.KY[1 - q], w.optY, L.LK8, L.c8, w.st,
+                       w.AX, 2 - q, L.LA8, Zc, Nc, w.zeros, n, za.lazy_dual,
+                       DualCtl{za.tol_abs, za.tol_rel, za.rho, za.fixed_iters, n, 1, w.done}};
+            ga.tiles = kn.tiles ? 1 : 0;
             launch_gyk(batch, m, ga, st);
             ACE_LAUNCHED("g / Y-step (gyk_kernel)");
         } else if (fused) {
@@ -814,7 +834,10 @@
                     za.Zn = Zo;
                     za.Nn = No;
                 }
-                launch_i8_apply_AH(batch, m, n, L.LAH8, w.g, w.X, L.c8, w.st, st, za.xfuse ? &za : nullptr);
+                ZArgs zp{};
+                zp.tiles = za.tiles;
+                zp.done_count = w.done;
+                launch_i8_apply_AH(batch, m, n, L.LAH8, w.g, w.X, L.c8, w.st, st, za.xfuse ? &za : nullptr, &zp);
             }
             else if (fused) launch_zgemm_fused(false, n, m, batch, L.AH, m, w.g, nullptr, m, w.X, w.Z, w.N, n, w.st, st);
             else if (i8r) {
@@ -824,6 +847,8 @@
                 zv.Z = w.Z;
                 zv.N = w.N;
                 zv.zeros = w.zeros;
+                zv.tiles = za.tiles;
+                zv.done_count = w.done;
                 launch_i8_apply_AH(nv, m, n, L.LAH8, w.g, w.X, L.c8, w.st, st, nullptr, &zv);
             } else applyAH(w.g, w.X, w.V);
             ACE_LAUNCHED((wmode || i8r) ? "apply_AH (i8ah_kernel)" : "apply_AH (zgemm)");
@@ -871,6 +896,7 @@
                           (gyk || pc) ? w.Y[1] : nullptr);
     }
     ACE_LAUNCHED("finalize");
+    ACE_TRY(tile_report(kn, w, st));
     return tk_report(kn, w, ACE_OK, st);
 }
 
diff --git a/2ace-mmwave-channel-estimation_amd/csrc/ace_api.cpp b/2ace-mmwave-channel-estimation_amd/csrc/ace_api.cpp
--- a/2ace-mmwave-channel-estimation_amd/csrc/ace_api.cpp
+++ b/2ace-mmwave-channel-estimation_amd/csrc/ace_api.cpp
@@ -134,8 +134,18 @@
         g_prof.msp_cap = 4096;
         ACE_HIP(hipHostMalloc(reinterpret_cast<void**>(&g_prof.msp_slots), sizeof(int) * g_prof.msp_cap));
     }
+    if (!g_prof.tile_slots)
+        ACE_HIP(hipHostMalloc(reinterpret_cast<void**>(&g_prof.tile_slots), sizeof(int) * g_prof.msp_cap));
     g_prof.msp_used = 0;
+    g_prof.tile_used = 0;
     g_prof.on = true;
+    return ACE_OK;
+}
+
+int ace_prof_tile_skips(long long* skips) {
+    g_err.clear();
+    if (!skips) return fail(ACE_ERR_ARG, "skips is NULL");
+    *skips = g_prof.tile_total;
     return ACE_OK;
 }
 
@@ -202,6 +212,9 @@
     g_prof.msp_total = 0;
     for (int i = 0; i < g_prof.msp_used; ++i) g_prof.msp_total += g_prof.msp_slots[i];
     g_prof.msp_used = 0;
+    g_prof.tile_total = 0;
+    for (int i = 0; i < g_prof.tile_used; ++i) g_prof.tile_total += g_prof.tile_slots[i];
+    g_prof.tile_used = 0;
     return ACE_OK;
 }
 
diff --git a/2ace-mmwave-channel-estimation_amd/csrc/ace_common.hpp b/2ace-mmwave-channel-estimation_amd/csrc/ace_common.hpp
--- a/2ace-mmwave-channel-estimation_amd/csrc/ace_common.hpp
+++ b/2ace-mmwave-channel-estimation_amd/csrc/ace_common.hpp
@@ -227,9 +227,11 @@
 size_t i8_frag_bytes(int mc, int kc);
 void launch_i8_expand(int m, int n, const double* A, const double* cmax, int8_t* LA, int8_t* LH, int* flag,
                       hipStream_t st);
+constexpr int I8_SKIP_SLOT = 44;
+constexpr int I8_AVOK_SLOT = 45;
 void launch_i8_apply_A(int nb, int n, int m, const int8_t* LA, const double* Z, const double* N, const double* Y,
                        const double* M, double* T, const double* cmax, const RealState* rs, const double* zeros,
-                       const double* AX, hipStream_t st, int rcols = 1);
+                       const double* AX, hipStream_t st, int rcols = 1, int tiles = 0, int* counters = nullptr);
 struct ZArgs;
 void launch_i8_apply_AH(int nb, int m, int n, const int8_t* LAH, const double* g, double* W, const double* cmax,
                         const RealState* rs, hipStream_t st, const ZArgs* fuse = nullptr,
@@ -279,6 +281,7 @@
     double fl[4];
     const unsigned char* rank_one;
     double room;
+    int tiles;
 };
 void launch_gyk(int nb, int m, const GykArgs& a, hipStream_t st);
 size_t gyf_lds_bytes(int m);
@@ -417,6 +420,7 @@
     int mthr;
     int tkeig;
     int* tkcnt;
+    int tiles;
 };
 __device__ __forceinline__ double2 xw(double2 z, double2 n, double2 w, double imu) {
     return make_double2(fma(-n.x, imu, z.x) + w.x, fma(-n.y, imu, z.y) + w.y);
diff --git a/2ace-mmwave-channel-estimation_amd/csrc/ace_host.hpp b/2ace-mmwave-channel-estimation_amd/csrc/ace_host.hpp
--- a/2ace-mmwave-channel-estimation_amd/csrc/ace_host.hpp
+++ b/2ace-mmwave-channel-estimation_amd/csrc/ace_host.hpp
@@ -56,6 +56,9 @@
     int* msp_slots = nullptr;
     int msp_cap = 0, msp_used = 0;
     long long msp_total = 0;
+    int* tile_slots = nullptr;
+    int tile_used = 0;
+    long long tile_total = 0;
 };
 inline Prof g_prof;
 inline std::atomic<long long> g_path[4];
diff --git a/2ace-mmwave-channel-estimation_amd/csrc/ace_i8gemm.hip b/2ace-mmwave-channel-estimation_amd/csrc/ace_i8gemm.hip
--- a/2ace-mmwave-channel-estimation_amd/csrc/ace_i8gemm.hip
+++ b/2ace-mmwave-channel-estimation_amd/csrc/ace_i8gemm.hip
@@ -7,16 +7,21 @@
 namespace {
 
 #ifdef ACE_PHASE_STAMPS
+#ifndef ACE_STAMP_BLOCK
+#define ACE_STAMP_BLOCK 5
+#endif
 #define STAMP_DECL unsigned long long ts_[12] = {}
-#define STAMP(i) do { if (blockIdx.x == 5 && threadIdx.x == 0) ts_[i] = __builtin_amdgcn_s_memrealtime(); } while (0)
+#define STAMP(i) do { if (threadIdx.x == 0) ts_[i] = __builtin_amdgcn_s_memrealtime(); } while (0)
 #define STAMP_D(i) (i < k_ ? ts_[i] - ts_[i - 1] : 0ull)
-#define STAMP_PRINT(name, k) do { if (blockIdx.x == 5 && threadIdx.x == 0) { const int k_ = (k); \
+#define STAMP_PRINT_IF(cond, name, k) do { if ((cond) && threadIdx.x == 0) { const int k_ = (k); \
     printf("%s %llu %llu %llu %llu %llu %llu %llu\n", name, STAMP_D(1), STAMP_D(2), STAMP_D(3), STAMP_D(4), \
            STAMP_D(5), STAMP_D(6), STAMP_D(7)); } } while (0)
+#define STAMP_PRINT(name, k) STAMP_PRINT_IF(blockIdx.x == ACE_STAMP_BLOCK, name, k)
 #else
 #define STAMP_DECL
 #define STAMP(i)
 #define STAMP_PRINT(name, k)
+#define STAMP_PRINT_IF(cond, name, k)
 #endif
 
 constexpr int RB = 16;
@@ -89,8 +94,64 @@
     kstep(a0, b.f[0][0], b.f[0][1], acc);
     kstep(a1, b.f[1][0], b.f[1][1], acc);
 }
+struct TileList {
+    int n;
+    int pk;
+};
+__device__ __forceinline__ int wg_or_mask(int v) { return __builtin_amdgcn_readfirstlane(__ockl_wgred_or_i32(v)); }
+__device__ __forceinline__ TileList tile_list(int mask) {
+    TileList tl{__builtin_popcount(mask & 15), 0};
+    int mk = mask & 15;
+#pragma unroll
+    for (int i = 0; i < 4; ++i) {
+        tl.pk |= (mk ? __builtin_ctz(mk) : 0) << (2 * i);
+        mk &= mk - 1;
+    }
+    return tl;
+}
+template <int NR>
+struct NRc {
+    static constexpr int value = NR;
+};
+template <class F>
+__device__ __forceinline__ void tile_dispatch(int n, F&& f) {
+    if (n == 4) f(NRc<4>{});
+    else if (n == 3) f(NRc<3>{});
+    else if (n == 2) f(NRc<2>{});
+    else f(NRc<1>{});
+}
+template <int NR>
+__device__ __forceinline__ int tile_of(const TileList& tl, int i) { return NR == 4 ? i : (tl.pk >> (2 * i)) & 3; }
+template <int NR>
+__device__ __forceinline__ void aload_t(const int8_t* arow, int rstride, const TileList& tl, i4v (&af)[4]) {
+    if constexpr (NR == 4) aload(arow, rstride, af);
+    else {
+#pragma unroll
+        for (int i = 0; i < NR; ++i) af[i] = *reinterpret_cast<const i4v*>(arow + 32 * tile_of<NR>(tl, i) * rstride);
+    }
+}
+template <int NR>
+__device__ __forceinline__ void kstep_t(const i4v (&af)[4], i4v b0, i4v b1, i16v (&acc)[4][2]) {
+#pragma unroll
+    for (int i = 0; i < NR; ++i) {
+        acc[i][0] = __builtin_amdgcn_mfma_i32_32x32x32_i8(af[i], b0, acc[i][0], 0, 0, 0);
+        acc[i][1] = __builtin_amdgcn_mfma_i32_32x32x32_i8(af[i], b1, acc[i][1], 0, 0, 0);
+    }
+}
+template <int NR>
+__device__ __forceinline__ void stage_mma_t(const int8_t* arow, int rstride, const TileList& tl, const BSet& b,
+                                            i16v (&acc)[4][2]) {
+    i4v a0[4], a1[4];
+    aload_t<NR>(arow, rstride, tl, a0);
+    aload_t<NR>(arow + 32, rstride, tl, a1);
+    kstep_t<NR>(a0, b.f[0][0], b.f[0][1], acc);
+    kstep_t<NR>(a1, b.f[1][0], b.f[1][1], acc);
+}
 constexpr int SKR = SK * 32;
 constexpr int RSA = SKR + 16;
+__device__ __forceinline__ int i8a_vote(int tiles, int slot, bool live, bool avok) {
+    return !tiles ? 15 : !live ? 0 : avok ? 16 : 1 << (slot >> 2);
+}
 template <bool TOL>
 __device__ __forceinline__ void i8a_block(int nb, int Kc, int Mc, int nks, const i4v* __restrict__ Bf,
                                           const double* __restrict__ Zp, const double* __restrict__ Np,
@@ -98,15 +159,24 @@
                                           double* __restrict__ Tp, int ldt, const double* __restrict__ cptr,
                                           const RealState* __restrict__ rs, const double* __restrict__ zeros,
                                           const double* __restrict__ AXp, int8_t (*As)[ROWS * RSA], double* sc_s,
-                                          double* imu_s, int* live_s, const int* avok_s, int j0, int cb, int rc = 1) {
+                                          double* imu_s, int* live_s, const int* avok_s, int j0, int cb, int rc,
+                                          int vote, int* cnt) {
     const int t = threadIdx.x, lane = t & 63, w = t >> 6;
     const int bl = t >> 5, cq = t & 31, jb = j0 + bl;
     const RealState* rj = rs + (jb < nb ? jb / rc : 0);
     const bool live = jb < nb && !rj->done;
     const double imu = live ? 1.0 / rj->mu : 0.0;
-    const d2* z = reinterpret_cast<const d2*>(Zp) + (long long)(live ? jb : 0) * Kc;
-    const d2* nn = (live && rj->nzero) ? reinterpret_cast<const d2*>(zeros)
-                                       : reinterpret_cast<const d2*>(Np) + (long long)(live ? jb : 0) * Kc;
+    const bool av = (vote & 16) && live && avok_s[bl];
+    const int myR = __builtin_amdgcn_readfirstlane(t >> 7);
+    const TileList tl = tile_list(vote);
+    const bool tile_on = vote >> myR & 1;
+    if (t == 0 && cnt && cb == 0) {
+        if (tl.n < 4) atomicAdd(cnt + I8_SKIP_SLOT, 4 - tl.n);
+        if ((vote & 16) && tl.n) atomicAdd(cnt + I8_AVOK_SLOT, 1);
+    }
+    const d2* z = av ? reinterpret_cast<const d2*>(zeros) : reinterpret_cast<const d2*>(Zp) + (long long)(live ? jb : 0) * Kc;
+    const d2* nn = (av || (live && rj->nzero)) ? reinterpret_cast<const d2*>(zeros)
+                                                : reinterpret_cast<const d2*>(Np) + (long long)(live ? jb : 0) * Kc;
     double p2, sc;
     plane_scale(live ? rj->vbound : 0.0, *cptr, p2, sc);
     if (cq == 0) {
@@ -154,42 +224,52 @@
     const i4v* bp0 = Bf + (long long)ct0 * nks * 64 + lane;
     const i4v* bp1 = bp0 + (long long)nks * 64;
 
+    const int8_t* arow0 = &As[0][(lane & 31) * RSA + 16 * (lane >> 5)];
+    const int8_t* arow1 = arow0 + ROWS * RSA;
+    const int h = lane >> 5, ldo = 2 * Mc;
+    auto body = [&](auto nrc) {
+    constexpr int NR = decltype(nrc)::value;
     i16v acc[4][2];
 #pragma unroll
-    for (int R = 0; R < 4; ++R) acc[R][0] = acc[R][1] = i16v{};
-
+    for (int i = 0; i < NR; ++i) acc[i][0] = acc[i][1] = i16v{};
+    auto lst = [&](const Raw& r, int s, int buf) {
+        if constexpr (NR == 4) lstore(r, s, buf);
+        else if (tile_on) lstore(r, s, buf);
+    };
+
+    if constexpr (NR > 0) {
     Raw r0, r1;
     BSet bA, bB;
     bload(bA, bp0, bp1, 0, kmax);
     gload(0, r0);
     gload(1, r1);
-    lstore(r0, 0, 0);
+    lst(r0, 0, 0);
     __syncthreads();
-    const int8_t* arow0 = &As[0][(lane & 31) * RSA + 16 * (lane >> 5)];
-    const int8_t* arow1 = arow0 + ROWS * RSA;
     for (int s = 0; s < nstage; s += 2) {
         bload(bB, bp0, bp1, (s + 1) * SK, kmax);
         gload(min(s + 2, nstage - 1), r0);
         __builtin_amdgcn_sched_barrier(0);
-        stage_mma(arow0, RSA, bA, acc);
+        stage_mma_t<NR>(arow0, RSA, tl, bA, acc);
         __builtin_amdgcn_sched_barrier(0);
-        lstore(r1, s + 1, 1);
+        lst(r1, s + 1, 1);
         __syncthreads();
         bload(bA, bp0, bp1, (s + 2) * SK, kmax);
         gload(min(s + 3, nstage - 1), r1);
         __builtin_amdgcn_sched_barrier(0);
-        stage_mma(arow1, RSA, bB, acc);
+        stage_mma_t<NR>(arow1, RSA, tl, bB, acc);
         __builtin_amdgcn_sched_barrier(0);
-        lstore(r0, s + 2, 0);
+        lst(r0, s + 2, 0);
         __syncthreads();
     }
-
-    const int h = lane >> 5, ldo = 2 * Mc;
-#pragma unroll
-    for (int R = 0; R < 4; ++R)
+    } else {
+        __syncthreads();
+    }
+
+#pragma unroll
+    for (int i = 0; i < NR; ++i)
 #pragma unroll
         for (int q = 0; q < 2; ++q) {
-            const int blo = 4 * R + 2 * q + h, j = j0 + blo;
+            const int blo = 4 * tile_of<NR>(tl, i) + 2 * q + h, j = j0 + blo;
             if (j >= nb || !live_s[blo]) continue;
             const double scb = sc_s[blo], im = imu_s[blo];
 #pragma unroll
@@ -197,12 +277,34 @@
                 const int col = (ct0 + c) * 32 + (lane & 31);
                 if (col >= ldo) continue;
                 const long long off = (long long)j * ldo + col;
-                const double av = avok_s[blo] ? AXp[off] : scb * recombine(acc[R][c], q);
+                const double av = avok_s[blo] ? AXp[off] : scb * recombine(acc[i][c], q);
                 const double tv = fma(-Mp[off], im, Yp[off]) - av;
                 if (TOL) Tp[blo * ldt + col] = tv;
                 else Tp[off] = tv;
             }
         }
+    if constexpr (NR < 4) {
+#pragma unroll
+        for (int R = 0; R < 4; ++R)
+#pragma unroll
+            for (int q = 0; q < 2; ++q) {
+                const int blo = 4 * R + 2 * q + h, j = j0 + blo;
+                if ((vote >> R & 1) || j >= nb || !live_s[blo]) continue;
+                const double im = imu_s[blo];
+#pragma unroll
+                for (int c = 0; c < 2; ++c) {
+                    const int col = (ct0 + c) * 32 + (lane & 31);
+                    if (col >= ldo) continue;
+                    const long long off = (long long)j * ldo + col;
+                    const double tv = fma(-Mp[off], im, Yp[off]) - AXp[off];
+                    if (TOL) Tp[blo * ldt + col] = tv;
+                    else Tp[off] = tv;
+                }
+            }
+    }
+    };
+    if (tl.n == 0) body(NRc<0>{});
+    else tile_dispatch(tl.n, body);
 }
 
 __global__ __launch_bounds__(NT, 1) void i8a_kernel(int nb, int Kc, int Mc, int nks, const i4v* __restrict__ Bf,
@@ -210,18 +312,20 @@
                                                     const double* __restrict__ Yp, const double* __restrict__ Mp,
                                                     double* __restrict__ Tp, const double* __restrict__ cptr,
                                                     const RealState* __restrict__ rs, const double* __restrict__ zeros,
-                                                    const double* __restrict__ AXp, int rc) {
+                                                    const double* __restrict__ AXp, int rc, int tiles, int* cnt) {
     __shared__ __attribute__((aligned(16))) int8_t As[2][ROWS * RSA];
     __shared__ double sc_s[RB], imu_s[RB];
     __shared__ int live_s[RB], avok_s[RB];
     const int t = threadIdx.x, j0 = blockIdx.x * RB;
+    int v = 0;
     if (t < RB) {
         const int j = j0 + t;
         avok_s[t] = AXp && j < nb && !rs[j].done && rs[j].avok;
-    }
-    __syncthreads();
+        v = i8a_vote(tiles, t, j < nb && !rs[j / rc].done, avok_s[t]);
+    }
+    const int vote = wg_or_mask(v);
     i8a_block<false>(nb, Kc, Mc, nks, Bf, Zp, Np, Yp, Mp, Tp, 0, cptr, rs, zeros, AXp, As, sc_s, imu_s, live_s, avok_s,
-                     j0, blockIdx.y, rc);
+                     j0, blockIdx.y, rc, vote, cnt);
 }
 
 struct FuseState {
@@ -248,7 +352,12 @@
     const int rc = (!FUSE && za.r > 1) ? za.r : 1;
     const bool live = jb < nb && (matz ? rs[jb].optsrc == 3
                                        : (!rs[jb / rc].done && !(za.msp && rs[jb / rc].mzit == za.it)));
-    if (!__syncthreads_or(live)) return;
+    const int myR = __builtin_amdgcn_readfirstlane(t >> 7);
+    const int lmask = wg_or_mask(live ? 1 << myR : 0);
+    if (!lmask) return;
+    const TileList tl = tile_list(za.tiles ? lmask : 15);
+    const bool tile_on = (za.tiles ? lmask : 15) >> myR & 1;
+    if (t == 0 && tl.n < 4 && za.done_count) atomicAdd(za.done_count + I8_SKIP_SLOT, 4 - tl.n);
     const int zn_id = 1 + (za.it & 1);
     if constexpr (!FUSE && !KY) {
         if (matz && t < RB) z0_s[t] = j0 + t < nb ? rs[j0 + t].z0id : 0;
@@ -309,7 +418,7 @@
         imu_s[bl] = (!KY && !FUSE && za.xzn && live) ? 1.0 / rs[jb / rc].mu : 0.0;
         if constexpr (!FUSE && !KY) nz_s[bl] = za.xzn && live && rc > 1 && rs[jb / rc].nzero;
     }
-    for (int s = 0; s < nst; ++s) {
+    for (int s = 0; s < nst && tile_on; ++s) {
         d2 x0, x1;
         if (s < GR) {
 #pragma unroll
@@ -352,45 +461,47 @@
             b.f[kk][1] = p[(long long)nks * 64];
         }
     };
-    auto zload = [&](int cbk, double (&zv)[4][2][2]) {
+    auto zload = [&](auto nrc, int cbk, double (&zv)[4][2][2]) {
+        constexpr int NR = decltype(nrc)::value;
         const int ct0 = cbk * (NCB / 32) + 2 * w;
 #pragma unroll
-        for (int R = 0; R < 4; ++R)
+        for (int i = 0; i < NR; ++i)
 #pragma unroll
             for (int q = 0; q < 2; ++q) {
-                const int blo = 4 * R + 2 * q + (lane >> 5), j = min(j0 + blo, nb - 1);
+                const int blo = 4 * tile_of<NR>(tl, i) + 2 * q + (lane >> 5), j = min(j0 + blo, nb - 1);
 #pragma unroll
                 for (int c = 0; c < 2; ++c) {
                     const int col = min((ct0 + c) * 32 + (lane & 31), 2 * Mc - 1);
-                    zv[R][q][c] = fs_s[blo].el ? za.Z[(long long)j * 2 * Mc + col] : 0.0;
+                    zv[i][q][c] = fs_s[blo].el ? za.Z[(long long)j * 2 * Mc + col] : 0.0;
                 }
             }
     };
-    auto epilogue = [&](int cbk, i16v (&acc)[4][2], const double (&zv)[4][2][2]) {
+    auto epilogue = [&](auto nrc, int cbk, i16v (&acc)[4][2], const double (&zv)[4][2][2]) {
+        constexpr int NR = decltype(nrc)::value;
         if constexpr (KY) {
             const int col = (cbk * (NCB / 64) + w) * 32 + (lane & 31);
 #pragma unroll
-            for (int R = 0; R < 4; ++R)
+            for (int i = 0; i < NR; ++i)
 #pragma unroll
                 for (int q = 0; q < 2; ++q) {
-                    const int blo = 4 * R + 2 * q + h, j = j0 + blo;
+                    const int blo = 4 * tile_of<NR>(tl, i) + 2 * q + h, j = j0 + blo;
                     if (j >= nb || !live_s[blo] || col >= ldo) continue;
                     i16v cmb;
 #pragma unroll
-                    for (int e = 0; e < 16; ++e) cmb[e] = acc[R][0][e] + 128 * acc[R][1][e];
+                    for (int e = 0; e < 16; ++e) cmb[e] = acc[i][0][e] + 128 * acc[i][1][e];
                     Wp[(long long)j * ldo + col] = sc_s[blo] * recombine(cmb, q);
                 }
 #pragma unroll
-            for (int R = 0; R < 4; ++R) acc[R][0] = acc[R][1] = i16v{};
+            for (int i = 0; i < NR; ++i) acc[i][0] = acc[i][1] = i16v{};
             return;
         }
         const int ct0 = cbk * (NCB / 32) + 2 * w;
         if constexpr (FUSE) {
 #pragma unroll
-            for (int R = 0; R < 4; ++R)
+            for (int i = 0; i < NR; ++i)
 #pragma unroll
                 for (int q = 0; q < 2; ++q) {
-                    const int blo = 4 * R + 2 * q + h, j = j0 + blo;
+                    const int R = tile_of<NR>(tl, i), blo = 4 * R + 2 * q + h, j = j0 + blo;
                     const bool el = fs_s[blo].el, kc = fs_s[blo].keep_cur;
                     double p0 = 0.0, p3 = 0.0;
                     if (j < nb && live_s[blo]) {
@@ -400,9 +511,9 @@
                             const int col = (ct0 + c) * 32 + (lane & 31);
                             if (col >= ldo) continue;
                             const long long off = (long long)j * ldo + col;
-                            const double wv = scb * recombine(acc[R][c], q);
+                            const double wv = scb * recombine(acc[i][c], q);
                             if (el) {
-                                const double x = zv[R][q][c] + wv, d = x - zv[R][q][c];
+                                const double x = zv[i][q][c] + wv, d = x - zv[i][q][c];
                                 za.Zn[off] = x;
                                 if (kc) za.Xcur[off] = x;
                                 p0 += x * x;
@@ -420,10 +531,10 @@
                 }
         } else {
 #pragma unroll
-        for (int R = 0; R < 4; ++R)
+        for (int i = 0; i < NR; ++i)
 #pragma unroll
             for (int q = 0; q < 2; ++q) {
-                const int blo = 4 * R + 2 * q + h, j = j0 + blo;
+                const int blo = 4 * tile_of<NR>(tl, i) + 2 * q + h, j = j0 + blo;
                 if (j >= nb || !live_s[blo]) continue;
                 const double scb = sc_s[blo];
 #pragma unroll
@@ -431,7 +542,7 @@
                     const int col = (ct0 + c) * 32 + (lane & 31);
                     if (col >= ldo) continue;
                     const long long off = (long long)j * ldo + col;
-                    const double wv = scb * recombine(acc[R][c], q);
+                    const double wv = scb * recombine(acc[i][c], q);
                     if (matz) Wp[off] = (z0_s[blo] == 1 ? za.Z : za.Zn)[off] + wv;
                     else if (za.xzn) {
                         const double* nrow = nz_s[blo] ? za.zeros : za.N + (long long)j * ldo;
@@ -442,11 +553,13 @@
             }
         }
 #pragma unroll
-        for (int R = 0; R < 4; ++R) acc[R][0] = acc[R][1] = i16v{};
+        for (int i = 0; i < NR; ++i) acc[i][0] = acc[i][1] = i16v{};
     };
+    tile_dispatch(tl.n, [&](auto nrc) {
+    constexpr int NR = decltype(nrc)::value;
     i16v acc[4][2];
 #pragma unroll
-    for (int R = 0; R < 4; ++R) acc[R][0] = acc[R][1] = i16v{};
+    for (int i = 0; i < NR; ++i) acc[i][0] = acc[i][1] = i16v{};
     BSet bA, bB;
     bfl(bA, 0);
     if constexpr (FUSE) {
@@ -458,39 +571,40 @@
                 const int f = f0 + 2 * SK * i;
                 bfl(bB, f + SK);
                 __builtin_amdgcn_sched_barrier(0);
-                stage_mma(arow + 32 * (f % nks), rst, bA, acc);
+                stage_mma_t<NR>(arow + 32 * (f % nks), rst, tl, bA, acc);
                 __builtin_amdgcn_sched_barrier(0);
                 bfl(bA, f + 2 * SK);
                 __builtin_amdgcn_sched_barrier(0);
-                stage_mma(arow + 32 * ((f + SK) % nks), rst, bB, acc);
+                stage_mma_t<NR>(arow + 32 * ((f + SK) % nks), rst, tl, bB, acc);
                 __builtin_amdgcn_sched_barrier(0);
             }
             const int f = f0 + 2 * SK * (per - 1);
             bfl(bB, f + SK);
-            zload(cbk, zv);
+            zload(nrc, cbk, zv);
             __builtin_amdgcn_sched_barrier(0);
-            stage_mma(arow + 32 * (f % nks), rst, bA, acc);
+            stage_mma_t<NR>(arow + 32 * (f % nks), rst, tl, bA, acc);
             __builtin_amdgcn_sched_barrier(0);
             bfl(bA, f + 2 * SK);
             __builtin_amdgcn_sched_barrier(0);
-            stage_mma(arow + 32 * ((f + SK) % nks), rst, bB, acc);
+            stage_mma_t<NR>(arow + 32 * ((f + SK) % nks), rst, tl, bB, acc);
             __builtin_amdgcn_sched_barrier(0);
-            epilogue(cbk, acc, zv);
+            epilogue(nrc, cbk, acc, zv);
         }
     } else {
         const double zv0[4][2][2] = {};
         for (int f = 0; f < total; f += 2 * SK) {
             bfl(bB, f + SK);
             __builtin_amdgcn_sched_barrier(0);
-            stage_mma(arow + 32 * (f % nks), rst, bA, acc);
+            stage_mma_t<NR>(arow + 32 * (f % nks), rst, tl, bA, acc);
             __builtin_amdgcn_sched_barrier(0);
             bfl(bA, f + 2 * SK);
             __builtin_amdgcn_sched_barrier(0);
-            stage_mma(arow + 32 * ((f + SK) % nks), rst, bB, acc);
+            stage_mma_t<NR>(arow + 32 * ((f + SK) % nks), rst, tl, bB, acc);
             __builtin_amdgcn_sched_barrier(0);
-            if ((f + 2 * SK) % nks == 0) epilogue(f / nks, acc, zv0);
-        }
-    }
+            if ((f + 2 * SK) % nks == 0) epilogue(nrc, f / nks, acc, zv0);
+        }
+    }
+    });
     STAMP(2);
     if (!KY && !FUSE) STAMP_PRINT("i8ah prologue|sweep:", 3);
     if constexpr (!FUSE && !KY) {
@@ -521,6 +635,10 @@
         }
         STAMP(3);
         STAMP_PRINT("i8ah-fused prologue|sweep|post:", 4);
+        STAMP_PRINT_IF(za.it >= 60 && __builtin_popcount(lmask) < 4,
+                       __builtin_popcount(lmask) == 1   ? "i8ah-fused 1 live tile prologue|sweep|post:"
+                       : __builtin_popcount(lmask) == 2 ? "i8ah-fused 2 live tiles prologue|sweep|post:"
+                                                        : "i8ah-fused 3 live tiles prologue|sweep|post:", 4);
     }
 }
 template <bool KY, bool FUSE>
@@ -795,14 +913,19 @@
                 for (int i = t; i < m; i += NT)
                     reinterpret_cast<d2*>(a.optY)[(long long)(j0 + r) * m + i] =
                         reinterpret_cast<const d2*>(a.Yn)[(long long)(j0 + r) * m + i];
-    int need = 0;
-    if (a.LA && t < GRB) need = live_s[t] && !avok_s[t];
-    if (__syncthreads_or(need)) {
+    int need = 0, av = 0;
+    if (a.LA && t < GRB) {
+        need = live_s[t] && !avok_s[t];
+        av = i8a_vote(a.tiles, t, live_s[t], avok_s[t]);
+    }
+    const int avote = wg_or_mask(need ? av | 32 : av);
+    if (avote & 32) {
         for (int idx = t; idx < GRB * tst; idx += NT) Ts[idx] = make_double2(0.0, 0.0);
         __syncthreads();
         i8a_block<true>(nb, a.n, m, i8_nks_dev(a.n), reinterpret_cast<const i4v*>(a.LA), a.Z, a.N, a.Yo, a.M,
                         reinterpret_cast<double*>(Ts), 2 * tst, a.c8, a.rs, a.zeros, a.AX,
-                        reinterpret_cast<int8_t(*)[ROWS * RSA]>(Ad), sc_s, p2_s, live_s, avok_s, j0, 0);
+                        reinterpret_cast<int8_t(*)[ROWS * RSA]>(Ad), sc_s, p2_s, live_s, avok_s, j0, 0, 1, avote & 31,
+                        a.dc.done_count);
     } else if (early) {
     } else
     for (int idx = t; idx < GRB * mp; idx += NT) {
@@ -1444,10 +1567,10 @@
 
 void launch_i8_apply_A(int nb, int n, int m, const int8_t* LA, const double* Z, const double* N, const double* Y,
                        const double* M, double* T, const double* cmax, const RealState* rs, const double* zeros,
-                       const double* AX, hipStream_t st, int rcols) {
+                       const double* AX, hipStream_t st, int rcols, int tiles, int* counters) {
     dim3 grid((nb + RB - 1) / RB, i8_ncols(m) / NCB, 1), block(NT);
     hipLaunchKernelGGL(i8a_kernel, grid, block, 0, st, nb, n, m, i8_nks(n), reinterpret_cast<const i4v*>(LA), Z, N,
-                       Y, M, T, cmax, rs, zeros, AX, rcols < 1 ? 1 : rcols);
+                       Y, M, T, cmax, rs, zeros, AX, rcols < 1 ? 1 : rcols, tiles, counters);
 }
 size_t i8k_frag_bytes(int m) { return (size_t)2 * ((2 * m + NCB / 2 - 1) / (NCB / 2)) * (NCB / 2) * i8_nks(m) * 32; }
 void launch_i8k_expand(int m, const double* K, const double* cmax, int8_t* LK, int* flag, hipStream_t st) {
diff --git a/include/ace.h b/include/ace.h
--- a/include/ace.h
+++ b/include/ace.h
@@ -300,6 +300,7 @@
 int ace_prof_sample(int stride, uint32_t full_mask);
 int ace_prof_stop(double* total_ms, int32_t* launches);
 int ace_prof_msp_steps(long long* steps);
+int ace_prof_tile_skips(long long* skips);
 int ace_prof_work(double* flops);
 int ace_prof_work_ex(double* flops, double* bytes, double* int8_ops);
 
```
